# xaskasdf/ntransformer

Hardware: AMD Instinct MI355X
Metric: decode tokens/sec (Llama-3.1-8B Q8_0 class, resident weights, greedy, batch 1) (higher is better)
Workload: dtype f32; 1 GPU; Llama-3.1-8B-shaped Q8_0 GGUF tensors (seed 20260925), resident in HBM, 16-token prompt, greedy decode; ctx=4096, replicas=1, hipgraph=True

## Files before the change

include/ntk_engine.h:

```cpp
#ifndef NTK_ENGINE_H
#define NTK_ENGINE_H

#include "ntk.h"

#if defined(__GNUC__)
#pragma GCC visibility push(default)
#endif
#ifdef __cplusplus
extern "C" {
#endif

int ntk_rope_kv_store(float* q, const float* k, const float* v, const int* positions, int seq_len, int n_heads, int n_kv_heads, int head_dim,
                      float theta_base, float freq_scale, int interleaved, void* k_cache, void* v_cache, int start_pos, int max_seq, void* stream);
typedef struct ntk_gemv_seg {
    const void* W;
    float*      y;
    int         rows;
    int         dtype;
} ntk_gemv_seg;

int ntk_gemv_fused(const ntk_gemv_seg* segs, int nseg, const float* x, int in_features, const float* norm_w,
                   float eps, const float* resid, int silu_pair, void* stream);

size_t ntk_q8l_bytes(int rows, int in_features);
// ... 45 lines not shown
                            const float* inv_freq, int n_heads, int n_kv_heads, int head_dim, int max_seq, float scale, float theta_base,
                            float freq_scale, int nsplit, float* scratch, void* stream);
int ntk_kv_dequant_q8_f16(void* k_f16, void* v_f16, const void* k_cache, const void* v_cache, int n_rows, int n_kv_heads, int head_dim,
                          int max_seq, void* stream);
int ntk_attention_decode_q8_batch(float* output, const float* q, const float* k, const float* v, const ntk_kv_batch* caches, const int* positions,
                                  int n_rows, const float* inv_freq, int n_heads, int n_kv_heads, int head_dim, int max_seq, float scale,
                                  float theta_base, float freq_scale, int nsplit, float* scratch, void* stream);

int ntk_debug_gemv_fused_form(const ntk_gemv_seg* segs, int nseg, const float* x, int in_features, const float* norm_w, float eps,
                              const float* resid, int silu_pair, int integer_activations, void* stream);

size_t   ntk_tp_comm_bytes(size_t max_floats);
void*    ntk_tp_comm_alloc(size_t bytes);
int      ntk_tp_comm_reset(void* comm, void* stream);
float*   ntk_tp_slot(void* comm, size_t max_floats, unsigned call_index);
int      ntk_tp_allreduce_add(float* hidden, void* const* peers, int rank, int world, size_t max_floats, unsigned call_index, int n, void* stream);
int      ntk_tp_advance_epoch(void* comm, void* stream);
unsigned ntk_tp_error(void* comm);
int      ntk_ipc_export(void* devptr, void* handle64);
int      ntk_ipc_open(const void* handle64, void** devptr);
int      ntk_ipc_close(void* devptr);

int ntk_gemm_quant(float* Y, const void* W, const float* X, int n_tokens, int out_features, int in_features,
                   int weight_dtype, const float* resid, void* stream);

typedef struct ntk_gemm_partials {
    const float* part[3];
    float*       y[3];
    int          rows[3];
    int          nseg, n_tokens, nsplit;
} ntk_gemm_partials;
typedef struct ntk_gemm_desc {
    const ntk_gemv_seg* segs;
    int                 nseg;
    const float*        X;
    int                 n_tokens, in_features;
    const float*        resid;
    void*               workspace;
    size_t              workspace_bytes;
    int                 reuse_x;
    const float*        row_max;
    ntk_gemm_partials*  partials;
    int                 weights_repacked;
    int                 full_form;
} ntk_gemm_desc;
size_t ntk_gemm_quant_workspace_bytes(int in_features, int out_features);
int ntk_gemm_quant_f16(const ntk_gemm_desc* desc, void* stream);
int ntk_reduce_rmsnorm_rowmax(float* hidden, const ntk_gemm_partials* partials, const float* weight, float eps, float* x_out, float* row_max,
                              float* zero_tokens, void* stream);
int ntk_reduce_silu_mul_rowmax(float* output, const ntk_gemm_partials* partials, float* row_max, void* stream);
int ntk_rmsnorm_rowmax(float* output, const float* input, const float* weight, int n_tokens, int hidden_size, float eps, float* row_max,
                       float* zero_tokens, void* stream);
int ntk_silu_mul_rowmax(float* output, const float* gate, const float* up, int n_tokens, int width, float* row_max, void* stream);
int ntk_gemm_prepare_x(const float* X, int n_tokens, int in_features, void* workspace, void* stream);
int ntk_rmsnorm_prepare_x(float* output, const float* input, const float* weight, int n_tokens, int hidden_size, float eps, void* workspace, void* stream);
int ntk_reduce_rmsnorm_prepare_x(float* hidden, const ntk_gemm_partials* partials, const float* weight, float eps, float* x_out, void* workspace, void* stream);
int ntk_silu_mul_prepare_x(float* output, const float* gate, const float* up, int n_tokens, int width, void* workspace, void* stream);
int ntk_reduce_silu_mul_prepare_x(float* output, const ntk_gemm_partials* partials, void* workspace, void* stream);

int ntk_embed_rows(float* out, const void* table, const int* tokens, int n_tokens, int hidden, int dtype,
                   void* stream);

int ntk_argmax(const float* logits, int n, int* d_out_token, int* h_mirror, float* scratch, void* stream);

int ntk_logprob_rows(const float* logits, int n_rows, int vocab, int ld, const int* targets, float* logprob, int* top1, void* stream);

size_t ntk_sample_scratch_bytes(int n);
int ntk_sample_top_k(float* logits, int n, const int* d_recent, int n_recent, float repeat_penalty, float temperature,
                     int top_k, float top_p, float r, int* d_out_token, int* h_mirror, void* scratch, void* stream);
int ntk_repeat_penalty(float* logits, int n, const int* d_recent, int n_recent, float repeat_penalty, void* stream);

#define NTK_SAMPLE_ROWS_MAX 16
typedef struct ntk_sample_rows {
    float temperature[NTK_SAMPLE_ROWS_MAX], top_p[NTK_SAMPLE_ROWS_MAX], repeat_penalty[NTK_SAMPLE_ROWS_MAX], r[NTK_SAMPLE_ROWS_MAX];
    int   top_k[NTK_SAMPLE_ROWS_MAX], n_recent[NTK_SAMPLE_ROWS_MAX];
} ntk_sample_rows;
size_t ntk_sample_rows_scratch_bytes(int n_rows, int vocab);
int ntk_sample_rows_top_k(float* logits, int n_rows, int vocab, int ld, const int* d_recent, int recent_ld, const ntk_sample_rows* rows, int* d_out,
                          int* h_mirror, void* scratch, void* stream);

int ntk_argmax_advance(const float* logits, int n, int* d_out_token, int* h_mirror, unsigned long long* h_ring4, int* d_pos,
                       float* scratch, void* stream);

int ntk_debug_sclk(unsigned long long* d_out2, void* stream);
int ntk_debug_sclk_begin(unsigned* d_flag, unsigned long long* d_out2, void* side_stream);
int ntk_debug_sclk_end(unsigned* d_flag, void* other_stream);

void ntk_debug_malloc_budget(long long bytes);

int ntk_advance_pos(int* d_pos, void* stream);

#ifdef __cplusplus
}
#endif
#if defined(__GNUC__)
#pragma GCC visibility pop
#endif
#endif
```

ntransformer_amd/_lib.py:

```python
from __future__ import annotations

import ctypes as C
import os

_HERE = os.path.dirname(os.path.abspath(__file__))
LIB_PATH = os.environ.get("NTK_LIB_PATH") or os.path.join(_HERE, "libntransformer_hip.so")

NTK_OK = 0
_STATUS = {0: "ok", -1: "unsupported dtype", -2: "bad shape", -3: "HIP launch/runtime error", -4: "misaligned pointer",
           -5: "null pointer", -6: "no usable GPU", -7: "out of memory", -8: "I/O error", -9: "malformed GGUF"}


class NtkError(RuntimeError):
    def __init__(self, status: int, what: str = ""):
        self.status = status
        super().__init__("ntk status %d (%s)%s" % (status, _STATUS.get(status, "?"), (": " + what) if what else ""))


def check(status: int, what: str = "") -> None:
    if status != NTK_OK:
        raise NtkError(status, what)


class KvBatch(C.Structure):
# ... 28 lines not shown
        return _lib
    if not os.path.exists(LIB_PATH):
        raise ImportError("%s is missing: run `python -c 'import __graft_entry__ as g; g.build()'` "
                          "(hipcc --offload-arch=gfx950); there is no CPU fallback" % LIB_PATH)
    L = C.CDLL(LIB_PATH, mode=C.RTLD_GLOBAL)
    vp, i, f, sz = C.c_void_p, C.c_int, C.c_float, C.c_size_t
    sig = {
        "ntk_abi_version": (i, []),
        "ntk_status_string": (C.c_char_p, [i]),
        "ntk_row_bytes": (sz, [i, C.c_int64]),
        "ntk_device_count": (i, []),
        "ntk_device_init": (i, [i]),
        "ntk_device_name": (i, [C.c_char_p, sz]),
        "ntk_device_mem_info": (i, [C.POINTER(sz), C.POINTER(sz)]),
        "ntk_stream": (vp, [i]),
        "ntk_stream_synchronize": (i, [vp]),
        "ntk_device_synchronize": (i, []),
        "ntk_event_create": (vp, []),
        "ntk_event_destroy": (i, [vp]),
        "ntk_event_record": (i, [vp, vp]),
        "ntk_event_synchronize": (i, [vp]),
        "ntk_event_elapsed_ms": (i, [vp, vp, C.POINTER(f)]),
        "nt_hip_malloc": (vp, [sz]), "nt_hip_free": (None, [vp]),
        "nt_hip_memcpy_h2d": (None, [vp, vp, sz]), "nt_hip_memcpy_d2h": (None, [vp, vp, sz]),
        "nt_hip_memcpy_d2d": (None, [vp, vp, sz]), "nt_hip_memset": (None, [vp, i, sz]),
        "nt_hip_malloc_host": (vp, [sz]), "nt_hip_free_host": (None, [vp]),
        "ntk_memcpy_h2d_async": (i, [vp, vp, sz, vp]), "ntk_memcpy_d2h_async": (i, [vp, vp, sz, vp]),
        "nt_cuda_malloc": (vp, [sz]), "nt_cuda_free": (None, [vp]),
        "nt_cuda_memcpy_h2d": (None, [vp, vp, sz]), "nt_cuda_memcpy_d2h": (None, [vp, vp, sz]),
        "nt_cuda_memcpy_d2d": (None, [vp, vp, sz]), "nt_cuda_memset": (None, [vp, i, sz]),
        "nt_cuda_malloc_host": (vp, [sz]), "nt_cuda_free_host": (None, [vp]),
        "ntk_rmsnorm": (i, [vp, vp, vp, i, i, f, vp]),
        "ntk_rmsnorm_f16": (i, [vp, vp, vp, i, i, f, vp]),
        "ntk_rope": (i, [vp, vp, vp, i, i, i, i, i, f, f, i, vp]),
        "ntk_softmax": (i, [vp, vp, i, i, vp]),
        "ntk_masked_softmax": (i, [vp, vp, vp, i, i, vp]),
        "ntk_gemv": (i, [vp, vp, vp, i, i, i, vp]),
        "ntk_gemv_add": (i, [vp, vp, vp, i, i, i, vp]),
        "ntk_gemm_f32": (i, [vp, vp, vp, i, i, i, vp]),
        "ntk_silu_mul": (i, [vp, vp, vp, i, vp]),
        "ntk_rmsnorm_rowmax": (i, [vp, vp, vp, i, i, f, vp, vp, vp]),
        "ntk_rope_kv_store": (i, [vp, vp, vp, vp, i, i, i, i, f, f, i, vp, vp, i, i, vp]),
        "ntk_silu_mul_rowmax": (i, [vp, vp, vp, i, i, vp, vp]),
        "ntk_add_bias": (i, [vp, vp, i, vp]),
        "ntk_attention_decode": (i, [vp, vp, vp, vp, i, i, i, i, i, f, vp]),
        "ntk_attention_prefill": (i, [vp, vp, vp, vp, i, i, i, i, i, i, f, vp]),
        "ntk_copy_to_kv_cache": (i, [vp, vp, vp, vp, i, i, i, i, i, vp]),
        "ntk_add": (i, [vp, vp, vp, i, vp]),
        "ntk_add_inplace": (i, [vp, vp, i, vp]),
        "ntk_copy": (i, [vp, vp, i, vp]),
        "ntk_cosine_similarity": (i, [vp, vp, vp, i, vp]),
        "ntk_gemv_fused": (i, [C.POINTER(GemvSeg), i, vp, i, vp, f, vp, i, vp]),
        "ntk_debug_gemv_fused_form": (i, [C.POINTER(GemvSeg), i, vp, i, vp, f, vp, i, i, vp]),
        "ntk_q8l_bytes": (sz, [i, i]),
        "ntk_q8l_pack": (i, [vp, vp, i, i, vp]),
        "ntk_q8l_unpack": (i, [vp, vp, i, i, vp]),
        "ntk_rp_bytes": (sz, [i, i, i]),
        "ntk_rp_pack": (i, [vp, vp, i, i, i, vp]),
        "ntk_rp_dequant": (i, [vp, vp, i, i, i, vp]),
        "ntk_rp_unpack": (i, [vp, vp, i, i, i, vp]),
        "ntk_gemv_rp": (i, [vp, vp, vp, i, i, i, vp]),
        "ntk_gemv_rp_fused": (i, [C.POINTER(GemvSeg), i, vp, i, vp, f, vp, i, vp]),
        "ntk_debug_rp_prologue": (i, [vp, vp, vp, f, i, i, i, vp]),
        "ntk_debug_mfma_i8_probe": (i, [vp, vp, vp, vp]),
        "ntk_gemm_quant": (i, [vp, vp, vp, i, i, i, i, vp, vp]),
        "ntk_attention_decode_split": (i, [vp, vp, vp, vp, vp, vp, vp, vp, i, i, i, i, f, f, f, i, vp, vp]),
        "ntk_attention_split_scratch_bytes": (C.c_size_t, [i, i, i]),
        "ntk_attention_split_scratch_init": (i, [vp, i, vp]),
        "ntk_attention_decode_split_merged": (i, [vp, vp, vp, vp, vp, vp, vp, vp, i, i, i, i, f, f, f, i, vp, vp]),
        "ntk_attention_decode_fused": (i, [vp, vp, vp, vp, vp, vp, vp, vp, i, i, i, i, f, f, f, vp]),
        "ntk_attention_decode_batch": (i, [vp, vp, vp, vp, vp, vp, i, vp, i, i, i, i, f, f, f, i, vp, vp]),
        "ntk_kv_q8_cache_bytes": (C.c_size_t, [i, i, i]),
        "ntk_kv_store_q8": (i, [vp, vp, vp, vp, i, i, i, i, i, vp]),
        "ntk_rope_kv_store_q8": (i, [vp, vp, vp, vp, i, i, i, i, f, f, i, vp, vp, i, i, vp]),
        "ntk_attention_decode_q8": (i, [vp, vp, vp, vp, vp, vp, vp, vp, i, i, i, i, f, f, f, i, vp, vp]),
        "ntk_kv_dequant_q8_f16": (i, [vp, vp, vp, vp, i, i, i, i, vp]),
        "ntk_attention_decode_q8_batch": (i, [vp, vp, vp, vp, vp, vp, i, vp, i, i, i, i, f, f, f, i, vp, vp]),
        "ntk_embed_rows": (i, [vp, vp, vp, i, i, i, vp]),
        "ntk_argmax": (i, [vp, i, vp, vp, vp, vp]),
        "ntk_logprob_rows": (i, [vp, i, i, i, vp, vp, vp, vp]),
        "ntk_sample_rows_scratch_bytes": (C.c_size_t, [i, i]),
        "ntk_sample_rows_top_k": (i, [vp, i, i, i, vp, i, C.POINTER(SampleRows), vp, vp, vp, vp]),
        "ntk_advance_pos": (i, [vp, vp]),
        "ntk_debug_sclk": (i, [vp, vp]),
        "ntk_debug_sclk_begin": (i, [vp, vp, vp]),
        "ntk_debug_sclk_end": (i, [vp, vp]),
    }
    for name, (res, args) in sig.items():
        fn = getattr(L, name)
        fn.restype = res
        fn.argtypes = args
    _lib = L
    return L


EXPORTS_NTK_H = None
```

ntransformer_amd/csrc/common.hip.h:

```cpp
#pragma once
#include <hip/hip_runtime.h>
#include <stdint.h>
#include "../../include/ntk_engine.h"

#define NTK_WAVE 64

#define NTK_HIP_TRY(expr)                                   \
    do {                                                    \
        hipError_t e__ = (expr);                            \
        if (e__ != hipSuccess) return NTK_E_LAUNCH;         \
    } while (0)

#define NTK_EXTRA_API extern "C" __attribute__((visibility("default")))
#ifdef NTK_TUNE
#include <cstdlib>
#define NTK_TUNE_ENV_INT(name, dflt) ([] { const char* e__ = getenv(name); return e__ ? atoi(e__) : (dflt); }())
#else
#define NTK_TUNE_ENV_INT(name, dflt) (dflt)
#endif

namespace ntk {

hipStream_t resolve_stream(void* s);
int         last_launch_status();
int         q8l_gemv_fused(const ntk_gemv_seg* segs, int nseg, const float* x, int in, const float* norm_w, float eps, const float* resid,
                           int silu_pair, hipStream_t st);

__device__ __forceinline__ float h2f(uint16_t bits) {
    _Float16 h;
    __builtin_memcpy(&h, &bits, 2);
    return (float)h;
}
__device__ __forceinline__ uint16_t f2h(float f) {
    _Float16 h = (_Float16)f;
    uint16_t bits;
    __builtin_memcpy(&bits, &h, 2);
    return bits;
}

__device__ __forceinline__ void rope_rotate(const float a, const float b, const float c, const float s, float& ra, float& rb) {
#pragma clang fp contract(off)
    ra = a * c - b * s;
    rb = b * c + a * s;
}

template <int CTRL, int ROW_MASK>
__device__ __forceinline__ float dpp_or_zero(float v) {
    return __int_as_float(__builtin_amdgcn_update_dpp(0, __float_as_int(v), CTRL, ROW_MASK, 0xF, false));
}
template <int CTRL, int ROW_MASK>
__device__ __forceinline__ float dpp_or_self(float v) {
    return __int_as_float(__builtin_amdgcn_update_dpp(__float_as_int(v), __float_as_int(v), CTRL, ROW_MASK, 0xF, false));
}
constexpr int DPP_QUAD_1032 = 0xB1, DPP_QUAD_2301 = 0x4E, DPP_ROW_HALF_MIRROR = 0x141, DPP_ROW_MIRROR = 0x140,
              DPP_ROW_BCAST15 = 0x142, DPP_ROW_BCAST31 = 0x143;

__device__ __forceinline__ float wave_sum_lane63(float v) {
    v += dpp_or_zero<DPP_QUAD_1032, 0xF>(v);
    v += dpp_or_zero<DPP_QUAD_2301, 0xF>(v);
    v += dpp_or_zero<DPP_ROW_HALF_MIRROR, 0xF>(v);
    v += dpp_or_zero<DPP_ROW_MIRROR, 0xF>(v);
    v += dpp_or_zero<DPP_ROW_BCAST15, 0xA>(v);
    v += dpp_or_zero<DPP_ROW_BCAST31, 0xC>(v);
    return v;
}
__device__ __forceinline__ float wave_sum(float v) {
    return __int_as_float(__builtin_amdgcn_readlane(__float_as_int(wave_sum_lane63(v)), 63));
}
__device__ __forceinline__ float wave_max(float v) {
    v = fmaxf(v, dpp_or_self<DPP_QUAD_1032, 0xF>(v));
    v = fmaxf(v, dpp_or_self<DPP_QUAD_2301, 0xF>(v));
    v = fmaxf(v, dpp_or_self<DPP_ROW_HALF_MIRROR, 0xF>(v));
    v = fmaxf(v, dpp_or_self<DPP_ROW_MIRROR, 0xF>(v));
    v = fmaxf(v, dpp_or_self<DPP_ROW_BCAST15, 0xA>(v));
    v = fmaxf(v, dpp_or_self<DPP_ROW_BCAST31, 0xC>(v));
    return __int_as_float(__builtin_amdgcn_readlane(__float_as_int(v), 63));
}

template <int N>
__device__ __forceinline__ float group_sum(float v) {
    static_assert(N == 1 || N == 2 || N == 4 || N == 8 || N == 16 || N == 32, "group size");
    if constexpr (N >= 2) v += dpp_or_zero<DPP_QUAD_1032, 0xF>(v);
    if constexpr (N >= 4) v += dpp_or_zero<DPP_QUAD_2301, 0xF>(v);
    if constexpr (N >= 8) v += dpp_or_zero<DPP_ROW_HALF_MIRROR, 0xF>(v);
    if constexpr (N >= 16) v += dpp_or_zero<DPP_ROW_MIRROR, 0xF>(v);
    if constexpr (N >= 32) v += __shfl_xor(v, 16, 64);
    return v;
}

__device__ __forceinline__ float block_sum(float v, float* red) {
    const int lane = threadIdx.x & 63, wave = threadIdx.x >> 6, nw = (blockDim.x + 63) >> 6;
    v = wave_sum(v);
    __syncthreads();
    if (lane == 0) red[wave] = v;
    __syncthreads();
    float t = 0.0f;
    for (int i = 0; i < nw; ++i) t += red[i];
    return t;
}
__device__ __forceinline__ float block_max(float v, float* red) {
    const int lane = threadIdx.x & 63, wave = threadIdx.x >> 6, nw = (blockDim.x + 63) >> 6;
    v = wave_max(v);
    __syncthreads();
    if (lane == 0) red[wave] = v;
    __syncthreads();
    float t = red[0];
    for (int i = 1; i < nw; ++i) t = fmaxf(t, red[i]);
    return t;
}

__device__ __forceinline__ uint32_t lds_u32_at(const uint8_t* base, int off) {
    const int a = off & ~3;
    const uint32_t lo = *reinterpret_cast<const uint32_t*>(base + a);
    const uint32_t hi = *reinterpret_cast<const uint32_t*>(base + a + 4);
    return __builtin_amdgcn_alignbyte(hi, lo, (uint32_t)(off & 3));
}
template <int N>
__device__ __forceinline__ void lds_read_dwords(uint32_t (&dst)[N], const uint8_t* base, int off) {
    const int a = off & ~3;
    const uint32_t sh = (uint32_t)(off & 3);
    uint32_t w[N + 1];
#pragma unroll
    for (int i = 0; i <= N; ++i) w[i] = *reinterpret_cast<const uint32_t*>(base + a + 4 * i);
#pragma unroll
    for (int i = 0; i < N; ++i) dst[i] = __builtin_amdgcn_alignbyte(w[i + 1], w[i], sh);
}
// ... 26 lines not shown
```

ntransformer_amd/csrc/elementwise.hip:

```cpp
#include "common.hip.h"
#include <cfloat>

namespace ntk {

template <bool HALF_OUT>
__global__ __launch_bounds__(1024) void rmsnorm_kernel(void* __restrict__ output, const float* __restrict__ input,
                                                       const float* __restrict__ weight, int hidden, float eps) {
    __shared__ float red[16];
    const float* x = input + (size_t)blockIdx.x * hidden;
    float ssq = 0.0f;
    for (int i = threadIdx.x; i < hidden; i += blockDim.x) ssq = fmaf(x[i], x[i], ssq);
    const float tot = block_sum(ssq, red);
    const float rms_inv = 1.0f / sqrtf(tot / (float)hidden + eps);
    for (int i = threadIdx.x; i < hidden; i += blockDim.x) {
        const float v = x[i] * rms_inv * weight[i];
        if constexpr (HALF_OUT) reinterpret_cast<uint16_t*>(output)[(size_t)blockIdx.x * hidden + i] = f2h(v);
        else reinterpret_cast<float*>(output)[(size_t)blockIdx.x * hidden + i] = v;
    }
}

template <bool MASKED>
__global__ __launch_bounds__(1024) void softmax_kernel(float* __restrict__ out, const float* __restrict__ in,
                                                       const uint8_t* __restrict__ mask, int cols) {
    __shared__ float red[16];
// ... 18 lines not shown
        const float g = gate[i];
        out[i] = g / (1.0f + expf(-g)) * up[i];
    }
}
__global__ void add_kernel(float* __restrict__ o, const float* __restrict__ a, const float* __restrict__ b, int n) {
    const int i = blockIdx.x * blockDim.x + threadIdx.x;
    if (i < n) o[i] = a[i] + b[i];
}
__global__ void copy_kernel(float* __restrict__ d, const float* __restrict__ s, int n) {
    const int i = blockIdx.x * blockDim.x + threadIdx.x;
    if (i < n) d[i] = s[i];
}
__global__ void gemm_f32_kernel(float* __restrict__ C, const float* __restrict__ A, const float* __restrict__ B, int M, int N, int K) {
    const int col = blockIdx.x * blockDim.x + threadIdx.x, row = blockIdx.y * blockDim.y + threadIdx.y;
    if (row >= M || col >= N) return;
    float s = 0.0f;
    for (int k = 0; k < K; ++k) s = fmaf(A[(size_t)row * K + k], B[(size_t)col * K + k], s);
    C[(size_t)row * N + col] = s;
}
__global__ __launch_bounds__(256) void cosine_kernel(float* __restrict__ result, const float* __restrict__ a,
                                                     const float* __restrict__ b, int n) {
    __shared__ float red[16];
    float d = 0.0f, na = 0.0f, nb = 0.0f;
    for (int i = threadIdx.x; i < n; i += blockDim.x) {
        d = fmaf(a[i], b[i], d); na = fmaf(a[i], a[i], na); nb = fmaf(b[i], b[i], nb);
    }
    d = block_sum(d, red); na = block_sum(na, red); nb = block_sum(nb, red);
    if (threadIdx.x == 0) {
        const float den = sqrtf(na) * sqrtf(nb);
        *result = den > 1e-8f ? d / den : 0.0f;
    }
}

__device__ float embed_elem(const uint8_t* __restrict__ table, int tok, int hidden, int dt, int e) {
    switch (dt) {
        case NTK_DT_F32: return reinterpret_cast<const float*>(table)[(size_t)tok * hidden + e];
        case NTK_DT_F16: return h2f(reinterpret_cast<const uint16_t*>(table)[(size_t)tok * hidden + e]);
        case NTK_DT_Q8_0: {
            const uint8_t* b = table + ((size_t)tok * (hidden / 32) + e / 32) * 34;
            const float d = h2f((uint16_t)(b[0] | (b[1] << 8)));
            return __fmul_rn(d, (float)(int8_t)b[2 + (e & 31)]);
        }
        case NTK_DT_Q4_0: {
            const uint8_t* b = table + ((size_t)tok * (hidden / 32) + e / 32) * 18;
            const float d = h2f((uint16_t)(b[0] | (b[1] << 8)));
            const int j = e & 31;
            const int nib = j < 16 ? (b[2 + j] & 0x0F) : (b[2 + j - 16] >> 4);
            return __fmul_rn(d, (float)(nib - 8));
        }
        case NTK_DT_Q4_K: {
            const uint8_t* b = table + ((size_t)tok * (hidden / 256) + e / 256) * 144;
            const float d = h2f((uint16_t)(b[0] | (b[1] << 8))), dmin = h2f((uint16_t)(b[2] | (b[3] << 8)));
            const int w = e & 255, sub = w >> 5, l = w & 31, chunk = sub >> 1;
            const uint8_t* s = b + 4;
            uint32_t sc, mn;
            if (sub < 4) { sc = s[sub] & 63; mn = s[sub + 4] & 63; }
            else { sc = (s[sub + 4] & 0x0F) | ((s[sub - 4] >> 6) << 4); mn = (s[sub + 4] >> 4) | ((s[sub] >> 6) << 4); }
            const uint8_t qb = b[16 + 32 * chunk + l];
            const int nib = (sub & 1) ? (qb >> 4) : (qb & 0x0F);
            return __fsub_rn(__fmul_rn(__fmul_rn(d, (float)sc), (float)nib), __fmul_rn(dmin, (float)mn));
        }
        case NTK_DT_Q6_K: {
            const uint8_t* b = table + ((size_t)tok * (hidden / 256) + e / 256) * 210;
            const float d = h2f((uint16_t)(b[208] | (b[209] << 8)));
            const int w = e & 255, hf = w >> 7, g = (w >> 5) & 3, l = w & 31, is = l >> 4;
            const uint8_t* ql = b + 64 * hf;
            const uint8_t* qh = b + 128 + 32 * hf;
            const int8_t sc = (int8_t)b[192 + 8 * hf + is + 2 * g];
            const uint8_t qlb = ql[l + 32 * (g & 1)];
            const int lo = (g >> 1) ? (qlb >> 4) : (qlb & 0x0F);
            const int q = (lo | (((qh[l] >> (2 * g)) & 3) << 4)) - 32;
            return __fmul_rn(__fmul_rn(d, (float)sc), (float)q);
        }
        default: return 0.0f;
    }
}
__global__ void embed_rows_kernel(float* __restrict__ out, const uint8_t* __restrict__ table, const int* __restrict__ tokens,
                                  int hidden, int dt) {
    const int tok = tokens[blockIdx.x];
    const int e = blockIdx.y * blockDim.x + threadIdx.x;
    if (e < hidden) out[(size_t)blockIdx.x * hidden + e] = embed_elem(table, tok, hidden, dt, e);
}

__device__ __forceinline__ void amax_merge(float& v, int& i, float ov, int oi) {
    if (ov > v || (ov == v && oi < i)) { v = ov; i = oi; }
}
__global__ __launch_bounds__(256) void argmax_stage1(const float* __restrict__ x, int n, float* __restrict__ sv, int* __restrict__ si) {
    __shared__ float rv[4];
    __shared__ int ri[4];
    float v = -FLT_MAX;
    int idx = 0x7FFFFFFF;
    for (int i = blockIdx.x * blockDim.x + threadIdx.x; i < n; i += gridDim.x * blockDim.x) amax_merge(v, idx, x[i], i);
    for (int off = 32; off > 0; off >>= 1) amax_merge(v, idx, __shfl_xor(v, off, 64), __shfl_xor(idx, off, 64));
    if ((threadIdx.x & 63) == 0) { rv[threadIdx.x >> 6] = v; ri[threadIdx.x >> 6] = idx; }
    __syncthreads();
    if (threadIdx.x == 0) {
        for (int w = 1; w < 4; ++w) amax_merge(v, idx, rv[w], ri[w]);
        sv[blockIdx.x] = v; si[blockIdx.x] = idx;
    }
}
__global__ __launch_bounds__(256) void argmax_stage2(const float* __restrict__ sv, const int* __restrict__ si, int nblk,
                                                     int* __restrict__ d_out, int* __restrict__ h_mirror) {
    __shared__ float rv[4];
    __shared__ int ri[4];
    float v = -FLT_MAX;
    int idx = 0x7FFFFFFF;
    for (int i = threadIdx.x; i < nblk; i += blockDim.x) amax_merge(v, idx, sv[i], si[i]);
    for (int off = 32; off > 0; off >>= 1) amax_merge(v, idx, __shfl_xor(v, off, 64), __shfl_xor(idx, off, 64));
    if ((threadIdx.x & 63) == 0) { rv[threadIdx.x >> 6] = v; ri[threadIdx.x >> 6] = idx; }
    __syncthreads();
    if (threadIdx.x == 0) {
        for (int w = 1; w < 4; ++w) amax_merge(v, idx, rv[w], ri[w]);
        if (idx == 0x7FFFFFFF) idx = 0;
        *d_out = idx;
        if (h_mirror) *h_mirror = idx;
    }
}
__global__ void advance_pos_kernel(int* p) { if (threadIdx.x == 0 && blockIdx.x == 0) *p += 1; }

__global__ __launch_bounds__(64) void sclk_probe_kernel(unsigned long long* out) {
    const unsigned long long t0 = __builtin_amdgcn_s_memtime(), r0 = __builtin_amdgcn_s_memrealtime();
    unsigned long long r1 = r0;
    float acc = (float)threadIdx.x;
    while (r1 - r0 < 5000ull) {
#pragma unroll
        for (int i = 0; i < 64; ++i) acc = fmaf(acc, 1.0000001f, 1e-9f);
        r1 = __builtin_amdgcn_s_memrealtime();
    }
    const unsigned long long t1 = __builtin_amdgcn_s_memtime();
    if (threadIdx.x == 0) { out[0] = t1 - t0; out[1] = r1 - r0; }
    if (acc == 12345.678f) out[2] = 0;
}

__global__ __launch_bounds__(64) void sclk_span_kernel(const unsigned* flag, unsigned long long* out) {
    const unsigned long long t0 = __builtin_amdgcn_s_memtime(), r0 = __builtin_amdgcn_s_memrealtime();
    unsigned long long r1 = r0;
    for (;;) {
        __builtin_amdgcn_s_sleep(64);
        r1 = __builtin_amdgcn_s_memrealtime();
        if (__hip_atomic_load(flag, __ATOMIC_RELAXED, __HIP_MEMORY_SCOPE_SYSTEM) != 0u || r1 - r0 > 300000000ull) break;
    }
    const unsigned long long t1 = __builtin_amdgcn_s_memtime();
    if (threadIdx.x == 0) { out[0] = t1 - t0; out[1] = r1 - r0; }
}

__global__ __launch_bounds__(256) void argmax_advance_stage2(const float* __restrict__ sv, const int* __restrict__ si, int nblk,
                                                             int* __restrict__ d_out, int* __restrict__ h_mirror,
                                                             unsigned long long* __restrict__ h_ring, int* __restrict__ d_pos) {
    __shared__ float rv[4];
    __shared__ int ri[4];
    float v = -FLT_MAX;
    int idx = 0x7FFFFFFF;
    for (int i = threadIdx.x; i < nblk; i += blockDim.x) amax_merge(v, idx, sv[i], si[i]);
    for (int off = 32; off > 0; off >>= 1) amax_merge(v, idx, __shfl_xor(v, off, 64), __shfl_xor(idx, off, 64));
    if ((threadIdx.x & 63) == 0) { rv[threadIdx.x >> 6] = v; ri[threadIdx.x >> 6] = idx; }
    __syncthreads();
    if (threadIdx.x == 0) {
        for (int w = 1; w < 4; ++w) amax_merge(v, idx, rv[w], ri[w]);
        if (idx == 0x7FFFFFFF) idx = 0;
        const int pos = *d_pos;
        *d_out = idx;
        if (h_mirror) *h_mirror = idx;
        if (h_ring)
            __hip_atomic_store(h_ring + (pos & 3), (unsigned long long)(unsigned)idx | ((unsigned long long)(unsigned)(pos + 1) << 32),
                               __ATOMIC_RELEASE, __HIP_MEMORY_SCOPE_SYSTEM);
        *d_pos = pos + 1;
    }
}

static inline dim3 g1(int n) { return dim3((n + 255) / 256); }

}

extern "C" {
using namespace ntk;

static int rms_block(int hidden) { return hidden <= 1024 ? 256 : (hidden <= 4096 ? 512 : 1024); }

int ntk_rmsnorm(float* output, const float* input, const float* weight, int batch_size, int hidden_size, float eps, void* stream) {
    if (!output || !input || !weight) return NTK_E_NULL;
    if (batch_size < 0 || hidden_size <= 0) return NTK_E_SHAPE;
    if (batch_size == 0) return NTK_OK;
    hipLaunchKernelGGL(rmsnorm_kernel<false>, dim3(batch_size), dim3(rms_block(hidden_size)), 0, resolve_stream(stream),
                       (void*)output, input, weight, hidden_size, eps);
    return last_launch_status();
}
int ntk_rmsnorm_f16(void* output, const float* input, const float* weight, int batch_size, int hidden_size, float eps, void* stream) {
    if (!output || !input || !weight) return NTK_E_NULL;
    if (batch_size < 0 || hidden_size <= 0) return NTK_E_SHAPE;
    if (batch_size == 0) return NTK_OK;
    hipLaunchKernelGGL(rmsnorm_kernel<true>, dim3(batch_size), dim3(rms_block(hidden_size)), 0, resolve_stream(stream),
                       output, input, weight, hidden_size, eps);
    return last_launch_status();
}
int ntk_softmax(float* output, const float* input, int rows, int cols, void* stream) {
    if (!output || !input) return NTK_E_NULL;
    if (rows < 0 || cols <= 0) return NTK_E_SHAPE;
    if (rows == 0) return NTK_OK;
    hipLaunchKernelGGL(softmax_kernel<false>, dim3(rows), dim3(cols <= 1024 ? 256 : 1024), 0, resolve_stream(stream), output,
                       input, (const uint8_t*)nullptr, cols);
    return last_launch_status();
}
int ntk_masked_softmax(float* output, const float* input, const uint8_t* mask, int rows, int cols, void* stream) {
    if (!output || !input || !mask) return NTK_E_NULL;
    if (rows < 0 || cols <= 0) return NTK_E_SHAPE;
    if (rows == 0) return NTK_OK;
    hipLaunchKernelGGL(softmax_kernel<true>, dim3(rows), dim3(cols <= 1024 ? 256 : 1024), 0, resolve_stream(stream), output,
                       input, mask, cols);
    return last_launch_status();
}
int ntk_gemm_f32(float* C, const float* A, const float* B, int M, int N, int K, void* stream) {
    if (!C || !A || !B) return NTK_E_NULL;
    if (M < 0 || N < 0 || K < 0) return NTK_E_SHAPE;
    if (M == 0 || N == 0) return NTK_OK;
    hipLaunchKernelGGL(gemm_f32_kernel, dim3((N + 15) / 16, (M + 15) / 16), dim3(16, 16), 0, resolve_stream(stream), C, A, B, M, N, K);
    return last_launch_status();
}
int ntk_silu_mul(float* output, const float* gate, const float* up, int size, void* stream) {
    if (!output || !gate || !up) return NTK_E_NULL;
    if (size < 0) return NTK_E_SHAPE;
    if (size == 0) return NTK_OK;
    hipLaunchKernelGGL(silu_mul_kernel, g1(size), dim3(256), 0, resolve_stream(stream), output, gate, up, size);
    return last_launch_status();
}
int ntk_add(float* out, const float* a, const float* b, int size, void* stream) {
    if (!out || !a || !b) return NTK_E_NULL;
    if (size < 0) return NTK_E_SHAPE;
    if (size == 0) return NTK_OK;
    hipLaunchKernelGGL(add_kernel, g1(size), dim3(256), 0, resolve_stream(stream), out, a, b, size);
    return last_launch_status();
}
int ntk_add_inplace(float* a, const float* b, int size, void* stream) { return ntk_add(a, a, b, size, stream); }
int ntk_add_bias(float* y, const float* bias, int size, void* stream) { return ntk_add(y, y, bias, size, stream); }
int ntk_copy(float* dst, const float* src, int size, void* stream) {
    if (!dst || !src) return NTK_E_NULL;
    if (size < 0) return NTK_E_SHAPE;
    if (size == 0) return NTK_OK;
    hipLaunchKernelGGL(copy_kernel, g1(size), dim3(256), 0, resolve_stream(stream), dst, src, size);
    return last_launch_status();
}
int ntk_cosine_similarity(float* result, const float* a, const float* b, int size, void* stream) {
    if (!result || !a || !b) return NTK_E_NULL;
    if (size < 0) return NTK_E_SHAPE;
    hipLaunchKernelGGL(cosine_kernel, dim3(1), dim3(256), 0, resolve_stream(stream), result, a, b, size);
    return last_launch_status();
}
int ntk_embed_rows(float* out, const void* table, const int* tokens, int n_tokens, int hidden, int dtype, void* stream) {
    if (!out || !table || !tokens) return NTK_E_NULL;
    if (n_tokens < 0 || hidden <= 0) return NTK_E_SHAPE;
    if (n_tokens == 0) return NTK_OK;
    hipLaunchKernelGGL(embed_rows_kernel, dim3(n_tokens, (hidden + 255) / 256), dim3(256), 0, resolve_stream(stream), out, (const uint8_t*)table,
                       tokens, hidden, dtype);
    const int st = last_launch_status();
    if (st != NTK_OK) return st;
    switch (dtype) {
        case NTK_DT_F32: case NTK_DT_F16: case NTK_DT_Q8_0: case NTK_DT_Q4_0: case NTK_DT_Q4_K: case NTK_DT_Q6_K: return NTK_OK;
        default: return NTK_E_DTYPE;
    }
}
int ntk_argmax(const float* logits, int n, int* d_out_token, int* h_mirror, float* scratch, void* stream) {
    if (!logits || !d_out_token || !scratch) return NTK_E_NULL;
    if (n <= 0) return NTK_E_SHAPE;
    const int nblk = n < 256 * 8 ? 1 : (n / (256 * 8) < 1024 ? n / (256 * 8) : 1024);
    float* sv = scratch;
    int* si = reinterpret_cast<int*>(scratch + 1024);
    hipStream_t st = resolve_stream(stream);
    hipLaunchKernelGGL(argmax_stage1, dim3(nblk), dim3(256), 0, st, logits, n, sv, si);
    hipLaunchKernelGGL(argmax_stage2, dim3(1), dim3(256), 0, st, (const float*)sv, (const int*)si, nblk, d_out_token, h_mirror);
    return last_launch_status();
}
int ntk_argmax_advance(const float* logits, int n, int* d_out_token, int* h_mirror, unsigned long long* h_ring4, int* d_pos, float* scratch,
                       void* stream) {
    if (!logits || !d_out_token || !scratch || !d_pos) return NTK_E_NULL;
    if (n <= 0) return NTK_E_SHAPE;
    const int nblk = n < 256 * 8 ? 1 : (n / (256 * 8) < 1024 ? n / (256 * 8) : 1024);
    float* sv = scratch;
    int* si = reinterpret_cast<int*>(scratch + 1024);
    hipStream_t st = resolve_stream(stream);
    hipLaunchKernelGGL(argmax_stage1, dim3(nblk), dim3(256), 0, st, logits, n, sv, si);
    hipLaunchKernelGGL(argmax_advance_stage2, dim3(1), dim3(256), 0, st, (const float*)sv, (const int*)si, nblk, d_out_token, h_mirror, h_ring4, d_pos);
    return last_launch_status();
}
int ntk_debug_sclk(unsigned long long* d_out2, void* stream) {
    if (!d_out2) return NTK_E_NULL;
    hipLaunchKernelGGL(sclk_probe_kernel, dim3(1), dim3(64), 0, resolve_stream(stream), d_out2);
    return last_launch_status();
}
int ntk_debug_sclk_begin(unsigned* d_flag, unsigned long long* d_out2, void* side_stream) {
    if (!d_flag || !d_out2 || !side_stream) return NTK_E_NULL;
    hipStream_t st = static_cast<hipStream_t>(side_stream);
    if (hipMemsetAsync(d_flag, 0, 4, st) != hipSuccess) return NTK_E_LAUNCH;
    hipLaunchKernelGGL(sclk_span_kernel, dim3(1), dim3(64), 0, st, (const unsigned*)d_flag, d_out2);
    return last_launch_status();
}
int ntk_debug_sclk_end(unsigned* d_flag, void* other_stream) {
    if (!d_flag || !other_stream) return NTK_E_NULL;
    static const unsigned one = 1u;
    return hipMemcpyAsync(d_flag, &one, 4, hipMemcpyHostToDevice, static_cast<hipStream_t>(other_stream)) == hipSuccess ? NTK_OK : NTK_E_LAUNCH;
}
int ntk_advance_pos(int* d_pos, void* stream) {
    if (!d_pos) return NTK_E_NULL;
    hipLaunchKernelGGL(advance_pos_kernel, dim3(1), dim3(64), 0, resolve_stream(stream), d_pos);
    return last_launch_status();
}

}
```

ntransformer_amd/csrc/engine/model.cpp:

```cpp
#include "model_impl.h"
#include <thread>

namespace nt {

Model::~Model() { free_all(); }

void Model::drop_graphs(int slot) {
    for (auto& row : graphs_)
        for (int k = 0; k <= kAttnRegimes; ++k) {
            if (slot >= 0 && k != slot) continue;
            if (row[k]) (void)hipGraphExecDestroy(reinterpret_cast<hipGraphExec_t>(row[k]));
            row[k] = nullptr;
        }
}

void Model::free_all() {
    drop_graphs();
    destroy_persistent_plan();
    persistent_on_ = false;
    for (int r = 0; r < 8; ++r) {
        if (tp_peer_opened_[r] && tp_peers_[r]) (void)ntk_ipc_close(tp_peers_[r]);
        tp_peers_[r] = nullptr;
        tp_peer_opened_[r] = false;
    }
    tp_connected_ = false;
    tp_comm_ = nullptr;
    tp_call_ = 0;
    if (own_stream_ && stream_) (void)hipStreamDestroy(static_cast<hipStream_t>(stream_));
    own_stream_ = false;
    stream_ = nullptr;
    for (void* p : allocs_) nt_hip_free(p);
    allocs_.clear();
    auto free_host = [](auto*& p) { if (p) nt_hip_free_host(p); p = nullptr; };
    free_host(h_token_); free_host(h_ring_); free_host(h_recent_); free_host(h_batch_recent_); free_host(h_batch_next_);
    sample_scratch_ = gemm_ws_ = gemm_ws2_ = nullptr;
    d_recent_ = nullptr;
    attn_sync_ = nullptr;
    shares_weights_ = false;
    layers_.clear();
    token_embd_ = output_norm_ = output_ = DevTensor();
    weight_bytes_ = repack_bytes_ = raw_freed_bytes_ = 0;
    raw_scratch_ = nullptr; raw_scratch_bytes_ = raw_cursor_ = 0; raw_err_ = 0;
    repack_done_ = output_tied_ = false;
    host_pos_ = attn_regime_ = 0;
    k_cache_ = v_cache_ = nullptr;
    slot_k_.clear(); slot_v_.clear(); slot_k_q8_.clear(); slot_v_q8_.clear();
    batch_logits_ = batch_logprob_ = batch_attn_scratch_ = nullptr; batch_in_ = batch_next_ = batch_recent_ = nullptr; batch_sample_scratch_ = nullptr;
    kv_capture_ = nullptr; kv_capture_layer_ = -1; kv_capture_T_ = 0;
    k_cache_q8_ = v_cache_q8_ = nullptr; kv_f16_k_ = kv_f16_v_ = nullptr; kv_q8_layer_bytes_ = 0; kv_cache_bytes_ = 0;
    hidden_ = residual_ = workspace_ = logits_ = argmax_scratch_ = rope_inv_freq_ = attn_scratch_ = row_max_ = nullptr;
    positions_ = tokens_dev_ = d_pos_ = d_token_ = nullptr;
    score_logits_ = score_logprob_ = nullptr; score_targets_ = score_top1_ = nullptr; score_cap_ = 0;
    score_ws_ = nullptr; score_ws_bytes_ = 0;
}

int Model::share_weights(const Model& src, int max_context) {
    if (&src == this) { err_ = "share_weights: a model cannot share its own weights"; return NTK_E_NULL; }
    free_all();
    if (src.layers_.empty()) { err_ = "share_weights: the source model is not loaded"; return NTK_E_NULL; }
    if (src.tp_world_ != 1 || src.shares_weights_) {
        err_ = "share_weights: the source must hold whole tensors of its own (no tensor parallelism, not itself a sharing sequence)";
        return NTK_E_SHAPE;
    }
    cfg_ = src.cfg_;
    cfg_full_ = src.cfg_;
    if (max_context > 0) cfg_.max_seq_len = max_context;
    vocab_ = src.vocab_;
    layers_ = src.layers_;
    token_embd_ = src.token_embd_; output_norm_ = src.output_norm_; output_ = src.output_;
    output_tied_ = src.output_tied_;
    weight_bytes_ = src.weight_bytes_;
    repack_ = src.repack_; repack_wanted_ = src.repack_; repack_done_ = true;
    repack_bytes_ = 0;
    shares_weights_ = true;
    if (src.raw_freed_bytes_ > 0 && src.raw_scratch_bytes_ > 0) {
        void* d = nt_hip_malloc(src.raw_scratch_bytes_);
        if (!d) { err_ = "share_weights: no device memory for the unpack scratch"; free_all(); return NTK_E_NOMEM; }
        allocs_.push_back(d);
        raw_scratch_ = d; raw_scratch_bytes_ = src.raw_scratch_bytes_;
        raw_freed_bytes_ = src.raw_freed_bytes_;
    }
    int rc = own_stream();
    if (rc == NTK_OK) rc = alloc_buffers();
    if (rc != NTK_OK) free_all();
    return rc;
}

int Model::set_attention_merge(bool on) {
    if (on == attn_merge_) return NTK_OK;
    if (!layers_.empty()) {
        NT_TRY(sync());
        drop_graphs();
    }
    attn_merge_ = on;
    return NTK_OK;
}

int Model::set_repack(int level) {
    level = level < 0 ? 0 : level > 3 ? 3 : level;
    if (shares_weights_) { err_ = "set_repack: this sequence shares another model's tensors"; return NTK_E_SHAPE; }
    repack_wanted_ = level;
    if (layers_.empty()) { repack_ = level; return NTK_OK; }
    if (level == 3) level = 2;
    if (level == repack_) return NTK_OK;
    NT_TRY(sync());
    drop_graphs();
    int rc = NTK_OK;
    if (level < 2 && raw_freed_bytes_ > 0) rc = restore_raw_all();
    if (rc == NTK_OK && level > 0 && !repack_done_) {
        rc = repack_all();
        if (rc == NTK_E_NOMEM) { fprintf(stderr, "warning: decode repack incomplete (device memory): the rest stays on the raw path\n"); rc = NTK_OK; err_.clear(); }
    }
    if (rc != NTK_OK) { err_ = std::string("set_repack: ") + ntk_status_string(rc); return rc; }
    repack_ = level;
    if (level == 2) {
        destroy_persistent_plan();
        persistent_on_ = false;
        rc = drop_raw_all();
    }
    return rc;
}

uint64_t Model::bytes_per_token(int pos) const {
    uint64_t b = 0;
    for (const auto& L : layers_)
        for (auto m : kLayerMatrices) b += (L.*m).nbytes;
    b += output_.nbytes;
    b += (uint64_t)(2 * cfg_.n_layers + 1) * cfg_.hidden_size * 4;
    const uint64_t kv_elems = (uint64_t)cfg_.n_kv_heads * cfg_.head_dim;
    const uint64_t kv_row = kv_q8_ ? kv_elems + kv_elems / 16 : kv_elems * 2;
    b += 2ull * cfg_.n_layers * kv_row * (uint64_t)(pos + 1) + 2ull * cfg_.n_layers * kv_row;
    b += ntk_row_bytes(token_embd_.dtype, cfg_.hidden_size);
    return b;
}

int Model::set_device_token(int token) {
    if (token < 0 || token >= cfg_.vocab_size) { err_ = "token id out of range"; return NTK_E_SHAPE; }
    *h_token_ = token;
    return ntk_memcpy_h2d_async(d_token_, h_token_, 4, stream_);
}
int Model::set_device_pos(int pos) {
    host_pos_ = pos;
    NT_TRY(ntk_memcpy_h2d_async(d_pos_, &pos, 4, stream_));
    NT_TRY(ntk_stream_synchronize(stream_));
    if (h_ring_) memset(h_ring_, 0, 64);
    return NTK_OK;
}
int Model::sync() { return ntk_stream_synchronize(stream_); }
int Model::host_token() const { return *h_token_; }
int Model::copy_logits(float* host) {
    NT_TRY(ntk_memcpy_d2h_async(host, logits_, (size_t)cfg_.vocab_size * 4, stream_));
    return ntk_stream_synchronize(stream_);
}

int Model::sample_on_device(const int* recent, int n_recent, float repeat_penalty, float temperature, int top_k, float top_p, float r) {
    if (!sample_scratch_ || !d_recent_ || !h_recent_) return NTK_E_NOMEM;
    if (n_recent > kRecentCap) { recent += n_recent - kRecentCap; n_recent = kRecentCap; }
    void* s = stream_;
    if (repeat_penalty > 1.0f && n_recent > 0) {
        memcpy(h_recent_, recent, (size_t)n_recent * 4);
        NT_TRY(ntk_memcpy_h2d_async(d_recent_, h_recent_, (size_t)n_recent * 4, s));
    } else {
        n_recent = 0;
    }
    if (temperature <= 0.0f) {
        NT_TRY(ntk_repeat_penalty(logits_, cfg_.vocab_size, d_recent_, n_recent, repeat_penalty, s));
        return ntk_argmax(logits_, cfg_.vocab_size, d_token_, h_token_, argmax_scratch_, s);
    }
    return ntk_sample_top_k(logits_, cfg_.vocab_size, d_recent_, n_recent, repeat_penalty, temperature, top_k, top_p, r, d_token_,
                            h_token_, sample_scratch_, s);
}

int Model::wait_token(int pos, int* token) {
    volatile unsigned long long* slot = h_ring_ + (pos & 3);
    const unsigned want = (unsigned)(pos + 1);
    for (unsigned spins = 0;; ++spins) {
        const unsigned long long v = *slot;
        if ((unsigned)(v >> 32) == want) { *token = (int)(unsigned)v; return NTK_OK; }
#if defined(__x86_64__) || defined(__i386__)
        __builtin_ia32_pause();
#else
        std::this_thread::yield();
#endif
        if ((spins & 0xFFFFu) == 0xFFFFu) {
            const auto now = std::chrono::steady_clock::now();
            if (spins == 0xFFFFu) wait_t0_ = now;
            else if (std::chrono::duration<double>(now - wait_t0_).count() > 2.0) break;
        }
    }
    static bool warned = false;
    if (!warned) { warned = true; fprintf(stderr, "warning: the pinned token ring was not seen updating for 2 s (host memory not coherent with a running kernel?); falling back to a stream synchronisation per token\n"); }
    NT_TRY(ntk_stream_synchronize(stream_));
    const unsigned long long v = *slot;
    if ((unsigned)(v >> 32) != want) { err_ = "decode step finished without publishing its token"; return NTK_E_LAUNCH; }
    *token = (int)(unsigned)v;
    return NTK_OK;
}

int Model::set_sequences(int n) {
    if (n < 1 || n > kMaxSequences) { err_ = "sequences must lie in 1 .. " + std::to_string(kMaxSequences); return NTK_E_SHAPE; }
    sequences_ = n;
    return NTK_OK;
}

int Model::set_batch_kv_q8(bool on) {
    if (!layers_.empty()) { err_ = "batch_kv_q8 must be set before the model is loaded"; return NTK_E_SHAPE; }
    batch_kv_q8_ = on;
    return NTK_OK;
}

int Model::set_kv_cache(const std::string& kind) {
    if (kind != "f16" && kind != "q8_0") { err_ = "kv_cache: unknown format '" + kind + "' (f16 or q8_0)"; return NTK_E_DTYPE; }
    if (!layers_.empty()) { err_ = "kv_cache must be set before the model is loaded"; return NTK_E_SHAPE; }
    const bool q8 = kind == "q8_0";
    if (q8 && fuse_attention_) { err_ = "kv_cache=q8_0 is not supported with the attention-inside-Wo launch (fuse_attention)"; return NTK_E_SHAPE; }
    kv_q8_ = q8;
    return NTK_OK;
}

int Model::set_fuse_attention(bool on) {
    if (on && kv_q8_) { err_ = "fuse_attention (attention inside the Wo launch) is not supported with kv_cache=q8_0"; return NTK_E_SHAPE; }
    fuse_attention_ = on;
    return NTK_OK;
}

bool Model::use_persistent_now() const {
    return persistent_plan_ && persistent_on_ && attn_regime_ == 0 && !prof_;
}

void Model::set_persistent(int level) {
    const bool on = level != 0;
    persistent_on_ = false;
    persistent_wanted_ = level;
    if (on && !experiments_built()) fprintf(stderr, "note: the persistent token kernels are built by experiments/Makefile only (experiments/libntransformer_hip_exp.so); this library decodes with fused launches\n");
    if (persistent_plan_ && persistent_kind_ != (level == 2 ? 2 : 1)) {
        (void)sync();
        destroy_persistent_plan();
    }
    if (!on || tp_world_ != 1 || layers_.empty()) return;
    if (kv_q8_) { fprintf(stderr, "note: the persistent token kernels read the F16 KV cache; kv_cache=q8_0 decodes with fused launches\n"); return; }
// ... 43 lines not shown
```

ntransformer_amd/csrc/engine/model.h:

```cpp
#pragma once
#include <array>
#include <chrono>
#include <cstdint>
#include <string>
#include <vector>
#include "gguf.h"
#include "synth.h"

struct ntk_sample_rows;

struct ihipGraphExec_t;

namespace nt {

struct DevTensor {
    void* ptr = nullptr;
    int dtype = 0;
    int64_t in_f = 0, out_f = 0;
    size_t nbytes = 0;
    void* rp = nullptr;
    size_t rp_bytes = 0;
};

struct LayerWeights {
// ... 39 lines not shown
        if (pos < 544) return 0;
        return pos < (head_dim == 128 ? 3072 : 16384) ? 1 : 2;
    }
    static int attention_splits(int regime, int head_dim) { return regime <= 1 ? 8 : head_dim == 128 ? 32 : 16; }
    static constexpr int kMaxAttnSplits = 32;
    void pick_attention_regime();
    int sync();
    int host_token() const;
    int wait_token(int pos, int* token);
    float* logits_ptr() { return logits_; }
    int copy_logits(float* host);
    int sample_on_device(const int* recent, int n_recent, float repeat_penalty, float temperature, int top_k, float top_p, float r);
    static bool device_sampler_supports(float temperature, int top_k, int vocab) {
        return temperature <= 0.0f || (top_k > 0 && top_k <= 64 && top_k < vocab && vocab <= 131072);
    }

    const ModelConfig& config() const { return cfg_; }
    const GgufVocab& vocab() const { return vocab_; }
    const std::string& error() const { return err_; }
    uint64_t weight_bytes() const { return weight_bytes_; }
    uint64_t bytes_per_token(int pos) const;
    void set_batched_prefill(bool on) { batched_prefill_ = on; }
    void set_persistent(int level);
    int persistent_kind() const { return persistent_plan_ ? persistent_kind_ : 0; }
    int set_fuse_attention(bool on);
    int set_kv_cache(const std::string& kind);
    bool kv_q8() const { return kv_q8_; }
    static int kv_q8_splits(int regime) { return regime == 0 ? 4 : regime == 1 ? 16 : 32; }
    uint64_t kv_cache_bytes() const { return kv_cache_bytes_; }
    int debug_kv_inputs_capture(int layer);
    int debug_kv_inputs_read(int n, float* k, float* v);
    int debug_kv_q8(int layer, int pos0, int n, uint8_t* k_blocks, uint8_t* v_blocks, bool write, int slot = 0);
    void set_prefill_row_max(bool on) { prefill_row_max_ = on; }
    void set_prefill_fused_split(bool on) { prefill_fused_split_ = on; }
    int set_attention_merge(bool on);
    int set_repack(int level);
    bool repack() const { return repack_ != 0; }
    int repack_level() const { return repack_; }
    uint64_t repack_bytes() const { return repack_bytes_; }
    uint64_t resident_weight_bytes() const { return weight_bytes_ - raw_freed_bytes_ + repack_bytes_ + raw_scratch_bytes_; }
    void set_bf16_prefill(bool on) { bf16_prefill_ = on; }
    bool persistent_available() const { return persistent_plan_ != nullptr; }
    void* persistent_plan() const { return persistent_plan_; }
    const char* decode_path() const;
    int check_persistent();
    int check_tp();
    int debug_run_layers(const float* hidden_in, int T, int start_pos, int first, int count, int mode, float* hidden_out);
    int debug_kv(int layer, int pos0, int n, uint16_t* k, uint16_t* v, bool write, int slot = 0);
    int profile_token(float ms[4], int calls[4], bool coarse);
    void* stream() const { return stream_; }

    int tp_configure(int rank, int world);
    int tp_rank() const { return tp_rank_; }
    int tp_world() const { return tp_world_; }
    int tp_export(void* handle64, void** raw);
    int tp_connect(const void* handles, void* const* raws);
    unsigned tp_error();
    static int slice_columns(void* dst, const void* src, int dtype, int64_t out_f, int64_t in_f, int rank, int world);

private:
    int load_impl(const std::string& gguf_path, int max_context);
    int finish_load();
    int init_device();
    int own_stream();
    int alloc_buffers();
    int upload(DevTensor& dst, const void* host, int dtype, int64_t in_f, int64_t out_f, size_t nbytes);
    int upload_shard(DevTensor& dst, const void* host_full, int dtype, int64_t in_f, int64_t out_f, size_t nbytes_full, Shard how);
    struct TensorSlot { DevTensor* dst; Shard how; int64_t in_f, out_f; };
    bool slot_of(const std::string& name, TensorSlot* slot);
    template <class F> void for_each_projection(F&& fn) { for (auto& L : layers_) for (auto m : kLayerMatrices) fn(L.*m); fn(output_); }
    int repack_all();
    int repack_one(DevTensor& t);
    int drop_raw_all();
    int restore_raw_all();
    void raw_begin() { raw_cursor_ = 0; }
    const void* raw_of(const DevTensor& t);
    int tp_check_shapes();
    int tp_allreduce(float* hidden, int n);
    float* tp_slot() const;
    void free_all();
    void drop_graphs(int slot = -1);
    struct Views { float *q, *k, *v, *attn_out, *gate, *up; };
    Views views(int T) const;
    int enqueue_token(bool greedy);
    int enqueue_layers(int first, int last);
    int decode_project(const DevTensor* const* ws, float* const* ys, int n, const float* x, const DevTensor* norm, const float* resid, int kind,
                       int silu_pair = 0, bool timed = true);
    struct KvTarget { int slot; const int* slots; int max_pos; };
    int layers_1to1(int T, int start_pos, int first, int last, const KvTarget& kv = KvTarget{0, nullptr, 0});
    int lm_head(float* logits, const float* X, int n, const float* row_max);
    bool lm_head_f16() const;
    int lm_head_workspace(const char* who);
    int batch_buffers();
    int batch_logits(const int* slots, const int* tokens, const int* positions, int B);
    int batch_sample_buffers();
    int score_buffers();
    void prof_mark(int cls, bool begin);
    bool use_persistent_now() const;
    static bool experiments_built();
    int build_persistent_plan(int kind);
    void destroy_persistent_plan();
    int launch_persistent();
    int attention_in_wo(const LayerWeights& L, int layer);
    int check_experiments();

    ModelConfig cfg_;
    GgufVocab vocab_;
    std::string err_;
    std::vector<LayerWeights> layers_;
    DevTensor token_embd_, output_norm_, output_;
    bool output_tied_ = false;
    uint64_t weight_bytes_ = 0;
    std::vector<void*> allocs_;
    bool shares_weights_ = false;

    uint16_t* k_cache_ = nullptr;
    uint16_t* v_cache_ = nullptr;
    bool kv_q8_ = false;
    int sequences_ = 1;
    std::vector<uint16_t*> slot_k_, slot_v_;
    float* batch_logits_ = nullptr;
    int* batch_in_ = nullptr;
    int batch_host_[3 * 16] = {};
    float* batch_logprob_ = nullptr;
    int* batch_next_ = nullptr;
    float* batch_attn_scratch_ = nullptr;
    int* batch_recent_ = nullptr;
    int* h_batch_recent_ = nullptr;
    void* batch_sample_scratch_ = nullptr;
    int* h_batch_next_ = nullptr;
    uint8_t* k_cache_q8_ = nullptr;
    uint8_t* v_cache_q8_ = nullptr;
    size_t kv_q8_layer_bytes_ = 0;
    bool batch_kv_q8_ = false;
    std::vector<uint8_t*> slot_k_q8_, slot_v_q8_;
    uint16_t* kv_f16_k_ = nullptr;
    uint16_t* kv_f16_v_ = nullptr;
    uint64_t kv_cache_bytes_ = 0;
    float* kv_capture_ = nullptr;
    int kv_capture_layer_ = -1, kv_capture_T_ = 0;
    float* hidden_ = nullptr;
    float* residual_ = nullptr;
    float* workspace_ = nullptr;
    size_t workspace_floats_ = 0;
    float* logits_ = nullptr;
    int score_rows_ = 256;
    float* score_logits_ = nullptr;
    int score_cap_ = 0;
    int* score_targets_ = nullptr;
    float* score_logprob_ = nullptr;
    int* score_top1_ = nullptr;
    void* score_ws_ = nullptr;
    size_t score_ws_bytes_ = 0;
    int* positions_ = nullptr;
    int* tokens_dev_ = nullptr;
    int* d_pos_ = nullptr;
    int* d_token_ = nullptr;
    int* h_token_ = nullptr;
    unsigned long long* h_ring_ = nullptr;
    std::chrono::steady_clock::time_point wait_t0_;
    float* argmax_scratch_ = nullptr;
    void* sample_scratch_ = nullptr;
    int* d_recent_ = nullptr;
    int* h_recent_ = nullptr;
    static constexpr int kRecentCap = kMaxRecent;
    float* rope_inv_freq_ = nullptr;
    void* stream_ = nullptr;
    bool batched_prefill_ = true;
    struct Timed { int cls; void* a; void* b; int n; bool shared_a; };
    bool prof_coarse_ = false;
    std::vector<Timed>* prof_ = nullptr;
    static constexpr int kPersistentSlot = kAttnRegimes;
    ihipGraphExec_t* graphs_[2][kAttnRegimes + 1] = {};
    int host_pos_ = 0;
    int attn_regime_ = 0;
    float* attn_scratch_ = nullptr;
    bool prefill_row_max_ = true;
    float* row_max_ = nullptr;
    void* gemm_ws_ = nullptr;
    void* gemm_ws2_ = nullptr;
    bool prefill_fused_split_ = true;
    size_t gemm_ws_bytes_ = 0;
    bool bf16_prefill_ = true;
    unsigned* attn_sync_ = nullptr;
    int repack_ = 3;
    int repack_wanted_ = 3;
    bool repack_done_ = false;
    uint64_t repack_bytes_ = 0;
    uint64_t raw_freed_bytes_ = 0;
    void* raw_scratch_ = nullptr;
    size_t raw_scratch_bytes_ = 0, raw_cursor_ = 0;
    int raw_err_ = 0;
    bool attn_merge_ = false;
    bool fuse_attention_ = false;
    int tp_rank_ = 0, tp_world_ = 1;
    void* tp_comm_ = nullptr;
    size_t tp_max_floats_ = 0;
    void* tp_peers_[8] = {nullptr, nullptr, nullptr, nullptr, nullptr, nullptr, nullptr, nullptr};
    bool tp_peer_opened_[8] = {false, false, false, false, false, false, false, false};
    bool tp_connected_ = false;
    unsigned tp_call_ = 0;
    bool own_stream_ = false;
    ModelConfig cfg_full_;
    void* persistent_plan_ = nullptr;
    bool persistent_on_ = false;
    int persistent_wanted_ = 0;
    int persistent_kind_ = 1;
};

}
```

ntransformer_amd/csrc/engine/model_debug.cpp:

```cpp
#include "model_impl.h"

namespace nt {

int Model::debug_run_layers(const float* hidden_in, int T, int start_pos, int first, int count, int mode, float* hidden_out) {
    if (!hidden_in || !hidden_out) return NTK_E_NULL;
    if (T <= 0 || start_pos < 0 || start_pos + T > cfg_.max_seq_len || first < 0 || count < 0 || first + count > cfg_.n_layers) return NTK_E_SHAPE;
    if (mode != 0 && T != 1) return NTK_E_SHAPE;
    if (tp_world_ > 1) return NTK_E_SHAPE;
    const size_t bytes = (size_t)T * cfg_.hidden_size * 4;
    void* s = stream_;
    NT_TRY(ntk_memcpy_h2d_async(hidden_, hidden_in, bytes, s));
    int rc;
    if (mode == 0) {
        std::vector<int> pos(T);
        for (int i = 0; i < T; ++i) pos[i] = start_pos + i;
        NT_TRY(ntk_memcpy_h2d_async(positions_, pos.data(), (size_t)T * 4, s));
        NT_TRY(ntk_stream_synchronize(s));
        rc = layers_1to1(T, start_pos, first, first + count);
    } else {
        NT_TRY(set_device_pos(start_pos));
        pick_attention_regime();
        if (mode == 1) {
            rc = enqueue_layers(first, first + count);
        } else {
            hipStream_t st = static_cast<hipStream_t>(s);
            hipGraphExec_t ex = nullptr;
            rc = capture_graph(st, hipStreamCaptureModeThreadLocal, [&] { return enqueue_layers(first, first + count); }, &ex);
            if (rc == NTK_OK && hipGraphLaunch(ex, st) != hipSuccess) rc = NTK_E_LAUNCH;
            if (rc == NTK_OK) rc = ntk_stream_synchronize(s);
            if (ex) (void)hipGraphExecDestroy(ex);
        }
    }
    if (rc != NTK_OK) return rc;
    NT_TRY(ntk_memcpy_d2h_async(hidden_out, hidden_, bytes, s));
    return ntk_stream_synchronize(s);
}

int Model::debug_kv(int layer, int pos0, int n, uint16_t* k, uint16_t* v, bool write, int slot) {
    if (!k || !v) return NTK_E_NULL;
    if (kv_q8_) { err_ = "debug_kv: the KV cache is q8_0 (use the _q8 form)"; return NTK_E_DTYPE; }
    if (layer < 0 || layer >= cfg_.n_layers || pos0 < 0 || n < 0 || pos0 + n > cfg_.max_seq_len || slot < 0 || slot >= (int)slot_k_.size()) return NTK_E_SHAPE;
    const size_t per = (size_t)cfg_.n_kv_heads * cfg_.head_dim;
    uint16_t* const kcache = slot_k_[slot];
    uint16_t* const vcache = slot_v_[slot];
    const size_t off = ((size_t)layer * cfg_.max_seq_len + pos0) * per, bytes = (size_t)n * per * 2;
    void* s = stream_;
    NT_TRY(write ? ntk_memcpy_h2d_async(kcache + off, k, bytes, s) : ntk_memcpy_d2h_async(k, kcache + off, bytes, s));
    NT_TRY(write ? ntk_memcpy_h2d_async(vcache + off, v, bytes, s) : ntk_memcpy_d2h_async(v, vcache + off, bytes, s));
    return ntk_stream_synchronize(s);
}

int Model::debug_kv_q8(int layer, int pos0, int n, uint8_t* k_blocks, uint8_t* v_blocks, bool write, int slot) {
    if (!k_blocks || !v_blocks) return NTK_E_NULL;
    if (!kv_q8_) { err_ = "debug_kv_q8: the KV cache is f16"; return NTK_E_DTYPE; }
    if (layer < 0 || layer >= cfg_.n_layers || pos0 < 0 || n < 0 || pos0 + n > cfg_.max_seq_len || slot < 0 || slot >= (int)slot_k_q8_.size()) return NTK_E_SHAPE;
    if (n == 0) return NTK_OK;
    const size_t per = (size_t)cfg_.n_kv_heads * cfg_.head_dim, nb = per / 32;
    const size_t qbytes = (size_t)n * per, sbytes = (size_t)n * nb * 2;
    void* s = stream_;
    std::vector<uint8_t> qh(qbytes), sh(sbytes);
    for (int side = 0; side < 2; ++side) {
        uint8_t* base = (side ? slot_v_q8_[slot] : slot_k_q8_[slot]) + (size_t)layer * kv_q8_layer_bytes_;
        uint8_t* qd = base + (size_t)pos0 * per;
        uint8_t* sd = base + (size_t)cfg_.max_seq_len * per + (size_t)pos0 * nb * 2;
        uint8_t* blocks = side ? v_blocks : k_blocks;
        if (write) {
            for (size_t b = 0; b < (size_t)n * nb; ++b) {
                memcpy(&sh[2 * b], blocks + 34 * b, 2);
                memcpy(&qh[32 * b], blocks + 34 * b + 2, 32);
            }
            NT_TRY(ntk_memcpy_h2d_async(qd, qh.data(), qbytes, s));
            NT_TRY(ntk_memcpy_h2d_async(sd, sh.data(), sbytes, s));
            NT_TRY(ntk_stream_synchronize(s));
        } else {
            NT_TRY(ntk_memcpy_d2h_async(qh.data(), qd, qbytes, s));
            NT_TRY(ntk_memcpy_d2h_async(sh.data(), sd, sbytes, s));
            NT_TRY(ntk_stream_synchronize(s));
            for (size_t b = 0; b < (size_t)n * nb; ++b) {
                memcpy(blocks + 34 * b, &sh[2 * b], 2);
                memcpy(blocks + 34 * b + 2, &qh[32 * b], 32);
            }
        }
    }
    return NTK_OK;
}

int Model::debug_kv_inputs_capture(int layer) {
    if (layers_.empty()) return NTK_E_NULL;
    if (layer >= cfg_.n_layers) return NTK_E_SHAPE;
    kv_capture_layer_ = layer < 0 ? -1 : layer;
    kv_capture_T_ = 0;
    if (layer >= 0 && !kv_capture_) {
        const size_t bytes = 2 * (size_t)cfg_.max_seq_len * cfg_.n_kv_heads * cfg_.head_dim * 4;
// ... 17 lines not shown
```

ntransformer_amd/csrc/engine/model_decode.cpp:

```cpp
#include "model_impl.h"

namespace nt {

void Model::prof_mark(int cls, bool begin) {
    if (!prof_) return;
    void* s = stream_;
    if (prof_coarse_) {
        if (!begin) return;
        if (!prof_->empty() && prof_->back().cls == cls) { ++prof_->back().n; return; }
        void* e = ntk_event_create();
        ntk_event_record(e, s);
        const bool shared = !prof_->empty();
        if (shared) prof_->back().b = e;
        prof_->push_back({cls, e, nullptr, 1, shared});
        return;
    }
    void* e = ntk_event_create();
    ntk_event_record(e, s);
    if (begin) prof_->push_back({cls, e, nullptr, 1, false}); else prof_->back().b = e;
}

int Model::enqueue_token(bool greedy) {
    const int H = cfg_.hidden_size;
    void* s = stream_;
    tp_call_ = 0;
    prof_mark(2, true);
    const int est = ntk_embed_rows(hidden_, token_embd_.ptr, d_token_, 1, H, token_embd_.dtype, s);
    prof_mark(2, false);
    if (est != NTK_OK && est != NTK_E_DTYPE) return est;
    if (use_persistent_now()) {
        NT_TRY(launch_persistent());
    } else {
        NT_TRY(enqueue_layers(0, cfg_.n_layers));
        const DevTensor* const w = &output_;
        const bool timed = is_quant(w->dtype);
        if (timed) prof_mark(0, true);
        NT_TRY(decode_project(&w, &logits_, 1, hidden_, &output_norm_, nullptr, 16, 0, false));
        if (timed) prof_mark(0, false);
    }
    prof_mark(2, true);
    if (greedy) NT_TRY(ntk_argmax_advance(logits_, cfg_.vocab_size, d_token_, h_token_, h_ring_, d_pos_, argmax_scratch_, s));
    else NT_TRY(ntk_advance_pos(d_pos_, s));
    if (tp_world_ > 1) NT_TRY(ntk_tp_advance_epoch(tp_comm_, s));
    prof_mark(2, false);
    return NTK_OK;
}

int Model::decode_project(const DevTensor* const* ws, float* const* ys, int n, const float* x, const DevTensor* norm, const float* resid, int kind,
                          int silu_pair, bool timed) {
    const int H = cfg_.hidden_size;
    void* s = stream_;
    auto mark = [&](bool begin) { if (timed) prof_mark(0, begin); };
    const float* nw = norm ? (const float*)norm->ptr : nullptr;
    auto one_launch = [&](bool rp, const float* r, int silu) {
        ntk_gemv_seg segs[3];
        if (!rp) raw_begin();
        for (int a = 0; a < n; ++a) segs[a] = {rp ? ws[a]->rp : raw_of(*ws[a]), ys[a], (int)ws[a]->out_f, ws[a]->dtype};
        mark(true);
        const int st = (rp ? ntk_gemv_rp_fused : ntk_gemv_fused)(segs, n, x, (int)ws[0]->in_f, nw, cfg_.norm_eps, r, silu, s);
        mark(false);
        return st;
    };
    bool all_rp = repack_ && (rp_mask() & kind), all_quant = true, mixed = false;
    for (int a = 0; a < n; ++a) {
        all_rp = all_rp && ws[a]->rp != nullptr && ws[a]->in_f == ws[0]->in_f;
        all_quant = all_quant && is_quant(ws[a]->dtype);
        mixed = mixed || ws[a]->dtype != ws[0]->dtype;
    }
    if (all_rp) {
        const int st = one_launch(true, resid, silu_pair);
        if (!not_taken(st)) return st;
    }
    if (n > 1 && !resid && all_quant && mixed) {
        const int st = one_launch(false, nullptr, 0);
        if (!not_taken(st)) return st;
    }
    bool done[3] = {false, false, false};
    for (int a = 0; a < n; ++a) {
        if (done[a]) continue;
        const DevTensor& w = *ws[a];
        if (!is_quant(w.dtype)) {
            const float* xin = x;
            if (nw) {
                NT_TRY(ntk_rmsnorm(residual_ + H, x, nw, 1, (int)w.in_f, cfg_.norm_eps, s));
                xin = residual_ + H;
            }
            float* y = resid ? residual_ : ys[a];
            raw_begin();
            NT_TRY(ntk_gemv(y, raw_of(w), xin, (int)w.out_f, (int)w.in_f, w.dtype, s));
            if (resid) NT_TRY(ntk_add(ys[a], resid, residual_, (int)w.out_f, s));
            done[a] = true;
            continue;
        }
        ntk_gemv_seg segs[3];
        int m = 0;
        raw_begin();
        for (int b = a; b < n; ++b) {
            if (done[b] || ws[b]->dtype != w.dtype) continue;
            segs[m++] = {raw_of(*ws[b]), ys[b], (int)ws[b]->out_f, ws[b]->dtype};
            done[b] = true;
        }
        mark(true);
        NT_TRY(ntk_gemv_fused(segs, m, x, (int)w.in_f, nw, cfg_.norm_eps, resid, silu_pair, s));
        mark(false);
    }
    return NTK_OK;
}

int Model::enqueue_layers(int first, int last_layer) {
    const int H = cfg_.hidden_size, I = cfg_.intermediate_size, hd = cfg_.head_dim, nh = cfg_.n_heads, nkv = cfg_.n_kv_heads;
    void* s = stream_;
    const float scale = 1.0f / sqrtf((float)hd);
    const size_t kv_layer = (size_t)cfg_.max_seq_len * nkv * hd;
    const Views act = views(1);
    auto project_add = [&](const DevTensor& w, const float* x, int kind) -> int {
        const DevTensor* const wp = &w;
        float* y = tp_world_ > 1 ? tp_slot() : hidden_;
        NT_TRY(decode_project(&wp, &y, 1, x, nullptr, tp_world_ > 1 ? nullptr : hidden_, kind));
        return tp_world_ > 1 ? tp_allreduce(hidden_, H) : (int)NTK_OK;
    };

    for (int i = first; i < last_layer; ++i) {
        const LayerWeights& L = layers_[i];
        const DevTensor* const qkv[3] = {&L.wq, &L.wk, &L.wv};
        float* const qkv_out[3] = {act.q, act.k, act.v};
        NT_TRY(decode_project(qkv, qkv_out, 3, hidden_, &L.attn_norm, nullptr, 1));
        const int fused = fuse_attention_ ? attention_in_wo(L, i) : (int)NTK_E_SHAPE;
        if (fused != NTK_OK) {
            if (!not_taken(fused)) return fused;
            uint16_t* kc = kv_q8_ ? nullptr : k_cache_ + (size_t)i * kv_layer;
            uint16_t* vc = kv_q8_ ? nullptr : v_cache_ + (size_t)i * kv_layer;
            prof_mark(1, true);
            if (kv_q8_)
                NT_TRY(ntk_attention_decode_q8(act.attn_out, act.q, act.k, act.v, k_cache_q8_ + (size_t)i * kv_q8_layer_bytes_,
                                               v_cache_q8_ + (size_t)i * kv_q8_layer_bytes_, d_pos_, rope_inv_freq_, nh, nkv, hd, cfg_.max_seq_len, scale,
                                               cfg_.rope_theta, cfg_.rope_freq_scale, kv_q8_splits(attn_regime_), attn_scratch_, s));
            else if (attn_regime_ == 0)
                NT_TRY(ntk_attention_decode_fused(act.attn_out, act.q, act.k, act.v, kc, vc, d_pos_, rope_inv_freq_, nh, nkv, hd,
                                                  cfg_.max_seq_len, scale, cfg_.rope_theta, cfg_.rope_freq_scale, s));
            else
                NT_TRY((attn_merge_ ? ntk_attention_decode_split_merged : ntk_attention_decode_split)(
                    act.attn_out, act.q, act.k, act.v, kc, vc, d_pos_, rope_inv_freq_, nh, nkv, hd, cfg_.max_seq_len, scale, cfg_.rope_theta,
                    cfg_.rope_freq_scale, attention_splits(attn_regime_, hd), attn_scratch_, s));
            prof_mark(1, false);
            NT_TRY(project_add(L.wo, act.attn_out, 2));
        }
        const DevTensor* const ffn[2] = {&L.w_gate, &L.w_up};
        float* const ffn_out[2] = {act.gate, act.up};
        const bool pair = is_quant(L.w_gate.dtype) && L.w_gate.dtype == L.w_up.dtype;
        if (pair) prof_mark(0, true);
        NT_TRY(decode_project(ffn, ffn_out, 2, hidden_, &L.ffn_norm, nullptr, 4, pair, !pair));
        if (pair) prof_mark(0, false);
        else NT_TRY(ntk_silu_mul(act.gate, act.gate, act.up, I, s));
        NT_TRY(project_add(L.w_down, act.gate, 8));
    }
    return NTK_OK;
}

void Model::pick_attention_regime() {
    attn_regime_ = (attn_scratch_ && (cfg_.head_dim == 64 || cfg_.head_dim == 128 || cfg_.head_dim == 256))
                       ? attention_regime(host_pos_, cfg_.head_dim) : 0;
    ++host_pos_;
}

int Model::decode_step_fused(bool greedy, bool use_graph) {
    pick_attention_regime();
    if (!use_graph) return enqueue_token(greedy);
    ihipGraphExec_t*& slot = graphs_[greedy ? 1 : 0][use_persistent_now() ? kPersistentSlot : attn_regime_];
    hipStream_t st = static_cast<hipStream_t>(stream_);
    if (!slot) {
        hipGraphExec_t ex = nullptr;
        NT_TRY(capture_graph(st, tp_world_ > 1 ? hipStreamCaptureModeRelaxed : hipStreamCaptureModeThreadLocal, [&] { return enqueue_token(greedy); }, &ex));
        slot = reinterpret_cast<ihipGraphExec_t*>(ex);
    }
    return hipGraphLaunch(reinterpret_cast<hipGraphExec_t>(slot), st) == hipSuccess ? NTK_OK : NTK_E_LAUNCH;
}

int Model::profile_token(float ms[4], int calls[4], bool coarse) {
    std::vector<Timed> rec;
    rec.reserve(1024);
    prof_ = &rec;
    prof_coarse_ = coarse;
    pick_attention_regime();
    int rc = enqueue_token(true);
    if (coarse && !rec.empty()) {
        void* e = ntk_event_create();
        ntk_event_record(e, stream_);
        rec.back().b = e;
    }
    prof_ = nullptr;
    prof_coarse_ = false;
    if (rc == NTK_OK) rc = ntk_stream_synchronize(stream_);
    for (int c = 0; c < 4; ++c) { ms[c] = 0.0f; calls[c] = 0; }
    for (auto& t : rec) {
        float m = 0.0f;
        if (t.a && t.b && ntk_event_elapsed_ms(t.a, t.b, &m) == NTK_OK) { ms[t.cls] += m; calls[t.cls] += t.n; }
        ++calls[3];
    }
    for (auto& t : rec) {
        if (t.a && !t.shared_a) ntk_event_destroy(t.a);
        if (t.b) ntk_event_destroy(t.b);
    }
    return rc;
}

}
```

ntransformer_amd/csrc/engine/model_prompt.cpp:

```cpp
#include "model_impl.h"
#include <type_traits>

namespace nt {

float* Model::forward(const int* tokens, int T, int start_pos, int slot) {
    if (T <= 0 || start_pos < 0 || start_pos + T > cfg_.max_seq_len) { err_ = "forward: sequence exceeds context"; return nullptr; }
    if (slot < 0 || slot >= sequences_) { err_ = "forward: no such sequence slot"; return nullptr; }
    for (int i = 0; i < T; ++i)
        if (tokens[i] < 0 || tokens[i] >= cfg_.vocab_size) { err_ = "forward: token id out of range"; return nullptr; }
    const int H = cfg_.hidden_size;
    void* s = stream_;
    tp_call_ = 0;
    if (ntk_memcpy_h2d_async(tokens_dev_, tokens, (size_t)T * 4, s) != NTK_OK) return nullptr;
    const int est = ntk_embed_rows(hidden_, token_embd_.ptr, tokens_dev_, T, H, token_embd_.dtype, s);
    if (est == NTK_E_DTYPE) fprintf(stderr, "Error: Unsupported embedding dtype: %s\n", dtype_name(token_embd_.dtype));
    else if (est != NTK_OK) return nullptr;
    std::vector<int> pos(T);
    for (int i = 0; i < T; ++i) pos[i] = start_pos + i;
    if (ntk_memcpy_h2d_async(positions_, pos.data(), (size_t)T * 4, s) != NTK_OK) return nullptr;
    if (ntk_stream_synchronize(s) != NTK_OK) return nullptr;

    const KvTarget kv{slot, nullptr, 0};
    int rc = layers_1to1(T, start_pos, 0, cfg_.n_layers, kv);
    auto ok = [&](int st) { if (st != NTK_OK && rc == NTK_OK) rc = st; };
    float* last = hidden_ + (size_t)(T - 1) * H;
    ok(ntk_rmsnorm(last, last, (const float*)output_norm_.ptr, 1, H, cfg_.norm_eps, s));
    {
        raw_begin();
        const int st = ntk_gemv(logits_, raw_of(output_), last, (int)output_.out_f, (int)output_.in_f, output_.dtype, s);
        if (st == NTK_E_DTYPE) fprintf(stderr, "Unsupported dtype for GEMV: %s\n", dtype_name(output_.dtype));
        else ok(st);
    }
    if (tp_world_ > 1) ok(ntk_tp_advance_epoch(tp_comm_, s));
    ok(ntk_stream_synchronize(s));
    if (raw_err_ != NTK_OK) { rc = raw_err_; raw_err_ = NTK_OK; }
    if (rc == NTK_OK) rc = check_tp();
    if (rc != NTK_OK) { if (err_.empty() || rc != NTK_E_LAUNCH) err_ = std::string("forward failed: ") + ntk_status_string(rc); return nullptr; }
    return logits_;
}

struct OperandPlanes {
    void* ws[2];
    int cur = 0;
    const float* of = nullptr;
    void* current() const { return ws[cur]; }
    bool hold(const float* X) const { return X == of; }
    void* other() { cur ^= 1; of = nullptr; return ws[cur]; }
    void written(const float* X, bool split) { of = split ? X : nullptr; }
    void in_current(const float* X) { of = X; }
};

static bool f16_ok(const DevTensor& w) {
    const bool kq = w.dtype == NTK_DT_Q4_0 || w.dtype == NTK_DT_Q4_K || w.dtype == NTK_DT_Q5_K || w.dtype == NTK_DT_Q6_K;
    return (w.dtype == NTK_DT_Q8_0 || kq) && w.in_f % (kq ? 256 : 128) == 0 && w.out_f % 16 == 0 && (w.ptr || w.rp);
}
static bool rp_only(const DevTensor& w) {
    return !w.ptr && w.rp && (w.dtype == NTK_DT_Q4_K || w.dtype == NTK_DT_Q5_K || w.dtype == NTK_DT_Q6_K) && w.out_f % 16 == 0;
}

int Model::layers_1to1(int T, int start_pos, int first, int last_layer, const KvTarget& kv) {
    const int H = cfg_.hidden_size, I = cfg_.intermediate_size, hd = cfg_.head_dim, nh = cfg_.n_heads, nkv = cfg_.n_kv_heads;
    const int qd = nh * hd, kvd = nkv * hd;
    void* s = stream_;
    const size_t kv_layer = (size_t)cfg_.max_seq_len * kvd;
    const float scale = 1.0f / sqrtf((float)hd);
    const Views act = views(T);
    int rc = NTK_OK;
    auto ok = [&](int st) { if (st != NTK_OK && rc == NTK_OK) rc = st; };
    auto gemv = [&](float* y, const DevTensor& w, const void* wp, const float* x) {
        const int st = ntk_gemv(y, wp, x, (int)w.out_f, (int)w.in_f, w.dtype, s);
        if (st == NTK_E_DTYPE) fprintf(stderr, "Unsupported dtype for GEMV: %s\n", dtype_name(w.dtype));
        else ok(st);
    };
    const bool batched = batched_prefill_ && T > 1;
    const bool bf16_now = bf16_prefill_ && gemm_ws_ && T > 1;
    OperandPlanes planes{{gemm_ws_, gemm_ws2_}};
    const bool with_max = batched && bf16_now && row_max_ != nullptr && prefill_row_max_;
    float* rm_a = with_max ? row_max_ : nullptr;
    float* rm_b = with_max ? row_max_ + cfg_.max_seq_len : nullptr;
    enum class XForm { plain, row_max, split };
    auto x_form = [&](int width, const DevTensor& next_w) {
        if (with_max && prefill_fused_split_ && gemm_ws2_ != nullptr && T <= 64 && tp_world_ == 1 && f16_ok(next_w) && (int)next_w.in_f == width) return XForm::split;
        return with_max ? XForm::row_max : XForm::plain;
    };
    auto gemm_group = [&](float* const* Ys, const DevTensor* const* Ws, int n, const float* X, const float* resid, const float* rm, ntk_gemm_partials* pt,
                          const void* const* raw) {
        bool repacked = raw == nullptr;
        for (int k = 0; k < n; ++k) repacked = repacked && rp_only(*Ws[k]);
        if (!repacked && !raw) raw_begin();
        ntk_gemv_seg segs[3];
        for (int k = 0; k < n; ++k) segs[k] = {repacked ? Ws[k]->rp : raw ? raw[k] : raw_of(*Ws[k]), Ys[k], (int)Ws[k]->out_f, Ws[k]->dtype};
        ntk_gemm_desc d{};
        d.segs = segs; d.nseg = n; d.X = X; d.n_tokens = T; d.in_features = (int)Ws[0]->in_f; d.resid = resid;
        d.workspace = planes.current(); d.workspace_bytes = gemm_ws_bytes_; d.reuse_x = planes.hold(X) ? 1 : 0; d.row_max = rm; d.partials = pt;
        d.weights_repacked = repacked ? 1 : 0;
// ... 192 lines not shown
    };
    auto release = [&](auto*& p) {
        if (!p) return;
        allocs_.erase(std::remove(allocs_.begin(), allocs_.end(), (void*)p), allocs_.end());
        nt_hip_free(p);
        p = nullptr;
    };
    auto fail = [&](const char* what) { err_ = std::string("score: no device memory for ") + what; return NTK_E_NOMEM; };
    if (!score_targets_ && !(score_targets_ = (int*)dev(S * 4))) return fail("the targets");
    if (!score_logprob_ && !(score_logprob_ = (float*)dev(S * 4))) return fail("the results");
    if (!score_top1_ && !(score_top1_ = (int*)dev(S * 4))) return fail("the results");
    if (score_cap_ < score_rows_) {
        NT_TRY(sync());
        release(score_logits_);
        score_cap_ = 0;
        if (!(score_logits_ = (float*)dev((size_t)score_rows_ * V * 4))) return fail("the chunk of logits (score_rows x vocab floats)");
        score_cap_ = score_rows_;
    }
    return lm_head_workspace("score");
}

int Model::lm_head_workspace(const char* who) {
    const size_t need = ntk_gemm_quant_workspace_bytes(cfg_.hidden_size, cfg_.vocab_size);
    if (!(gemm_ws_ && bf16_prefill_ && f16_ok(output_) && need > gemm_ws_bytes_ && need > score_ws_bytes_)) return NTK_OK;
    if (score_ws_) {
        NT_TRY(sync());
        allocs_.erase(std::remove(allocs_.begin(), allocs_.end(), score_ws_), allocs_.end());
        nt_hip_free(score_ws_);
        score_ws_ = nullptr;
    }
    score_ws_bytes_ = 0;
    if (!(score_ws_ = nt_hip_malloc(need + 256))) { err_ = std::string(who) + ": no device memory for the LM head's GEMM workspace"; return NTK_E_NOMEM; }
    allocs_.push_back(score_ws_);
    score_ws_bytes_ = need;
    return NTK_OK;
}

bool Model::lm_head_f16() const { return batched_prefill_ && is_quant(output_.dtype) && bf16_prefill_ && gemm_ws_ && f16_ok(output_); }

int Model::lm_head(float* logits, const float* X, int n, const float* chunk_max) {
    const DevTensor& w = output_;
    const int H = cfg_.hidden_size, V = cfg_.vocab_size;
    void* s = stream_;
    const bool batched = batched_prefill_ && is_quant(w.dtype);
    void* const ws = score_ws_ ? score_ws_ : gemm_ws_;
    const size_t ws_bytes = score_ws_ ? score_ws_bytes_ : gemm_ws_bytes_;
    int st = NTK_E_DTYPE;
    if (lm_head_f16()) {
        const bool repacked = rp_only(w);
        if (!repacked) raw_begin();
        const ntk_gemv_seg seg{repacked ? w.rp : raw_of(w), logits, V, w.dtype};
        ntk_gemm_desc d{};
        d.segs = &seg; d.nseg = 1; d.X = X; d.n_tokens = n; d.in_features = H;
        d.workspace = ws; d.workspace_bytes = ws_bytes; d.row_max = chunk_max; d.weights_repacked = repacked ? 1 : 0;
        d.full_form = 1;
        st = ntk_gemm_quant_f16(&d, s);
    }
    if (batched && not_taken(st)) { raw_begin(); st = ntk_gemm_quant(logits, raw_of(w), X, n, V, H, w.dtype, nullptr, s); }
    if (batched && !not_taken(st)) return st;
    raw_begin();
    const void* wp = raw_of(w);
    for (int t = 0; t < n; ++t) {
        st = ntk_gemv(logits + (size_t)t * V, wp, X + (size_t)t * H, V, H, w.dtype, s);
        if (st == NTK_E_DTYPE) fprintf(stderr, "Unsupported dtype for GEMV: %s\n", dtype_name(w.dtype));
        if (st != NTK_OK) return st;
    }
    return NTK_OK;
}

int Model::score(const int* tokens, const int* targets, int T, int start_pos, float* logprob_out, int* top1_out, int slot) {
    if (!tokens || !targets || !logprob_out) { err_ = "score: null argument"; return NTK_E_NULL; }
    if (tp_world_ > 1) { err_ = "score: not available under tensor parallelism"; return NTK_E_SHAPE; }
    if (T <= 0) { err_ = "score: no tokens to score"; return NTK_E_SHAPE; }
    if (start_pos < 0 || start_pos + T > cfg_.max_seq_len) { err_ = "score: sequence exceeds context"; return NTK_E_SHAPE; }
    if (slot < 0 || slot >= sequences_) { err_ = "score: no such sequence slot"; return NTK_E_SHAPE; }
    const int H = cfg_.hidden_size, V = cfg_.vocab_size;
    for (int i = 0; i < T; ++i) {
        if (tokens[i] < 0 || tokens[i] >= V) { err_ = "score: token id out of range"; return NTK_E_SHAPE; }
        if (targets[i] >= V) { err_ = "score: target id out of range"; return NTK_E_SHAPE; }
    }
    NT_TRY(score_buffers());
    void* s = stream_;
    tp_call_ = 0;
    NT_TRY(ntk_memcpy_h2d_async(tokens_dev_, tokens, (size_t)T * 4, s));
    NT_TRY(ntk_memcpy_h2d_async(score_targets_, targets, (size_t)T * 4, s));
    const int est = ntk_embed_rows(hidden_, token_embd_.ptr, tokens_dev_, T, H, token_embd_.dtype, s);
    if (est == NTK_E_DTYPE) fprintf(stderr, "Error: Unsupported embedding dtype: %s\n", dtype_name(token_embd_.dtype));
    else if (est != NTK_OK) return est;
    std::vector<int> pos(T);
    for (int i = 0; i < T; ++i) pos[i] = start_pos + i;
    NT_TRY(ntk_memcpy_h2d_async(positions_, pos.data(), (size_t)T * 4, s));
    NT_TRY(ntk_stream_synchronize(s));

    const KvTarget kv{slot, nullptr, 0};
    int rc = layers_1to1(T, start_pos, 0, cfg_.n_layers, kv);
    auto ok = [&](int st) { if (st != NTK_OK && rc == NTK_OK) rc = st; };
    const float* rm = lm_head_f16() && row_max_ && prefill_row_max_ ? row_max_ : nullptr;
    if (rm) ok(ntk_rmsnorm_rowmax(residual_, hidden_, (const float*)output_norm_.ptr, T, H, cfg_.norm_eps, row_max_, nullptr, s));
    else ok(ntk_rmsnorm(residual_, hidden_, (const float*)output_norm_.ptr, T, H, cfg_.norm_eps, s));
    for (int t0 = 0; t0 < T && rc == NTK_OK; t0 += score_rows_) {
        const int n = std::min(score_rows_, T - t0);
        ok(lm_head(score_logits_, residual_ + (size_t)t0 * H, n, rm ? rm + t0 : nullptr));
        ok(ntk_logprob_rows(score_logits_, n, V, V, score_targets_ + t0, score_logprob_ + t0, top1_out ? score_top1_ + t0 : nullptr, s));
    }
    if (rc == NTK_OK) ok(ntk_memcpy_d2h_async(logprob_out, score_logprob_, (size_t)T * 4, s));
    if (rc == NTK_OK && top1_out) ok(ntk_memcpy_d2h_async(top1_out, score_top1_, (size_t)T * 4, s));
    ok(ntk_stream_synchronize(s));
    if (raw_err_ != NTK_OK) { rc = raw_err_; raw_err_ = NTK_OK; }
    if (rc != NTK_OK && (err_.empty() || rc != NTK_E_LAUNCH)) err_ = std::string("score failed: ") + ntk_status_string(rc);
    return rc;
}

int Model::batch_buffers() {
    const size_t V = (size_t)cfg_.vocab_size, N = kMaxSequences;
    auto need = [&](auto*& p, size_t bytes) {
        if (p) return true;
        void* d = nt_hip_malloc(bytes + 256);
        if (!d) return false;
        allocs_.push_back(d);
        nt_hip_memset(d, 0, bytes);
        p = static_cast<std::remove_reference_t<decltype(p)>>(d);
        return true;
    };
    if (!need(batch_in_, 3 * N * 4) || !need(batch_logprob_, N * 4) || !need(batch_next_, N * 4) ||
        !need(batch_attn_scratch_, N * ntk_attention_split_scratch_bytes(cfg_.n_heads, cfg_.head_dim, kMaxAttnSplits)) || !need(batch_logits_, N * V * 4)) {
        err_ = "decode_batch: no device memory for the batch buffers (16 x vocab floats of logits)";
        return NTK_E_NOMEM;
    }
    return lm_head_workspace("decode_batch");
}

int Model::validate_batch(const int* slots, const int* tokens, const int* positions, int B, int sequences, int max_seq, int vocab, std::string* why) {
    auto fail = [&](int rc, const char* msg) { if (why) *why = msg; return rc; };
    if (!slots || !tokens || !positions) return fail(NTK_E_NULL, "decode_batch: null argument");
    if (B < 1 || B > sequences || B > kMaxSequences) return fail(NTK_E_SHAPE, "decode_batch: the batch must hold 1 .. `sequences` rows");
    unsigned seen = 0;
    for (int b = 0; b < B; ++b) {
        if (slots[b] < 0 || slots[b] >= sequences || slots[b] >= kMaxSequences) return fail(NTK_E_SHAPE, "decode_batch: no such sequence slot");
        if (seen & (1u << slots[b])) return fail(NTK_E_SHAPE, "decode_batch: the same sequence slot twice in one batch");
        seen |= 1u << slots[b];
        if (positions[b] < 0 || positions[b] >= max_seq) return fail(NTK_E_SHAPE, "decode_batch: position outside the context");
        if (tokens[b] < 0 || tokens[b] >= vocab) return fail(NTK_E_SHAPE, "decode_batch: token id out of range");
    }
    return NTK_OK;
}

int Model::batch_logits(const int* slots, const int* tokens, const int* positions, int B) {
    const int H = cfg_.hidden_size, N = kMaxSequences;
    void* s = stream_;
    tp_call_ = 0;
    int* const host = batch_host_;
    KvTarget kv{0, slots, 0};
    for (int b = 0; b < N; ++b) {
        host[b] = b < B ? tokens[b] : 0;
        host[N + b] = b < B ? positions[b] : 0;
        host[2 * N + b] = -1;
        if (b < B) kv.max_pos = std::max(kv.max_pos, positions[b]);
    }
    NT_TRY(ntk_memcpy_h2d_async(batch_in_, host, sizeof batch_host_, s));
    const int est = ntk_embed_rows(hidden_, token_embd_.ptr, batch_in_, B, H, token_embd_.dtype, s);
    if (est == NTK_E_DTYPE) fprintf(stderr, "Error: Unsupported embedding dtype: %s\n", dtype_name(token_embd_.dtype));
    else if (est != NTK_OK) return est;

    int rc = layers_1to1(B, 0, 0, cfg_.n_layers, kv);
    auto ok = [&](int st) { if (st != NTK_OK && rc == NTK_OK) rc = st; };
    const float* rm = lm_head_f16() && row_max_ && prefill_row_max_ ? row_max_ : nullptr;
    if (rm) ok(ntk_rmsnorm_rowmax(residual_, hidden_, (const float*)output_norm_.ptr, B, H, cfg_.norm_eps, row_max_, nullptr, s));
    else ok(ntk_rmsnorm(residual_, hidden_, (const float*)output_norm_.ptr, B, H, cfg_.norm_eps, s));
    ok(lm_head(batch_logits_, residual_, B, rm));
    return rc;
}

int Model::decode_batch(const int* slots, const int* tokens, const int* positions, int B, float* logits_out, int* next_out) {
    NT_TRY(validate_batch(slots, tokens, positions, B, sequences_, cfg_.max_seq_len, cfg_.vocab_size, &err_));
    if ((kv_q8_ && !batch_kv_q8_) || tp_world_ > 1) { err_ = "decode_batch: not available with kv_cache=q8_0 or tensor parallelism"; return NTK_E_SHAPE; }
    NT_TRY(batch_buffers());
    const int V = cfg_.vocab_size, N = kMaxSequences;
    void* s = stream_;
    int rc = batch_logits(slots, tokens, positions, B);
    auto ok = [&](int st) { if (st != NTK_OK && rc == NTK_OK) rc = st; };
    if (next_out) ok(ntk_logprob_rows(batch_logits_, B, V, V, batch_in_ + 2 * N, batch_logprob_, batch_next_, s));
    if (rc == NTK_OK && logits_out) ok(ntk_memcpy_d2h_async(logits_out, batch_logits_, (size_t)B * V * 4, s));
    if (rc == NTK_OK && next_out) ok(ntk_memcpy_d2h_async(next_out, batch_next_, (size_t)B * 4, s));
    ok(ntk_stream_synchronize(s));
    if (raw_err_ != NTK_OK) { rc = raw_err_; raw_err_ = NTK_OK; }
    if (rc != NTK_OK && (err_.empty() || rc != NTK_E_LAUNCH)) err_ = std::string("decode_batch failed: ") + ntk_status_string(rc);
    return rc;
}

int Model::batch_sample_buffers() {
    const size_t N = kMaxSequences;
    auto need = [&](auto*& p, size_t bytes) {
        if (p) return true;
        void* d = nt_hip_malloc(bytes + 256);
        if (!d) return false;
        allocs_.push_back(d);
        p = static_cast<std::remove_reference_t<decltype(p)>>(d);
        return true;
    };
    if (!need(batch_recent_, N * kRecentCap * 4) || !need(batch_sample_scratch_, ntk_sample_rows_scratch_bytes((int)N, cfg_.vocab_size))) {
        err_ = "decode_batch_sample: no device memory for the rows' windows and the sampler's scratch";
        return NTK_E_NOMEM;
    }
    if (!h_batch_recent_) h_batch_recent_ = (int*)nt_hip_malloc_host(N * kRecentCap * 4);
    if (!h_batch_next_) h_batch_next_ = (int*)nt_hip_malloc_host(N * 4);
    if (!h_batch_recent_ || !h_batch_next_) { err_ = "decode_batch_sample: no pinned host memory for the windows and the sampled tokens"; return NTK_E_NOMEM; }
    return NTK_OK;
}

int Model::decode_batch_sample(const int* slots, const int* tokens, const int* positions, int B, const ntk_sample_rows& rows, const int* const* recent,
                               float* logits_out, float* const* row_logits, int* next_out) {
    NT_TRY(validate_batch(slots, tokens, positions, B, sequences_, cfg_.max_seq_len, cfg_.vocab_size, &err_));
    if ((kv_q8_ && !batch_kv_q8_) || tp_world_ > 1) { err_ = "decode_batch_sample: not available with kv_cache=q8_0 or tensor parallelism"; return NTK_E_SHAPE; }
    if (!next_out) { err_ = "decode_batch_sample: null argument"; return NTK_E_NULL; }
    const int V = cfg_.vocab_size;
    int pitch = 0;
    for (int b = 0; b < B; ++b) {
        if (V > 131072 || !device_sampler_supports(rows.temperature[b], rows.top_k[b], V)) {
            err_ = "decode_batch_sample: a row the device sampler does not take (temperature > 0 needs 0 < top_k <= 64, top_k < vocab <= 131072)";
            return NTK_E_SHAPE;
        }
        if (rows.n_recent[b] < 0 || rows.n_recent[b] > kMaxRecent) { err_ = "decode_batch_sample: a window of 0 .. 4096 tokens per row"; return NTK_E_SHAPE; }
        if (rows.repeat_penalty[b] > 1.0f && rows.n_recent[b] > 0) {
            if (!recent || !recent[b]) { err_ = "decode_batch_sample: null window"; return NTK_E_NULL; }
            pitch = std::max(pitch, rows.n_recent[b]);
        }
    }
    NT_TRY(batch_buffers());
    NT_TRY(batch_sample_buffers());
    void* s = stream_;
    ntk_sample_rows dev = rows;
    for (int b = 0; b < B; ++b) {
        if (rows.repeat_penalty[b] > 1.0f && rows.n_recent[b] > 0) memcpy(h_batch_recent_ + (size_t)b * pitch, recent[b], (size_t)rows.n_recent[b] * 4);
// ... 18 lines not shown
```

ntransformer_amd/csrc/gemv.hip:

```cpp
#include "gemv_core.hip.h"
#ifdef NTK_EXPERIMENTS
#include "ntk_experiments.h"
#endif
#include <algorithm>
#include <cmath>
#include <cstdio>
#include <cstdlib>

namespace ntk {

#ifdef NTK_EXPERIMENTS
#include "gemv_attfuse.hip.h"
#else
struct AttnFuse {};
#endif

enum { NS_ANY = 0, NS_ONE = 1, NS_SPLIT = 2 };
template <int DT, bool NORM, bool XFAST, bool A16, bool ATT = false, bool XI = false, bool LM = false, int NSF = NS_ANY>
__device__ __forceinline__ void gemv_quant_body(const GemvParams& p, const int bid, const int nblk, const AttnFuse* attp = nullptr) {
    using F = Fmt<DT>;
    static_assert(!LM || (DT == NTK_DT_Q8_0 && !A16 && !ATT && !XI), "lane-major rows: Q8_0");
    static_assert(NSF == NS_ANY || LM, "compile-time slice forms: the lane-major kernels");
    constexpr int NL = LM ? 4 : F::NL;
    constexpr int STAGE = LM ? 0 : NL * 1024 + 64;
    extern __shared__ __attribute__((aligned(16))) uint8_t smem[];
#ifdef NTK_GEMV_TRACE
    unsigned long long gv_t[GT_EV] = {0, 0, 0, 0, 0, 0, 0, 0, 0, 0, 0, 0, 0, 0};
#endif
    GV_STAMP(0);
#ifndef NTK_GEMV_NO_KARG_PREFETCH
    {
        const auto* ka = __builtin_amdgcn_kernarg_segment_ptr();
        unsigned d0, d1, d2, d3, d4;
        asm volatile("s_load_dword %0, %5, 0x0\n\ts_load_dword %1, %5, 0x40\n\ts_load_dword %2, %5, 0x80\n\ts_load_dword %3, %5, 0xc0\n\t"
                     "s_load_dword %4, %5, 0x100\n\ts_waitcnt lgkmcnt(0)"
                     : "=&s"(d0), "=&s"(d1), "=&s"(d2), "=&s"(d3), "=&s"(d4) : "s"(ka) : "memory");
        __builtin_amdgcn_sched_barrier(0);
    }
#endif

    const int tid = threadIdx.x;
    constexpr int XIT = 8, WIT = 4;
    u32x4 xv[XIT], wv[WIT];
    if constexpr (XFAST && !ATT) {
        const int step0 = (int)blockDim.x * 4;
#pragma unroll
        for (int i = 0; i < XIT; ++i) {
            xv[i] = u32x4{0u, 0u, 0u, 0u};
            if (i * step0 < p.in) xv[i] = *reinterpret_cast<const u32x4*>(p.x + min(tid * 4 + i * step0, p.in - 4));
        }
        if constexpr (NORM) {
#pragma unroll
            for (int i = 0; i < WIT; ++i) {
                wv[i] = u32x4{0u, 0u, 0u, 0u};
                if (i * step0 < p.in) wv[i] = *reinterpret_cast<const u32x4*>(p.norm_w + min(tid * 4 + i * step0, p.in - 4));
            }
        }
        GV_STAMP(7);
    }
    const int lane = tid & 63;
    const int wave = __builtin_amdgcn_readfirstlane(tid >> 6);
    const int ns = NSF == NS_ONE ? 1 : p.ns;
    const bool single = NSF == NS_ANY ? p.ns == 1 : NSF == NS_ONE;
    const int nwaves = ns * p.rw;
    const int s = wave % ns;
    const int g = wave / ns;
    constexpr bool norm = NORM;

    const size_t image_bytes = (size_t)std::min(ns, 4) * 64 * XPITCH * 4;
    const size_t stage0 = single ? image_bytes : 0;
    const size_t regionA = single ? image_bytes + (size_t)nwaves * STAGE : std::max((size_t)nwaves * STAGE, image_bytes);
    float* part = reinterpret_cast<float*>(smem + regionA);
    float* red = part + 2 * p.rw * ns * RB;
    const size_t lds_floats_total = regionA / 4 + (size_t)(2 * p.rw * ns * RB + 16 + 16);

    uint8_t* stage = smem + stage0 + (size_t)wave * STAGE;
    const int my_len = min(p.slice_cols, p.in - s * p.slice_cols);
    const int ncols = min(64, max(0, my_len - 64 * lane));
    const unsigned slice_byte0 = (unsigned)((size_t)s * p.slice_cols / F::BW * F::BB);
    const unsigned slice_bytes = (unsigned)(my_len / F::BW * F::BB);
    const int group = bid * p.rw + g;
    const int ngroups = nblk * p.rw;
    const int mats = p.silu_pair ? 2 : 1;
    const int n_my = (p.total_rows > group) ? ((p.total_rows - 1 - group) / ngroups + 1) * mats : 0;

    static_assert(MAX_SEG == 3, "locate / seg_y: unrolled for three segments");
    const int seg_rows0 = p.seg[0].rows, seg_rows1 = p.seg[1].rows;
    float* const seg_y0 = p.seg[0].y;
    float* const seg_y1 = p.seg[1].y;
    float* const seg_y2 = p.seg[2].y;
    auto locate = [&](int q, int& seg, int& row) {
        int r = group + (q >> (mats - 1)) * ngroups;
        if (p.silu_pair) { seg = q & 1; row = r; return; }
        seg = 0;
        if (p.nseg > 1 && r >= seg_rows0) {
            r -= seg_rows0; seg = 1;
            if (p.nseg > 2 && r >= seg_rows1) { r -= seg_rows1; seg = 2; }
        }
        row = r;
    };
    auto seg_y = [&](int seg) { return seg == 0 ? seg_y0 : seg == 1 ? seg_y1 : seg_y2; };
    int cu_seg = 0, cu_row = group, cu_rows = p.silu_pair ? 0x7fffffff : p.seg[0].rows;
    auto cursor_normalise = [&]() {
        while (cu_seg + 1 < p.nseg && cu_row >= cu_rows) { cu_row -= cu_rows; ++cu_seg; cu_rows = p.seg[cu_seg].rows; }
    };
    if (!p.silu_pair) cursor_normalise();
    auto cursor_advance = [&]() {
        if (p.silu_pair) {
            if (cu_seg == 0) { cu_seg = 1; } else { cu_seg = 0; cu_row += ngroups; }
        } else {
            cu_row += ngroups;
            cursor_normalise();
        }
    };

    u32x4 pf[NL], pf2[LM ? NL : 1];
    uint32_t pf_sc = 0u, pf2_sc = 0u;
    const int lm_nl = my_len >> 6, lm_lane = min(lane, max(lm_nl - 1, 0));
    unsigned pre_off[NL];
    if constexpr (A16) {
        const unsigned last0 = (slice_bytes - 1u) & ~15u;
#pragma unroll
        for (int j = 0; j < NL; ++j) pre_off[j] = min(16u * (unsigned)(lane + 64 * j), last0);
    }
    int pf_seg = 0, pf_row = 0, pf_shift = 0;
    float pf_res = 0.0f;
    auto issue = [&]() {
        pf_seg = cu_seg; pf_row = cu_row;
        if (p.resid != nullptr && single) {
            int idx = cu_row;
            asm volatile("" : "+v"(idx));
            pf_res = p.resid[idx];
        }
        if constexpr (LM) return;
        const unsigned rel = (unsigned)p.seg[cu_seg].delta + (unsigned)cu_row * p.row_bytes + slice_byte0;
        pf_shift = (int)(rel & 15u);
        const unsigned nbytes = (rel & 15u) + slice_bytes;
        const unsigned last = (nbytes - 1u) & ~15u;
        const uint8_t* a = p.seg[cu_seg].W + (rel & ~15u);
#pragma unroll
        for (int j = 0; j < NL; ++j) {
            unsigned off;
            if constexpr (A16) off = pre_off[j]; else off = min(16u * (unsigned)(lane + 64 * j), last);
            pf[j] = __builtin_nontemporal_load(reinterpret_cast<const u32x4*>(a + off));
        }
    };
    auto issue_lm = [&](u32x4 (&c)[NL], uint32_t& sc) {
        const uint8_t* a = p.seg[cu_seg].W + ((unsigned)cu_row * p.row_bytes + slice_byte0);
#pragma unroll
        for (int j = 0; j < NL; ++j)
            c[j] = __builtin_nontemporal_load(reinterpret_cast<const u32x4*>(a + 16u * (unsigned)(j * lm_nl + lm_lane)));
        sc = __builtin_nontemporal_load(reinterpret_cast<const uint32_t*>(a + 64u * (unsigned)lm_nl + 4u * (unsigned)lm_lane));
    };
    auto issue_first = [&]() { issue(); if constexpr (LM) issue_lm(pf, pf_sc); };
    if (n_my <= 0) { cu_seg = 0; cu_row = 0; }

    f32x2 x2[32];
    XInt xi;
    static_assert(!XI || (XFAST && !ATT && ((DT == NTK_DT_Q4_K && A16) || DT == NTK_DT_Q6_K)), "integer activations: fast prologue, Q4_K (aligned rows) / Q6_K");
    {
        float* ximg = reinterpret_cast<float*>(smem);
        constexpr int GS = 4;
        auto img_index = [&](int c, int g0) {
            if (single) return (c >> 6) * XPITCH + (c & 63);
            const int sp = c / p.slice_cols, cc = c - sp * p.slice_cols;
            return ((sp - g0) * 64 + (cc >> 6)) * XPITCH + (cc & 63);
        };
        const int step = (int)blockDim.x * 4;
        const int dummy = (int)(lds_floats_total - 16);
        const bool have_lo = ncols > 0, have_hi = ncols > 32;
        auto read_own_row = [&](int g0) {
            const float* xrow = ximg + ((s - g0) * 64 + lane) * XPITCH;
            const float* xr0 = xrow, *xr1 = xrow + 32;
            if constexpr (DT == NTK_DT_Q6_K) {
                xr0 = ximg + ((s - g0) * 64 + (lane & ~1)) * XPITCH + 32 * (lane & 1);
                xr1 = xr0 + XPITCH;
            }
#pragma unroll
            for (int j = 0; j < 64; j += 4) {
                const float4 v = *reinterpret_cast<const float4*>((j < 32 ? xr0 : xr1 - 32) + j);
                const bool have = j < 32 ? have_lo : have_hi;
                x2[j / 2] = f32x2{have ? v.x : 0.0f, have ? v.y : 0.0f};
                x2[j / 2 + 1] = f32x2{have ? v.z : 0.0f, have ? v.w : 0.0f};
            }
        };
        if constexpr (XFAST) {
            if constexpr (ATT) {
#ifdef NTK_EXPERIMENTS
                issue_first();
                att_wait(*attp);
#pragma unroll
                for (int i = 0; i < XIT; ++i) xv[i] = asm_load16_sc1(p.x, 4u * (unsigned)min(tid * 4 + i * step, p.in - 4));
                asm volatile("s_waitcnt vmcnt(0)" : "+v"(xv[0]), "+v"(xv[1]), "+v"(xv[2]), "+v"(xv[3]), "+v"(xv[4]), "+v"(xv[5]), "+v"(xv[6]), "+v"(xv[7]));
#endif
            } else {
#ifndef NTK_GEMV_NO_XWAIT
            asm volatile("" : "+v"(xv[0]), "+v"(xv[1]), "+v"(xv[2]), "+v"(xv[3]), "+v"(xv[4]), "+v"(xv[5]), "+v"(xv[6]), "+v"(xv[7]));
            if constexpr (NORM) asm volatile("" : "+v"(wv[0]), "+v"(wv[1]), "+v"(wv[2]), "+v"(wv[3]));
#endif
            issue_first();
            GV_STAMP(8);
            }
            __builtin_amdgcn_sched_barrier(0);
            GV_STAMP(1);
            float rms_inv = 1.0f;
            if constexpr (NORM) {
                float ssq = 0.0f;
#pragma unroll
                for (int i = 0; i < WIT; ++i) {
                    const float m = (tid * 4 + i * step < p.in) ? 1.0f : 0.0f;
                    const float x0 = __uint_as_float(xv[i].x), x1 = __uint_as_float(xv[i].y), x2_ = __uint_as_float(xv[i].z), x3 = __uint_as_float(xv[i].w);
                    ssq = fmaf(x0 * m, x0, ssq); ssq = fmaf(x1 * m, x1, ssq); ssq = fmaf(x2_ * m, x2_, ssq); ssq = fmaf(x3 * m, x3, ssq);
                }
                ssq = wave_sum(ssq);
                if (lane == 0) red[wave] = ssq;
                __syncthreads();
                float tot = 0.0f;
                for (int w = 0; w < nwaves; ++w) tot += red[w];
                rms_inv = 1.0f / sqrtf(tot / (float)p.in + p.eps);
#pragma unroll
                for (int i = 0; i < WIT; ++i) {
                    xv[i].x = __float_as_uint(__uint_as_float(xv[i].x) * rms_inv * __uint_as_float(wv[i].x));
                    xv[i].y = __float_as_uint(__uint_as_float(xv[i].y) * rms_inv * __uint_as_float(wv[i].y));
                    xv[i].z = __float_as_uint(__uint_as_float(xv[i].z) * rms_inv * __uint_as_float(wv[i].z));
                    xv[i].w = __float_as_uint(__uint_as_float(xv[i].w) * rms_inv * __uint_as_float(wv[i].w));
                }
            }
            if constexpr (XI) {
                uint8_t* dimg = smem;
                auto xi_store = [&](const u32x4 q, const int sp, const int cc, const bool live) {
                    const float v0 = live ? __uint_as_float(q.x) : 0.0f, v1 = live ? __uint_as_float(q.y) : 0.0f,
                                v2 = live ? __uint_as_float(q.z) : 0.0f, v3 = live ? __uint_as_float(q.w) : 0.0f;
                    float am = fmaxf(fmaxf(fabsf(v0), fabsf(v1)), fmaxf(fabsf(v2), fabsf(v3)));
                    am = fmaxf(am, dpp_or_self<DPP_QUAD_1032, 0xF>(am));
                    am = fmaxf(am, dpp_or_self<DPP_QUAD_2301, 0xF>(am));
                    am = fmaxf(am, dpp_or_self<DPP_ROW_HALF_MIRROR, 0xF>(am));
                    float sm = (v0 + v1) + (v2 + v3);
                    sm += dpp_or_zero<DPP_QUAD_1032, 0xF>(sm);
                    sm += dpp_or_zero<DPP_QUAD_2301, 0xF>(sm);
                    const int e = am > 0.0f ? __builtin_amdgcn_frexp_expf(am) : 0;
                    const float up = __builtin_ldexpf(1.0f, 22 - e), inv = __builtin_ldexpf(1.0f, e - 22);
                    const uint32_t x0 = __float_as_uint(fmaf(v0, up, 12582912.0f)) - 0x4B400000u, x1 = __float_as_uint(fmaf(v1, up, 12582912.0f)) - 0x4B400000u,
                                   x2i = __float_as_uint(fmaf(v2, up, 12582912.0f)) - 0x4B400000u, x3 = __float_as_uint(fmaf(v3, up, 12582912.0f)) - 0x4B400000u;
                    const uint32_t ta = __builtin_amdgcn_perm(x1, x0, 0x05010400u);
                    const uint32_t tb = __builtin_amdgcn_perm(x1, x0, 0x07030602u);
                    const uint32_t tc = __builtin_amdgcn_perm(x3, x2i, 0x05010400u);
                    const uint32_t td = __builtin_amdgcn_perm(x3, x2i, 0x07030602u);
                    const uint32_t p0 = __builtin_amdgcn_perm(tc, ta, 0x05040100u);
                    const uint32_t p1 = __builtin_amdgcn_perm(tc, ta, 0x07060302u);
                    const uint32_t p2 = __builtin_amdgcn_perm(td, tb, 0x05040100u);
                    if (live) {
                        uint8_t* row = dimg + (size_t)(sp * 64 + (cc >> 6)) * (XPITCH * 4);
                        *reinterpret_cast<uint32_t*>(row + (cc & 63)) = p0;
                        *reinterpret_cast<uint32_t*>(row + 64 + (cc & 63)) = p1;
                        *reinterpret_cast<uint32_t*>(row + 128 + (cc & 63)) = p2;
                        float* meta = reinterpret_cast<float*>(row + 192);
                        if ((cc & 31) == 0) meta[(cc >> 5) & 1] = inv;
                        if ((cc & 15) == 0) meta[2 + ((cc >> 4) & 3)] = sm;
                    }
                };
                auto xi_read = [&](const int g0) {
                    const bool have_lo_ = ncols > 0, have_hi_ = ncols > 32;
                    const uint8_t* rowA = dimg + (size_t)((s - g0) * 64 + lane) * (XPITCH * 4);
                    const uint8_t* rowB = rowA;
                    int offA = 0, offB = 32;
                    if constexpr (DT == NTK_DT_Q6_K) {
                        rowA = dimg + (size_t)((s - g0) * 64 + (lane & ~1)) * (XPITCH * 4);
                        rowB = rowA + XPITCH * 4;
                        offA = offB = 32 * (lane & 1);
                    }
#pragma unroll
                    for (int pl = 0; pl < 3; ++pl)
#pragma unroll
                        for (int k4 = 0; k4 < 4; ++k4) {
                            const uint8_t* src = (k4 < 2 ? rowA + offA : rowB + offB) + 64 * pl + 16 * (k4 & 1);
                            const u32x4 v = *reinterpret_cast<const u32x4*>(src);
                            const bool have = k4 < 2 ? have_lo_ : have_hi_;
                            xi.d[pl][4 * k4] = have ? v.x : 0u; xi.d[pl][4 * k4 + 1] = have ? v.y : 0u;
                            xi.d[pl][4 * k4 + 2] = have ? v.z : 0u; xi.d[pl][4 * k4 + 3] = have ? v.w : 0u;
                        }
                    const float* mA = reinterpret_cast<const float*>(rowA + 192);
                    const float* mB = reinterpret_cast<const float*>(rowB + 192);
                    xi.inv[0] = have_lo_ ? mA[offA >> 5] : 0.0f;
                    xi.inv[1] = have_hi_ ? mB[offB >> 5] : 0.0f;
                    xi.sx[0] = have_lo_ ? mA[2 + (offA >> 4)] : 0.0f; xi.sx[1] = have_lo_ ? mA[3 + (offA >> 4)] : 0.0f;
                    xi.sx[2] = have_hi_ ? mB[2 + (offB >> 4)] : 0.0f; xi.sx[3] = have_hi_ ? mB[3 + (offB >> 4)] : 0.0f;
                };
                int isp = 0, icc = tid * 4;
#pragma unroll
                for (int i = 0; i < XIT; ++i) {
                    if (i * step >= p.in) continue;
                    xi_store(xv[i], isp, icc, tid * 4 + i * step < p.in);
                    icc += step;
                    if (icc >= p.slice_cols) { icc -= p.slice_cols; ++isp; }
                }
                __syncthreads();
                xi_read(0);
            } else
            {
                const int cend = min(p.in, GS * p.slice_cols);
                int isp = 0, icc = tid * 4;
#pragma unroll
                for (int i = 0; i < XIT; ++i) {
                    if (i * step >= cend) continue;
                    const int c = tid * 4 + i * step;
                    *reinterpret_cast<u32x4*>(ximg + (c < cend ? (isp * 64 + (icc >> 6)) * XPITCH + (icc & 63) : dummy)) = xv[i];
                    icc += step;
                    if (icc >= p.slice_cols) { icc -= p.slice_cols; ++isp; }
                }
                for (int c = XIT * step + tid * 4; c < cend; c += step)
                    *reinterpret_cast<float4*>(ximg + img_index(c, 0)) = *reinterpret_cast<const float4*>(p.x + c);
                GV_STAMP(9);
                __syncthreads();
                GV_STAMP(10);
                if (s < GS) read_own_row(0);
#ifdef NTK_GEMV_TRACE
                asm volatile("s_waitcnt lgkmcnt(0)" ::: "memory");
                GV_STAMP(11);
#endif
            }
            if constexpr (!XI)
            for (int g0 = GS; g0 < ns; g0 += GS) {
                const int cbeg = g0 * p.slice_cols, cend = min(p.in, (g0 + GS) * p.slice_cols);
                __syncthreads();
                for (int c = cbeg + tid * 4; c < cend; c += step)
                    *reinterpret_cast<float4*>(ximg + img_index(c, g0)) = *reinterpret_cast<const float4*>(p.x + c);
                __syncthreads();
                if (s >= g0 && s < g0 + GS) read_own_row(g0);
            }
        } else {
            issue_first();
            float rms_inv = 1.0f;
            if (NORM && !(kAblate & 1)) {
                float ssq = 0.0f;
                for (int c = tid; c < p.in; c += blockDim.x) ssq = fmaf(p.x[c], p.x[c], ssq);
                ssq = wave_sum(ssq);
                if (lane == 0) red[wave] = ssq;
                __syncthreads();
                float tot = 0.0f;
                for (int w = 0; w < nwaves; ++w) tot += red[w];
                rms_inv = 1.0f / sqrtf(tot / (float)p.in + p.eps);
            }
            for (int g0 = 0; g0 < ns; g0 += GS) {
                const int cbeg = g0 * p.slice_cols, cend = min(p.in, (g0 + GS) * p.slice_cols);
                if (g0 > 0) __syncthreads();
                if (!(kAblate & 1)) {
                    for (int c = cbeg + tid; c < cend; c += blockDim.x)
                        ximg[img_index(c, g0)] = NORM ? p.x[c] * rms_inv * p.norm_w[c] : p.x[c];
                }
                __syncthreads();
                if (s >= g0 && s < g0 + GS) read_own_row(g0);
            }
        }
        if ((kAblate & 1) || XI) {
#pragma unroll
            for (int j = 0; j < 32; ++j) x2[j] = f32x2{1.0f, 1.0f};
        }
        if (!single && !LM) __syncthreads();
        GV_STAMP(2);
    }
    float sx16[4], sx32[2];
#pragma unroll
    for (int r = 0; r < 4; ++r) {
        float t = 0.0f;
#pragma unroll
        for (int j = 0; j < 8; ++j) t += x2[8 * r + j].x + x2[8 * r + j].y;
        sx16[r] = t;
    }
    sx32[0] = sx16[0] + sx16[1];
    sx32[1] = sx16[2] + sx16[3];
    if constexpr (DT == NTK_DT_Q4_K) {
#pragma unroll
        for (int j = 16; j < 32; ++j) x2[j] *= 0.0625f;
    }
    if constexpr (DT == NTK_DT_Q4_0) {
#pragma unroll
        for (int j = 0; j < 32; ++j) if ((j & 8) != 0) x2[j] *= 0.0625f;
    }
    float gate_carry = 0.0f;
    float pair_g = 0.0f, pair_u = 0.0f;
    auto silu_flush = [&](const int last_pair) {
        const int base = last_pair & ~63;
        if (lane <= last_pair - base) {
            const int row = group + (base + lane) * ngroups;
            p.seg[0].y[row] = pair_g / (1.0f + expf(-pair_g)) * pair_u;
        }
    };

    float res_pf = 0.0f;
    auto prefetch_resid = [&](int b) {
        if (p.resid == nullptr || s != 0 || lane >= RB || b * RB + lane >= n_my) return;
        int seg, row;
        locate(b * RB + lane, seg, row);
        res_pf = p.resid[row];
    };
    if (!single) prefetch_resid(0);
    auto combine = [&](int b, int cnt) {
        if (s != 0) return;
        const float* pg = part + (size_t)(b & 1) * p.rw * ns * RB + (size_t)(g * ns) * RB;
        float t = 0.0f;
        if (lane < cnt)
            for (int ss = 0; ss < ns; ++ss) t += pg[ss * RB + lane];
        const float nxt = __shfl_down(t, 1, 64);
        if (lane < cnt) {
            int seg, row;
            locate(b * RB + lane, seg, row);
            if (p.silu_pair) {
                if ((lane & 1) == 0) seg_y0[row] = t / (1.0f + expf(-t)) * nxt;
            } else {
                float v = t;
                if (p.resid != nullptr && seg == 0) v = res_pf + v;
                seg_y(seg)[row] = v;
            }
        }
        prefetch_resid(b + 1);
    };

    auto row_step = [&](const int q, u32x4 (&cur)[NL], uint32_t& cur_sc, u32x4 (&nxt)[LM ? NL : 1], uint32_t& nxt_sc) __attribute__((always_inline)) {
        const int seg = pf_seg, row = pf_row, shift = A16 ? 0 : pf_shift;
        const float res = pf_res;
        float acc;
        if constexpr (LM) {
            asm volatile("" : "+v"(cur[0]), "+v"(cur[1]), "+v"(cur[2]), "+v"(cur[3]), "+v"(cur_sc));
#ifdef NTK_GEMV_TRACE
            if (q == 0) GV_STAMP(3);
            if (q == n_my - 1) GV_STAMP(5);
#endif
            if (q + 1 < n_my) { cursor_advance(); issue(); issue_lm(nxt, nxt_sc); }
            __builtin_amdgcn_sched_barrier(0);
            acc = dot_q8_regs(cur, cur_sc, ncols, x2);
        } else {
#pragma unroll
            for (int j = 0; j < NL; ++j) {
                if (kAblate & 4) { asm volatile("" ::"v"(pf[j])); continue; }
                *reinterpret_cast<u32x4*>(stage + 16 * (lane + 64 * j)) = pf[j];
            }
            __builtin_amdgcn_wave_barrier();
#ifdef NTK_GEMV_TRACE
            if (q == 0) GV_STAMP(3);
            if (q == n_my - 1) GV_STAMP(5);
#endif
            if (q + 1 < n_my) { cursor_advance(); issue(); }
            if constexpr (XI && DT == NTK_DT_Q6_K) acc = DotI<DT>::run(stage, shift, lane, ncols, xi);
            else if constexpr (XI) acc = DotI<DT>::run(stage, lane, ncols, xi);
            else acc = (kAblate & 2) ? x2[0].x + (float)q : Dot<DT, A16>::run(stage, shift, lane, ncols, x2, sx16, sx32);
            __builtin_amdgcn_wave_barrier();
        }
        const float tot = wave_sum_lane63(acc);
#ifdef NTK_GEMV_TRACE
        if (q == 0) { asm volatile("" :: "v"(tot)); GV_STAMP(4); }
#endif

        if (single) {
            if (p.silu_pair) {
                const float t63 = __int_as_float(__builtin_amdgcn_readlane(__float_as_int(tot), 63));
                const int pi = (q >> 1) & 63;
                if ((q & 1) == 0) { if (lane == pi) pair_g = t63; }
                else {
                    if (lane == pi) pair_u = t63;
                    if (pi == 63 || q == n_my - 1) silu_flush(q >> 1);
                }
            } else if (lane == 63) {
                float v = tot;
                if (p.resid != nullptr && seg == 0) v = res + v;
                p.seg[seg].y[row] = v;
            }
        } else {
            const int b = q / RB, i = q % RB;
            if (lane == 63) part[(size_t)(b & 1) * p.rw * ns * RB + (size_t)(g * ns + s) * RB + i] = tot;
            if (i == RB - 1) {
                __syncthreads();
                combine(b, RB);
            }
        }
    };
    for (int q = 0; q < n_my; ++q) {
        row_step(q, pf, pf_sc, pf2, pf2_sc);
        if constexpr (LM) { if (++q < n_my) row_step(q, pf2, pf2_sc, pf, pf_sc); }
    }
    if (!single) {
        int done = n_my / RB;
        if (n_my % RB) {
            __syncthreads();
            combine(done, n_my % RB);
            ++done;
        }
        for (; done < p.nbatch; ++done) __syncthreads();
    }
#ifdef NTK_EXPERIMENTS
    if constexpr (ATT) att_finish(*attp, nblk);
#endif
#ifdef NTK_GEMV_TRACE
    GV_STAMP(6);
    if (tid == 0 && bid < GT_WG) {
        gv_t[13] = (unsigned long long)n_my;
        for (int e = 0; e < GT_EV; ++e) g_gemv_trace[p.trace_slot & (GT_SLOTS - 1)][bid][e] = gv_t[e];
    }
#endif
}

template <bool NORM, bool XFAST, int NSF>
__global__ __launch_bounds__(512, Fmt<NTK_DT_Q8_0>::MINW) void gemv_q8l_kernel(const GemvParams p) {
    gemv_quant_body<NTK_DT_Q8_0, NORM, XFAST, false, false, false, true, NSF>(p, (int)blockIdx.x, (int)gridDim.x);
}
template <bool UNPACK>
__global__ __launch_bounds__(256) void q8l_pack_kernel(uint8_t* __restrict__ dst, const uint8_t* __restrict__ src, const int rows, const int in,
                                                       const int slice_cols) {
    const int lanes_row = in >> 6;
    const size_t t = (size_t)blockIdx.x * blockDim.x + threadIdx.x;
    if (t >= (size_t)rows * lanes_row) return;
    const int row = (int)(t / lanes_row), gl = (int)(t % lanes_row);
    const int lanes_slice = slice_cols >> 6, sl = gl / lanes_slice, l = gl - sl * lanes_slice;
    const int nl = min(lanes_slice, lanes_row - sl * lanes_slice);
    const size_t row0 = (size_t)row * lanes_row * 68;
    uint32_t* file = reinterpret_cast<uint32_t*>(const_cast<uint8_t*>(UNPACK ? dst : src) + row0 + (size_t)gl * 68);
    uint8_t* slice = const_cast<uint8_t*>(UNPACK ? src : dst) + row0 + (size_t)sl * lanes_slice * 68;
    uint32_t w[17], q[16], sc;
    if constexpr (!UNPACK) {
#pragma unroll
        for (int k = 0; k < 17; ++k) w[k] = file[k];
#pragma unroll
        for (int k = 0; k < 8; ++k) { q[k] = (w[k] >> 16) | (w[k + 1] << 16); q[8 + k] = w[9 + k]; }
        sc = (w[0] & 0xFFFFu) | (w[8] & 0xFFFF0000u);
#pragma unroll
        for (int j = 0; j < 4; ++j) *reinterpret_cast<u32x4*>(slice + (size_t)(j * nl + l) * 16) = u32x4{q[4 * j], q[4 * j + 1], q[4 * j + 2], q[4 * j + 3]};
        *reinterpret_cast<uint32_t*>(slice + (size_t)64 * nl + 4 * l) = sc;
    } else {
#pragma unroll
        for (int j = 0; j < 4; ++j) {
            const u32x4 v = *reinterpret_cast<const u32x4*>(slice + (size_t)(j * nl + l) * 16);
            q[4 * j] = v.x; q[4 * j + 1] = v.y; q[4 * j + 2] = v.z; q[4 * j + 3] = v.w;
        }
        sc = *reinterpret_cast<const uint32_t*>(slice + (size_t)64 * nl + 4 * l);
        w[0] = (sc & 0xFFFFu) | (q[0] << 16);
#pragma unroll
        for (int k = 1; k < 8; ++k) w[k] = (q[k - 1] >> 16) | (q[k] << 16);
        w[8] = (q[7] >> 16) | (sc & 0xFFFF0000u);
#pragma unroll
        for (int k = 0; k < 8; ++k) w[9 + k] = q[8 + k];
#pragma unroll
        for (int k = 0; k < 17; ++k) file[k] = w[k];
    }
}

#ifdef NTK_EXPERIMENTS
template <int DT>
__global__ __launch_bounds__(512, Fmt<DT>::MINW) void gemv_quant_att_kernel(const GemvParams p, const AttnFuse att) {
    extern __shared__ __attribute__((aligned(16))) uint8_t att_smem[];
    const int nh = att.n_heads;
    if ((int)blockIdx.x < nh) {
        att_produce(att, reinterpret_cast<float*>(att_smem), (int)blockIdx.x);
        return;
    }
    gemv_quant_body<DT, false, true, A16_OK<DT>, true>(p, (int)blockIdx.x - nh, (int)gridDim.x - nh, &att);
}
#endif

template <int DT, bool NORM, bool XFAST, bool A16>
__global__ __launch_bounds__(512, Fmt<DT>::MINW) void gemv_quant_kernel(const GemvParams p) {
    gemv_quant_body<DT, NORM, XFAST, A16>(p, (int)blockIdx.x, (int)gridDim.x);
}
template <int DT, bool NORM>
__global__ __launch_bounds__(512, Fmt<DT>::MINW) void gemv_quant_xi_kernel(const GemvParams p) {
    gemv_quant_body<DT, NORM, true, A16_OK<DT>, false, true>(p, (int)blockIdx.x, (int)gridDim.x);
}
template <int DTA, int DTB, bool NORM>
__global__ __launch_bounds__(512, 4) void gemv_quant_pair_kernel(const GemvParams pa, const GemvParams pb, const int split) {
    if ((int)blockIdx.x < split) gemv_quant_body<DTA, NORM, true, A16_OK<DTA>>(pa, (int)blockIdx.x, split);
    else gemv_quant_body<DTB, NORM, true, A16_OK<DTB>>(pb, (int)blockIdx.x - split, (int)gridDim.x - split);
}

#ifdef NTK_EXPERIMENTS
#include "gemv_colsplit.hip.h"
#endif

template <typename T, bool ADD>
__global__ __launch_bounds__(256) void gemv_dense_kernel(float* __restrict__ y, const T* __restrict__ W,
                                                         const float* __restrict__ x, int out, int in) {
    const int lane = threadIdx.x & 63;
    const int wave = blockIdx.x * (blockDim.x >> 6) + (threadIdx.x >> 6);
    const int nwaves = gridDim.x * (blockDim.x >> 6);
    constexpr int V = 16 / (int)sizeof(T);
    for (int r = wave; r < out; r += nwaves) {
        const T* w = W + (size_t)r * in;
        float acc = 0.0f;
        int done = 0;
// ... 5 lines not shown
                    const float4 xv = *reinterpret_cast<const float4*>(x + 4 * i);
                    acc = fmaf(__uint_as_float(raw.x), xv.x, acc); acc = fmaf(__uint_as_float(raw.y), xv.y, acc);
                    acc = fmaf(__uint_as_float(raw.z), xv.z, acc); acc = fmaf(__uint_as_float(raw.w), xv.w, acc);
                } else {
                    const float4 x0 = *reinterpret_cast<const float4*>(x + 8 * i);
                    const float4 x1 = *reinterpret_cast<const float4*>(x + 8 * i + 4);
                    acc = fmaf(h2f((uint16_t)(raw.x & 0xFFFF)), x0.x, acc); acc = fmaf(h2f((uint16_t)(raw.x >> 16)), x0.y, acc);
                    acc = fmaf(h2f((uint16_t)(raw.y & 0xFFFF)), x0.z, acc); acc = fmaf(h2f((uint16_t)(raw.y >> 16)), x0.w, acc);
                    acc = fmaf(h2f((uint16_t)(raw.z & 0xFFFF)), x1.x, acc); acc = fmaf(h2f((uint16_t)(raw.z >> 16)), x1.y, acc);
                    acc = fmaf(h2f((uint16_t)(raw.w & 0xFFFF)), x1.z, acc); acc = fmaf(h2f((uint16_t)(raw.w >> 16)), x1.w, acc);
                }
            }
            done = nv * V;
        }
        for (int i = done + lane; i < in; i += 64) {
            float wv;
            if constexpr (sizeof(T) == 4) wv = (float)w[i]; else wv = h2f((uint16_t)w[i]);
            acc = fmaf(wv, x[i], acc);
        }
        acc = wave_sum(acc);
        if (lane == 0) y[r] = ADD ? y[r] + acc : acc;
    }
}

static bool is_quant(int dt) {
    return dt == NTK_DT_Q8_0 || dt == NTK_DT_Q4_0 || dt == NTK_DT_Q4_K || dt == NTK_DT_Q5_K || dt == NTK_DT_Q6_K;
}

struct GemvLaunch {
    GemvParams p;
    int grid, nwaves;
    size_t lds;
    bool xfast, a16;
};

static bool raise_lds_limit(const void* fn) {
    return hipFuncSetAttribute(fn, hipFuncAttributeMaxDynamicSharedMemorySize, 160 * 1024) == hipSuccess;
}

template <int DT>
static int prepare_quant(const ntk_gemv_seg* segs, int nseg, const float* x, int in, const float* norm_w, float eps,
                         const float* resid, int silu_pair, int max_wg, GemvLaunch& L, bool lm = false) {
    using F = Fmt<DT>;
    if (in <= 0 || in % F::BW != 0) return NTK_E_SHAPE;
    GemvParams& p = L.p;
    p = GemvParams{};
    long total = 0;
    const size_t row_bytes = (size_t)in / F::BW * F::BB;
    for (int i = 0; i < nseg; ++i) {
        if (segs[i].rows < 0) return NTK_E_SHAPE;
        if (segs[i].rows > 0 && (!segs[i].W || !segs[i].y)) return NTK_E_NULL;
        if ((size_t)segs[i].rows * row_bytes > 0xFFFFFFF0ull) return NTK_E_SHAPE;
        const uintptr_t w = reinterpret_cast<uintptr_t>(segs[i].W);
        if (w & 1) return NTK_E_ALIGN;
        p.seg[i].W = reinterpret_cast<const uint8_t*>(w & ~(uintptr_t)15);
        p.seg[i].delta = (int)(w & 15);
        p.seg[i].y = segs[i].y;
        p.seg[i].rows = segs[i].rows;
        total += segs[i].rows;
    }
    if (silu_pair) {
        if (nseg != 2 || segs[0].rows != segs[1].rows || resid) return NTK_E_SHAPE;
        total = segs[0].rows;
    }
    p.nseg = nseg;
    p.total_rows = (int)total;
    p.x = x;
    p.in = in;
    if (!gemv_slices(in, F::BW == 256 ? 256 : 64, p.ns, p.slice_cols)) return NTK_E_SHAPE;
    static const int env_waves = std::max(1, NTK_TUNE_ENV_INT("NTK_GEMV_WAVES", 8));
    p.rw = std::max(1, env_waves / p.ns);
    L.nwaves = p.ns * p.rw;
    p.x_vec = ((reinterpret_cast<uintptr_t>(x) & 15) == 0 &&
               (!norm_w || (reinterpret_cast<uintptr_t>(norm_w) & 15) == 0) && (p.slice_cols % 4 == 0)) ? 1 : 0;
    p.norm_w = norm_w;
    p.eps = eps;
    p.resid = resid;
    p.silu_pair = silu_pair;
    p.row_bytes = (unsigned)row_bytes;
    const int mats = silu_pair ? 2 : 1;
    int grid = (int)std::min<long>((total + p.rw - 1) / p.rw, max_wg);
    grid = std::max(grid, 1);
    L.grid = grid;
    const long ngroups = (long)grid * p.rw;
    const long rows_per_group = (total + ngroups - 1) / ngroups;
    p.nbatch = (int)((rows_per_group * mats + RB - 1) / RB);
    const int STAGE = lm ? 0 : F::NL * 1024 + 64;
    const size_t image_bytes = (size_t)std::min(p.ns, 4) * 64 * XPITCH * 4;
    const size_t regionA = p.ns == 1 ? image_bytes + (size_t)L.nwaves * STAGE : std::max((size_t)L.nwaves * STAGE, image_bytes);
    L.lds = regionA + (size_t)(2 * p.rw * p.ns * RB + 16 + 16) * sizeof(float);
    L.xfast = p.x_vec && (in % 4 == 0) && in >= 4 && !(kAblate & 1) && (!norm_w || in <= 4 * 4 * 64 * L.nwaves) &&
              (p.ns == 1 || 4 * 64 * L.nwaves <= p.slice_cols);
    bool a16 = (DT == NTK_DT_Q4_K || DT == NTK_DT_Q5_K);
    for (int i = 0; i < nseg; ++i) a16 = a16 && p.seg[i].delta == 0;
    L.a16 = a16;
    return NTK_OK;
}

constexpr size_t kXiMinBytes = (size_t)48 << 20;
enum { XI_DEFAULT = -1, XI_NEVER = 0, XI_ALWAYS = 1 };

static int max_workgroups() {
    static const int max_wg = std::max(1, NTK_TUNE_ENV_INT("NTK_GEMV_MAX_WG", 512));
    return max_wg;
}

template <int DT>
static int launch_quant(const ntk_gemv_seg* segs, int nseg, const float* x, int in, const float* norm_w, float eps,
                        const float* resid, int silu_pair, hipStream_t st, int xi_mode = XI_DEFAULT) {
    GemvLaunch L;
    const int rc = prepare_quant<DT>(segs, nseg, x, in, norm_w, eps, resid, silu_pair, max_workgroups(), L);
    if (rc != NTK_OK) return rc;
    if (L.p.total_rows == 0) return NTK_OK;
    using KernelFn = void (*)(const GemvParams);
    static const KernelFn table[2][2][2] = {
        {{gemv_quant_kernel<DT, false, false, false>, gemv_quant_kernel<DT, false, false, A16_OK<DT>>},
         {gemv_quant_kernel<DT, false, true, false>, gemv_quant_kernel<DT, false, true, A16_OK<DT>>}},
        {{gemv_quant_kernel<DT, true, false, false>, gemv_quant_kernel<DT, true, false, A16_OK<DT>>},
         {gemv_quant_kernel<DT, true, true, false>, gemv_quant_kernel<DT, true, true, A16_OK<DT>>}}};
    if (L.lds > 64 * 1024) {
        static bool once = [] {
            bool ok = true;
            for (int a = 0; a < 2; ++a)
                for (int b = 0; b < 2; ++b)
                    for (int c = 0; c < 2; ++c)
                        ok = ok && hipFuncSetAttribute((const void*)table[a][b][c], hipFuncAttributeMaxDynamicSharedMemorySize,
                                                       160 * 1024) == hipSuccess;
            return ok;
        }();
        if (!once || L.lds > 160 * 1024) return NTK_E_SHAPE;
    }
#ifdef NTK_EXPERIMENTS
    if constexpr (DT == NTK_DT_Q8_0) {
        static const int cs_mode = NTK_TUNE_ENV_INT("NTK_GEMV_COLSPLIT", 0);
        bool cs = cs_mode != 0 && in == CS_COLS && L.xfast && !(kAblate & 7);
        for (int i = 0; i < nseg && cs; ++i) cs = L.p.seg[i].delta == 0;
        if (cs) {
            const int total = L.p.total_rows, mats = silu_pair ? 2 : 1;
            const int cgrid = std::min(total, max_workgroups());
            const size_t items = (size_t)((total + cgrid - 1) / cgrid) * mats;
            const size_t clds = (size_t)8 * CS_RBT * CS_STRIPE + items * 8 * sizeof(float) + 64;
            using CFn = void (*)(const GemvParams);
            static const CFn ct[2] = {gemv_q8_colsplit_kernel<false>, gemv_q8_colsplit_kernel<true>};
            static const bool ok = raise_lds_limit((const void*)ct[0]) && raise_lds_limit((const void*)ct[1]);
            if (ok && clds <= 150 * 1024) {
                hipLaunchKernelGGL(ct[norm_w ? 1 : 0], dim3(cgrid), dim3(512), clds, st, L.p);
                return last_launch_status();
            }
        }
    }
#endif
    const dim3 g(L.grid), b(64 * L.nwaves);
#ifdef NTK_GEMV_TRACE
    static int trace_counter = 0;
    L.p.trace_slot = trace_counter++;
#endif
    if constexpr (DT == NTK_DT_Q4_K || DT == NTK_DT_Q6_K) {
        const size_t launch_bytes = (size_t)L.p.total_rows * (silu_pair ? 2 : 1) * L.p.row_bytes;
        const bool want = xi_mode == XI_ALWAYS || (xi_mode == XI_DEFAULT && launch_bytes >= kXiMinBytes);
        if (want && L.xfast && (L.a16 || DT == NTK_DT_Q6_K) && L.p.ns <= 2 && in <= 8 * 4 * 64 * L.nwaves) {
            using XFn = void (*)(const GemvParams);
            static const XFn xt[2] = {gemv_quant_xi_kernel<DT, false>, gemv_quant_xi_kernel<DT, true>};
            if (L.lds > 64 * 1024) {
                static bool once2 = hipFuncSetAttribute((const void*)xt[0], hipFuncAttributeMaxDynamicSharedMemorySize, 160 * 1024) == hipSuccess &&
                                    hipFuncSetAttribute((const void*)xt[1], hipFuncAttributeMaxDynamicSharedMemorySize, 160 * 1024) == hipSuccess;
                if (!once2) return NTK_E_SHAPE;
            }
            hipLaunchKernelGGL(xt[norm_w ? 1 : 0], g, b, L.lds, st, L.p);
            return last_launch_status();
        }
    }
    hipLaunchKernelGGL(table[norm_w ? 1 : 0][L.xfast ? 1 : 0][L.a16 ? 1 : 0], g, b, L.lds, st, L.p);
    return last_launch_status();
}

static size_t q8l_bytes(int rows, int in) {
    int ns, sc;
    return rows > 0 && q8l_layout(in, ns, sc) ? (size_t)rows * (size_t)(in / 32 * 34) : 0;
}

static int q8l_pack(void* dst, const void* raw, int rows, int in, bool unpack, hipStream_t st) {
    int ns, sc;
    if (rows <= 0 || !q8l_layout(in, ns, sc)) return NTK_E_SHAPE;
    if ((reinterpret_cast<uintptr_t>(unpack ? raw : dst) & 15) || (reinterpret_cast<uintptr_t>(unpack ? dst : raw) & 3)) return NTK_E_ALIGN;
    const size_t n = (size_t)rows * (in / 64);
    if ((n + 255) / 256 > 0x7FFFFFFFull) return NTK_E_SHAPE;
    const dim3 g((unsigned)((n + 255) / 256)), b(256);
    uint8_t* d = static_cast<uint8_t*>(dst);
    const uint8_t* r = static_cast<const uint8_t*>(raw);
    if (unpack) hipLaunchKernelGGL(q8l_pack_kernel<true>, g, b, 0, st, d, r, rows, in, sc);
    else hipLaunchKernelGGL(q8l_pack_kernel<false>, g, b, 0, st, d, r, rows, in, sc);
    return last_launch_status();
}

int q8l_gemv_fused(const ntk_gemv_seg* segs, int nseg, const float* x, int in, const float* norm_w, float eps, const float* resid,
                   int silu_pair, hipStream_t st) {
    int ns, sc;
    if (!q8l_layout(in, ns, sc)) return NTK_E_SHAPE;
    for (int i = 0; i < nseg; ++i)
        if (reinterpret_cast<uintptr_t>(segs[i].W) & 15) return NTK_E_ALIGN;
    GemvLaunch L;
    const int rc = prepare_quant<NTK_DT_Q8_0>(segs, nseg, x, in, norm_w, eps, resid, silu_pair, max_workgroups(), L, true);
    if (rc != NTK_OK) return rc;
    if (L.p.total_rows == 0) return NTK_OK;
    using KernelFn = void (*)(const GemvParams);
#define Q8L_FORMS(NORM, XFAST) {gemv_q8l_kernel<NORM, XFAST, NS_ONE>, gemv_q8l_kernel<NORM, XFAST, NS_SPLIT>}
    static const KernelFn table[2][2][2] = {{Q8L_FORMS(false, false), Q8L_FORMS(false, true)}, {Q8L_FORMS(true, false), Q8L_FORMS(true, true)}};
#undef Q8L_FORMS
    if (L.lds > 64 * 1024) {
        static const bool once = [] {
            bool ok = true;
            for (int a = 0; a < 2; ++a)
                for (int b = 0; b < 2; ++b)
                    for (int c = 0; c < 2; ++c) ok = ok && raise_lds_limit((const void*)table[a][b][c]);
            return ok;
        }();
        if (!once || L.lds > 160 * 1024) return NTK_E_SHAPE;
    }
#ifdef NTK_GEMV_TRACE
    static int trace_counter = 0;
    L.p.trace_slot = trace_counter++;
#endif
    hipLaunchKernelGGL(table[norm_w ? 1 : 0][L.xfast ? 1 : 0][L.p.ns == 1 ? 0 : 1], dim3(L.grid), dim3(64 * L.nwaves), L.lds, st, L.p);
    return last_launch_status();
}

#ifdef NTK_EXPERIMENTS
template <int DT>
static int launch_att(const AttnFuse& att, const ntk_gemv_seg* seg, int in, const float* resid, hipStream_t st) {
    GemvLaunch L;
    const int rc = prepare_quant<DT>(seg, 1, att.out, in, nullptr, 0.0f, resid, 0, max_workgroups(), L);
    if (rc != NTK_OK) return rc;
    if (!L.xfast || L.nwaves != 8 || L.p.seg[0].delta != 0 || L.p.total_rows == 0 || L.grid < 1) return NTK_E_ALIGN;
    const size_t att_lds = sizeof(float) * ((size_t)3 * att.hd + 16 + (size_t)8 * att.hd);
    if (att_lds > L.lds) return NTK_E_SHAPE;
    if (L.lds > 64 * 1024) {
        static bool once = hipFuncSetAttribute((const void*)gemv_quant_att_kernel<DT>, hipFuncAttributeMaxDynamicSharedMemorySize, 160 * 1024) == hipSuccess;
        if (!once || L.lds > 160 * 1024) return NTK_E_SHAPE;
    }
    hipLaunchKernelGGL(gemv_quant_att_kernel<DT>, dim3(L.grid + att.n_heads), dim3(64 * L.nwaves), L.lds, st, L.p, att);
    return last_launch_status();
}
#endif

template <int DTA, int DTB>
static int launch_pair(const ntk_gemv_seg* sa, int na, const ntk_gemv_seg* sb, int nb, const float* x, int in, const float* norm_w,
                       float eps, hipStream_t st) {
    const double ba = (double)Fmt<DTA>::BB / Fmt<DTA>::BW, bb = (double)Fmt<DTB>::BB / Fmt<DTB>::BW;
    long ra = 0, rb = 0;
    for (int i = 0; i < na; ++i) ra += sa[i].rows;
    for (int i = 0; i < nb; ++i) rb += sb[i].rows;
    if (ra <= 0 || rb <= 0) return NTK_E_SHAPE;
    const int total_wg = max_workgroups();
    int wa = (int)(total_wg * (ra * ba) / (ra * ba + rb * bb) + 0.5);
    wa = std::min(std::max(wa, 1), total_wg - 1);
    GemvLaunch A, B;
    int rc = prepare_quant<DTA>(sa, na, x, in, norm_w, eps, nullptr, 0, wa, A);
    if (rc == NTK_OK) rc = prepare_quant<DTB>(sb, nb, x, in, norm_w, eps, nullptr, 0, total_wg - wa, B);
    if (rc != NTK_OK) return rc;
    if (!A.xfast || !B.xfast || A.nwaves != B.nwaves || A.a16 != A16_OK<DTA> || B.a16 != A16_OK<DTB>) return NTK_E_ALIGN;
    for (int i = 0; i < na; ++i) if (A.p.seg[i].delta != 0 && A16_OK<DTA>) return NTK_E_ALIGN;
    using PairFn = void (*)(const GemvParams, const GemvParams, int);
    const size_t lds = std::max(A.lds, B.lds);
    static const PairFn table[2] = {gemv_quant_pair_kernel<DTA, DTB, false>, gemv_quant_pair_kernel<DTA, DTB, true>};
    if (lds > 64 * 1024) {
        static bool once = hipFuncSetAttribute((const void*)table[0], hipFuncAttributeMaxDynamicSharedMemorySize, 160 * 1024) == hipSuccess &&
                           hipFuncSetAttribute((const void*)table[1], hipFuncAttributeMaxDynamicSharedMemorySize, 160 * 1024) == hipSuccess;
        if (!once || lds > 160 * 1024) return NTK_E_SHAPE;
    }
    hipLaunchKernelGGL(table[norm_w ? 1 : 0], dim3(A.grid + B.grid), dim3(64 * A.nwaves), lds, st, A.p, B.p, A.grid);
    return last_launch_status();
}

static int dispatch_quant(int dt, const ntk_gemv_seg* segs, int nseg, const float* x, int in, const float* norm_w,
                          float eps, const float* resid, int silu_pair, hipStream_t st, int xi_mode = XI_DEFAULT) {
    switch (dt) {
        case NTK_DT_Q8_0: return launch_quant<NTK_DT_Q8_0>(segs, nseg, x, in, norm_w, eps, resid, silu_pair, st);
        case NTK_DT_Q4_0: return launch_quant<NTK_DT_Q4_0>(segs, nseg, x, in, norm_w, eps, resid, silu_pair, st);
        case NTK_DT_Q4_K: return launch_quant<NTK_DT_Q4_K>(segs, nseg, x, in, norm_w, eps, resid, silu_pair, st, xi_mode);
        case NTK_DT_Q5_K: return launch_quant<NTK_DT_Q5_K>(segs, nseg, x, in, norm_w, eps, resid, silu_pair, st);
        case NTK_DT_Q6_K: return launch_quant<NTK_DT_Q6_K>(segs, nseg, x, in, norm_w, eps, resid, silu_pair, st, xi_mode);
        default: return NTK_E_DTYPE;
    }
}

template <bool ADD>
static int launch_dense(float* y, const void* W, const float* x, int out, int in, int dt, hipStream_t st) {
    if (out == 0) return NTK_OK;
    const int grid = std::min((out + 3) / 4, 2048);
    if (dt == NTK_DT_F32)
        hipLaunchKernelGGL((gemv_dense_kernel<float, ADD>), dim3(grid), dim3(256), 0, st, y, (const float*)W, x, out, in);
    else
        hipLaunchKernelGGL((gemv_dense_kernel<uint16_t, ADD>), dim3(grid), dim3(256), 0, st, y, (const uint16_t*)W, x, out, in);
    return last_launch_status();
}

}

extern "C" {

#ifdef NTK_GEMV_TRACE
NTK_EXTRA_API int ntk_debug_gemv_trace(unsigned long long* out, size_t n) {
    return hipMemcpyFromSymbol(out, HIP_SYMBOL(ntk::g_gemv_trace), n * sizeof(unsigned long long)) == hipSuccess ? 0 : -3;
}
#endif

size_t ntk_q8l_bytes(int rows, int in_features) { return ntk::q8l_bytes(rows, in_features); }
int ntk_q8l_pack(void* dst, const void* raw, int rows, int in_features, void* stream) {
    if (!dst || !raw) return NTK_E_NULL;
    return ntk::q8l_pack(dst, raw, rows, in_features, false, ntk::resolve_stream(stream));
}
int ntk_q8l_unpack(void* raw, const void* packed, int rows, int in_features, void* stream) {
    if (!raw || !packed) return NTK_E_NULL;
    return ntk::q8l_pack(raw, packed, rows, in_features, true, ntk::resolve_stream(stream));
}

int ntk_gemv(float* y, const void* W, const float* x, int out_features, int in_features, int weight_dtype, void* stream) {
    if (!y || !W || !x) return NTK_E_NULL;
    if (out_features < 0 || in_features <= 0) return NTK_E_SHAPE;
    hipStream_t st = ntk::resolve_stream(stream);
    if (weight_dtype == NTK_DT_F32 || weight_dtype == NTK_DT_F16)
        return ntk::launch_dense<false>(y, W, x, out_features, in_features, weight_dtype, st);
    if (!ntk::is_quant(weight_dtype)) return NTK_E_DTYPE;
    ntk_gemv_seg seg{W, y, out_features, weight_dtype};
    return ntk::dispatch_quant(weight_dtype, &seg, 1, x, in_features, nullptr, 0.0f, nullptr, 0, st);
}

int ntk_gemv_add(float* y, const void* W, const float* x, int out_features, int in_features, int weight_dtype, void* stream) {
    if (!y || !W || !x) return NTK_E_NULL;
    if (out_features < 0 || in_features <= 0) return NTK_E_SHAPE;
    if (weight_dtype != NTK_DT_F16) return NTK_E_DTYPE;
    return ntk::launch_dense<true>(y, W, x, out_features, in_features, weight_dtype, ntk::resolve_stream(stream));
}

#ifdef NTK_EXPERIMENTS
int ntk_attention_gemv_fused(float* attn_out, const float* q, const float* k, const float* v, void* k_cache, void* v_cache,
                             const int* d_pos, const float* inv_freq, int n_heads, int n_kv_heads, int head_dim, int max_seq,
                             float scale, float theta_base, float freq_scale, const ntk_gemv_seg* wo, const float* resid,
                             unsigned* sync3, void* stream) {
    if (!attn_out || !q || !k || !v || !k_cache || !v_cache || !d_pos || !wo || !wo->W || !wo->y || !sync3) return NTK_E_NULL;
    if (n_heads <= 0 || n_kv_heads <= 0 || n_heads % n_kv_heads != 0 || max_seq <= 0) return NTK_E_SHAPE;
    if (head_dim != 64 && head_dim != 128 && head_dim != 256) return NTK_E_SHAPE;
    if ((reinterpret_cast<uintptr_t>(k_cache) & 15) || (reinterpret_cast<uintptr_t>(v_cache) & 15)) return NTK_E_ALIGN;
    ntk::AttnFuse a{};
    a.q = q; a.k = k; a.v = v; a.out = attn_out;
    a.kc = static_cast<uint16_t*>(k_cache); a.vc = static_cast<uint16_t*>(v_cache);
    a.d_pos = d_pos; a.inv_freq = inv_freq; a.sync = sync3;
    a.n_heads = n_heads; a.n_kv_heads = n_kv_heads; a.hd = head_dim; a.max_seq = max_seq;
    a.scale = scale; a.theta = theta_base; a.fscale = freq_scale;
    const int in = n_heads * head_dim;
    hipStream_t st = ntk::resolve_stream(stream);
    switch (wo->dtype) {
        case NTK_DT_Q8_0: return ntk::launch_att<NTK_DT_Q8_0>(a, wo, in, resid, st);
        case NTK_DT_Q4_0: return ntk::launch_att<NTK_DT_Q4_0>(a, wo, in, resid, st);
        case NTK_DT_Q4_K: return ntk::launch_att<NTK_DT_Q4_K>(a, wo, in, resid, st);
        case NTK_DT_Q5_K: return ntk::launch_att<NTK_DT_Q5_K>(a, wo, in, resid, st);
        case NTK_DT_Q6_K: return ntk::launch_att<NTK_DT_Q6_K>(a, wo, in, resid, st);
        default: return NTK_E_DTYPE;
    }
}
#endif

static int gemv_fused_form(const ntk_gemv_seg* segs, int nseg, const float* x, int in_features, const float* norm_w, float eps,
                           const float* resid, int silu_pair, void* stream, int xi_mode) {
    if (!segs || !x) return NTK_E_NULL;
    if (nseg < 1 || nseg > ntk::MAX_SEG) return NTK_E_SHAPE;
    ntk_gemv_seg a[3], b[3];
    int na = 0, nb = 0;
    for (int i = 0; i < nseg; ++i) {
        if (!ntk::is_quant(segs[i].dtype)) return NTK_E_DTYPE;
        if (segs[i].dtype == segs[0].dtype) a[na++] = segs[i];
        else if (nb == 0 || segs[i].dtype == b[0].dtype) b[nb++] = segs[i];
        else return NTK_E_DTYPE;
    }
    hipStream_t st = ntk::resolve_stream(stream);
    if (nb == 0) return ntk::dispatch_quant(segs[0].dtype, segs, nseg, x, in_features, norm_w, eps, resid, silu_pair, st, xi_mode);
    if (resid || silu_pair) return NTK_E_DTYPE;
    const int da = a[0].dtype, db = b[0].dtype;
    if (da == NTK_DT_Q4_K && db == NTK_DT_Q6_K) return ntk::launch_pair<NTK_DT_Q4_K, NTK_DT_Q6_K>(a, na, b, nb, x, in_features, norm_w, eps, st);
    if (da == NTK_DT_Q6_K && db == NTK_DT_Q4_K) return ntk::launch_pair<NTK_DT_Q4_K, NTK_DT_Q6_K>(b, nb, a, na, x, in_features, norm_w, eps, st);
    if (da == NTK_DT_Q4_K && db == NTK_DT_Q5_K) return ntk::launch_pair<NTK_DT_Q4_K, NTK_DT_Q5_K>(a, na, b, nb, x, in_features, norm_w, eps, st);
    if (da == NTK_DT_Q5_K && db == NTK_DT_Q4_K) return ntk::launch_pair<NTK_DT_Q4_K, NTK_DT_Q5_K>(b, nb, a, na, x, in_features, norm_w, eps, st);
    return NTK_E_DTYPE;
}

int ntk_gemv_fused(const ntk_gemv_seg* segs, int nseg, const float* x, int in_features, const float* norm_w, float eps,
                   const float* resid, int silu_pair, void* stream) {
    return gemv_fused_form(segs, nseg, x, in_features, norm_w, eps, resid, silu_pair, stream, ntk::XI_DEFAULT);
}
int ntk_debug_gemv_fused_form(const ntk_gemv_seg* segs, int nseg, const float* x, int in_features, const float* norm_w, float eps,
                              const float* resid, int silu_pair, int integer_activations, void* stream) {
    if (integer_activations < -1 || integer_activations > 1) return NTK_E_SHAPE;
    return gemv_fused_form(segs, nseg, x, in_features, norm_w, eps, resid, silu_pair, stream, integer_activations);
}

}
```

ntransformer_amd/ops.py:

```python
from __future__ import annotations

import ctypes as C
from typing import Optional, Sequence

import numpy as np

from . import _lib
from ._lib import GemvSeg, check


class DeviceBuffer:

    def __init__(self, nbytes: int):
        self.nbytes = int(nbytes)
        self.ptr = _lib.lib().nt_hip_malloc(max(self.nbytes, 1))
        if not self.ptr:
            raise _lib.NtkError(-7, "hipMalloc(%d)" % nbytes)

    @classmethod
    def from_numpy(cls, a: np.ndarray) -> "DeviceBuffer":
        a = np.ascontiguousarray(a)
        b = cls(a.nbytes)
        if a.nbytes:
            _lib.lib().nt_hip_memcpy_h2d(b.ptr, a.ctypes.data_as(C.c_void_p), a.nbytes)
# ... 312 lines not shown
    scratch = DeviceBuffer(int(L.ntk_sample_scratch_bytes(C.c_int(n))))
    L.ntk_sample_top_k.argtypes = [C.c_void_p, C.c_int, C.c_void_p, C.c_int, C.c_float, C.c_float, C.c_int, C.c_float, C.c_float,
                                   C.c_void_p, C.c_void_p, C.c_void_p, C.c_void_p]
    st = L.ntk_sample_top_k(_p(logits), n, _p(recent), n_recent, repeat_penalty, temperature, top_k, top_p, r, _p(d_out), None,
                            _p(scratch), stream)
    synchronize()
    return st


def sample_rows_top_k(logits, n_rows, vocab, ld, recent, recent_ld, rows, d_out, stream=None, null=()):
    L = _lib.lib()
    if not isinstance(rows, _lib.SampleRows):
        sr = _lib.SampleRows()
        for b, (temperature, top_k, top_p, repeat_penalty, r, n_recent) in enumerate(rows):
            sr.temperature[b], sr.top_k[b], sr.top_p[b], sr.repeat_penalty[b], sr.r[b], sr.n_recent[b] = temperature, top_k, top_p, repeat_penalty, r, n_recent
        rows = sr
    scratch = DeviceBuffer(int(L.ntk_sample_rows_scratch_bytes(min(max(n_rows, 1), 16), min(max(vocab, 1), 1 << 20))))
    arg = lambda name, v: None if name in null else v
    st = L.ntk_sample_rows_top_k(arg("logits", _p(logits)), n_rows, vocab, ld, _p(recent), recent_ld, arg("rows", C.pointer(rows)), arg("d_out", _p(d_out)), None,
                                 arg("scratch", _p(scratch)), stream)
    synchronize()
    return st


def gemm_quant(Y, W, X, n_tokens, out_features, in_features, dtype, resid=None, stream=None):
    check(_lib.lib().ntk_gemm_quant(_p(Y), _p(W), _p(X), n_tokens, out_features, in_features, int(dtype), _p(resid),
                                    stream), "gemm_quant")


def attention_decode_fused(output, q, k, v, k_cache, v_cache, d_pos, n_heads, n_kv_heads, head_dim, max_seq, scale,
                           theta_base, freq_scale=1.0, inv_freq=None, stream=None):
    check(_lib.lib().ntk_attention_decode_fused(_p(output), _p(q), _p(k), _p(v), _p(k_cache), _p(v_cache), _p(d_pos),
                                                _p(inv_freq), n_heads, n_kv_heads, head_dim, max_seq, scale, theta_base,
                                                freq_scale, stream), "attention_decode_fused")


def attention_decode_split(output, q, k, v, k_cache, v_cache, d_pos, n_heads, n_kv_heads, head_dim, max_seq, scale,
                           theta_base, nsplit, freq_scale=1.0, inv_freq=None, stream=None):
    scratch = DeviceBuffer(int(_lib.lib().ntk_attention_split_scratch_bytes(n_heads, head_dim, nsplit)))
    check(_lib.lib().ntk_attention_decode_split(_p(output), _p(q), _p(k), _p(v), _p(k_cache), _p(v_cache), _p(d_pos),
                                                _p(inv_freq), n_heads, n_kv_heads, head_dim, max_seq, scale, theta_base,
                                                freq_scale, nsplit, _p(scratch), stream), "attention_decode_split")
    synchronize()
    return None


def attention_decode_split_merged(output, q, k, v, k_cache, v_cache, d_pos, n_heads, n_kv_heads, head_dim, max_seq, scale,
                                  theta_base, nsplit, freq_scale=1.0, inv_freq=None, stream=None, launches=1):
    scratch = DeviceBuffer(int(_lib.lib().ntk_attention_split_scratch_bytes(n_heads, head_dim, nsplit)))
    check(_lib.lib().ntk_attention_split_scratch_init(_p(scratch), n_heads, stream), "attention_split_scratch_init")
    for _ in range(launches):
        check(_lib.lib().ntk_attention_decode_split_merged(_p(output), _p(q), _p(k), _p(v), _p(k_cache), _p(v_cache), _p(d_pos),
                                                           _p(inv_freq), n_heads, n_kv_heads, head_dim, max_seq, scale, theta_base,
                                                           freq_scale, nsplit, _p(scratch), stream), "attention_decode_split_merged")
    synchronize()
    return None


def attention_decode_batch(output, q, k, v, k_caches, v_caches, positions, n_rows, n_heads, n_kv_heads, head_dim, max_seq, scale,
                           theta_base, nsplit=1, freq_scale=1.0, inv_freq=None, stream=None, table=True):
    L = _lib.lib()
    kv = _lib.KvBatch()
    for b, (kc, vc) in enumerate(zip(k_caches, v_caches)):
        kv.k[b], kv.v[b] = _p(kc), _p(vc)
    scratch = DeviceBuffer(max(n_rows, 1) * int(L.ntk_attention_split_scratch_bytes(n_heads, head_dim, nsplit)))
    check(L.ntk_attention_decode_batch(_p(output), _p(q), _p(k), _p(v), C.addressof(kv) if table else None, _p(positions), n_rows, _p(inv_freq),
                                       n_heads, n_kv_heads, head_dim, max_seq, scale, theta_base, freq_scale, nsplit, _p(scratch), stream),
          "attention_decode_batch")
    synchronize()
    return None


def embed_rows(out, table, tokens, n_tokens, hidden, dtype, stream=None, allow_unsupported=False):
    st = _lib.lib().ntk_embed_rows(_p(out), _p(table), _p(tokens), n_tokens, hidden, int(dtype), stream)
    if not (allow_unsupported and st == -1):
        check(st, "embed_rows")
    return st


def argmax(logits, n, d_out_token, scratch, h_mirror=None, stream=None):
    check(_lib.lib().ntk_argmax(_p(logits), n, _p(d_out_token), _p(h_mirror), _p(scratch), stream), "argmax")


def logprob_rows(logits, n_rows, vocab, ld, targets, logprob, top1=None, stream=None):
    check(_lib.lib().ntk_logprob_rows(_p(logits), n_rows, vocab, ld, _p(targets), _p(logprob), _p(top1), stream), "logprob_rows")


def advance_pos(d_pos, stream=None):
    check(_lib.lib().ntk_advance_pos(_p(d_pos), stream), "advance_pos")


def sclk_mhz(stream=None) -> float:
    import numpy as np
    b = DeviceBuffer.zeros(24)
    check(_lib.lib().ntk_debug_sclk(_p(b), stream), "sclk probe")
    synchronize(stream)
    v = b.numpy(np.uint64)
    return 100.0 * float(v[0]) / max(float(v[1]), 1.0)


class SclkSpan:

    def __enter__(self):
        L = _lib.lib()
        self.flag, self.out = DeviceBuffer.zeros(8), DeviceBuffer.zeros(24)
        self.mhz = None
        check(L.ntk_debug_sclk_begin(_p(self.flag), _p(self.out), L.ntk_stream(1)), "sclk begin")
        return self

    def __exit__(self, *exc):
        import numpy as np
        L = _lib.lib()
        check(L.ntk_debug_sclk_end(_p(self.flag), L.ntk_stream(2)), "sclk end")
        check(L.ntk_stream_synchronize(L.ntk_stream(2)), "sync")
        check(L.ntk_stream_synchronize(L.ntk_stream(1)), "sync")
        v = self.out.numpy(np.uint64)
        if v[1] > 0:
            self.mhz = 100.0 * float(v[0]) / float(v[1])
        return False
```

Before: 554.5 tokens/s.

## Fuse LM-head argmax into Q8 GEMV and fold embedding into greedy tail

Adds a Q8_0 lane-major GEMV variant that computes per-block argmax candidates while writing logits. A new greedy tail kernel reduces those candidates, advances the token and position, and writes the next token's embedding row into the hidden buffer. The decode graph then gets a 'primed' form that skips the separate embedding launch. This removes the separate argmax stage-1 pass over the logits and the embed kernel per token, at the cost of extra graph variants and state tracking to invalidate the primed hidden buffer. The launch planner also adjusts rows-per-wave to balance the lane-major grid.

```diff
diff --git a/include/ntk_engine.h b/include/ntk_engine.h
--- a/include/ntk_engine.h
+++ b/include/ntk_engine.h
@@ -151,6 +151,11 @@
 int ntk_argmax_advance(const float* logits, int n, int* d_out_token, int* h_mirror, unsigned long long* h_ring4, int* d_pos,
                        float* scratch, void* stream);
 
+int ntk_gemv_q8l_argmax(const ntk_gemv_seg* seg, const float* x, int in_features, const float* norm_w, float eps, float* scratch, int* n_pairs,
+                        void* stream);
+int ntk_greedy_tail(const float* scratch, int n_pairs, int* d_out_token, int* h_mirror, unsigned long long* h_ring4, int* d_pos, float* hidden_out,
+                    const void* table, int hidden, int dtype, void* stream);
+
 int ntk_debug_sclk(unsigned long long* d_out2, void* stream);
 int ntk_debug_sclk_begin(unsigned* d_flag, unsigned long long* d_out2, void* side_stream);
 int ntk_debug_sclk_end(unsigned* d_flag, void* other_stream);
diff --git a/ntransformer_amd/_lib.py b/ntransformer_amd/_lib.py
--- a/ntransformer_amd/_lib.py
+++ b/ntransformer_amd/_lib.py
@@ -134,6 +134,9 @@
         "ntk_sample_rows_scratch_bytes": (C.c_size_t, [i, i]),
         "ntk_sample_rows_top_k": (i, [vp, i, i, i, vp, i, C.POINTER(SampleRows), vp, vp, vp, vp]),
         "ntk_advance_pos": (i, [vp, vp]),
+        "ntk_argmax_advance": (i, [vp, i, vp, vp, vp, vp, vp, vp]),
+        "ntk_gemv_q8l_argmax": (i, [C.POINTER(GemvSeg), vp, i, vp, f, vp, C.POINTER(i), vp]),
+        "ntk_greedy_tail": (i, [vp, i, vp, vp, vp, vp, vp, vp, i, i, vp]),
         "ntk_debug_sclk": (i, [vp, vp]),
         "ntk_debug_sclk_begin": (i, [vp, vp, vp]),
         "ntk_debug_sclk_end": (i, [vp, vp]),
diff --git a/ntransformer_amd/csrc/common.hip.h b/ntransformer_amd/csrc/common.hip.h
--- a/ntransformer_amd/csrc/common.hip.h
+++ b/ntransformer_amd/csrc/common.hip.h
@@ -42,6 +42,10 @@
 #pragma clang fp contract(off)
     ra = a * c - b * s;
     rb = b * c + a * s;
+}
+
+__device__ __forceinline__ void amax_merge(float& v, int& i, float ov, int oi) {
+    if (ov > v || (ov == v && oi < i)) { v = ov; i = oi; }
 }
 
 template <int CTRL, int ROW_MASK>
diff --git a/ntransformer_amd/csrc/elementwise.hip b/ntransformer_amd/csrc/elementwise.hip
--- a/ntransformer_amd/csrc/elementwise.hip
+++ b/ntransformer_amd/csrc/elementwise.hip
@@ -124,9 +124,6 @@
     if (e < hidden) out[(size_t)blockIdx.x * hidden + e] = embed_elem(table, tok, hidden, dt, e);
 }
 
-__device__ __forceinline__ void amax_merge(float& v, int& i, float ov, int oi) {
-    if (ov > v || (ov == v && oi < i)) { v = ov; i = oi; }
-}
 __global__ __launch_bounds__(256) void argmax_stage1(const float* __restrict__ x, int n, float* __restrict__ sv, int* __restrict__ si) {
     __shared__ float rv[4];
     __shared__ int ri[4];
@@ -210,6 +207,33 @@
     }
 }
 
+__global__ __launch_bounds__(256) void greedy_tail_kernel(const float* __restrict__ sv, const int* __restrict__ si, int nblk, int* __restrict__ d_out,
+                                                          int* __restrict__ h_mirror, unsigned long long* __restrict__ h_ring, int* __restrict__ d_pos,
+                                                          float* __restrict__ out, const uint8_t* __restrict__ table, int hidden, int dt) {
+    __shared__ float rv[4];
+    __shared__ int ri[4];
+    float v = -FLT_MAX;
+    int idx = 0x7FFFFFFF;
+    for (int i = threadIdx.x; i < nblk; i += blockDim.x) amax_merge(v, idx, sv[i], si[i]);
+    for (int off = 32; off > 0; off >>= 1) amax_merge(v, idx, __shfl_xor(v, off, 64), __shfl_xor(idx, off, 64));
+    if ((threadIdx.x & 63) == 0) { rv[threadIdx.x >> 6] = v; ri[threadIdx.x >> 6] = idx; }
+    __syncthreads();
+    v = rv[0]; idx = ri[0];
+    for (int w = 1; w < 4; ++w) amax_merge(v, idx, rv[w], ri[w]);
+    if (idx == 0x7FFFFFFF) idx = 0;
+    if (blockIdx.x == 0 && threadIdx.x == 0) {
+        const int pos = *d_pos;
+        *d_out = idx;
+        if (h_mirror) *h_mirror = idx;
+        if (h_ring)
+            __hip_atomic_store(h_ring + (pos & 3), (unsigned long long)(unsigned)idx | ((unsigned long long)(unsigned)(pos + 1) << 32),
+                               __ATOMIC_RELEASE, __HIP_MEMORY_SCOPE_SYSTEM);
+        *d_pos = pos + 1;
+    }
+    const int e = blockIdx.x * blockDim.x + threadIdx.x;
+    if (e < hidden) out[e] = embed_elem(table, idx, hidden, dt, e);
+}
+
 static inline dim3 g1(int n) { return dim3((n + 255) / 256); }
 
 }
@@ -323,6 +347,19 @@
     hipLaunchKernelGGL(argmax_advance_stage2, dim3(1), dim3(256), 0, st, (const float*)sv, (const int*)si, nblk, d_out_token, h_mirror, h_ring4, d_pos);
     return last_launch_status();
 }
+int ntk_greedy_tail(const float* scratch, int n_pairs, int* d_out_token, int* h_mirror, unsigned long long* h_ring4, int* d_pos, float* hidden_out,
+                    const void* table, int hidden, int dtype, void* stream) {
+    if (!scratch || !d_out_token || !d_pos || !hidden_out || !table) return NTK_E_NULL;
+    if (n_pairs <= 0 || n_pairs > 1024 || hidden <= 0) return NTK_E_SHAPE;
+    hipLaunchKernelGGL(greedy_tail_kernel, g1(hidden), dim3(256), 0, resolve_stream(stream), scratch, reinterpret_cast<const int*>(scratch + 1024), n_pairs,
+                       d_out_token, h_mirror, h_ring4, d_pos, hidden_out, (const uint8_t*)table, hidden, dtype);
+    const int st = last_launch_status();
+    if (st != NTK_OK) return st;
+    switch (dtype) {
+        case NTK_DT_F32: case NTK_DT_F16: case NTK_DT_Q8_0: case NTK_DT_Q4_0: case NTK_DT_Q4_K: case NTK_DT_Q6_K: return NTK_OK;
+        default: return NTK_E_DTYPE;
+    }
+}
 int ntk_debug_sclk(unsigned long long* d_out2, void* stream) {
     if (!d_out2) return NTK_E_NULL;
     hipLaunchKernelGGL(sclk_probe_kernel, dim3(1), dim3(64), 0, resolve_stream(stream), d_out2);
diff --git a/ntransformer_amd/csrc/engine/model.cpp b/ntransformer_amd/csrc/engine/model.cpp
--- a/ntransformer_amd/csrc/engine/model.cpp
+++ b/ntransformer_amd/csrc/engine/model.cpp
@@ -6,12 +6,13 @@
 Model::~Model() { free_all(); }
 
 void Model::drop_graphs(int slot) {
-    for (auto& row : graphs_)
-        for (int k = 0; k <= kAttnRegimes; ++k) {
-            if (slot >= 0 && k != slot) continue;
-            if (row[k]) (void)hipGraphExecDestroy(reinterpret_cast<hipGraphExec_t>(row[k]));
-            row[k] = nullptr;
-        }
+    for (auto& form : graphs_)
+        for (auto& row : form)
+            for (int k = 0; k <= kAttnRegimes; ++k) {
+                if (slot >= 0 && k != slot) continue;
+                if (row[k]) (void)hipGraphExecDestroy(reinterpret_cast<hipGraphExec_t>(row[k]));
+                row[k] = nullptr;
+            }
 }
 
 void Model::free_all() {
@@ -43,6 +44,7 @@
     raw_scratch_ = nullptr; raw_scratch_bytes_ = raw_cursor_ = 0; raw_err_ = 0;
     repack_done_ = output_tied_ = false;
     host_pos_ = attn_regime_ = 0;
+    touch_token_state();
     k_cache_ = v_cache_ = nullptr;
     slot_k_.clear(); slot_v_.clear(); slot_k_q8_.clear(); slot_v_q8_.clear();
     batch_logits_ = batch_logprob_ = batch_attn_scratch_ = nullptr; batch_in_ = batch_next_ = batch_recent_ = nullptr; batch_sample_scratch_ = nullptr;
@@ -137,6 +139,7 @@
 int Model::set_device_token(int token) {
     if (token < 0 || token >= cfg_.vocab_size) { err_ = "token id out of range"; return NTK_E_SHAPE; }
     *h_token_ = token;
+    touch_token_state();
     return ntk_memcpy_h2d_async(d_token_, h_token_, 4, stream_);
 }
 int Model::set_device_pos(int pos) {
@@ -156,6 +159,7 @@
 int Model::sample_on_device(const int* recent, int n_recent, float repeat_penalty, float temperature, int top_k, float top_p, float r) {
     if (!sample_scratch_ || !d_recent_ || !h_recent_) return NTK_E_NOMEM;
     if (n_recent > kRecentCap) { recent += n_recent - kRecentCap; n_recent = kRecentCap; }
+    touch_token_state();
     void* s = stream_;
     if (repeat_penalty > 1.0f && n_recent > 0) {
         memcpy(h_recent_, recent, (size_t)n_recent * 4);
diff --git a/ntransformer_amd/csrc/engine/model.h b/ntransformer_amd/csrc/engine/model.h
--- a/ntransformer_amd/csrc/engine/model.h
+++ b/ntransformer_amd/csrc/engine/model.h
@@ -145,7 +145,7 @@
     void drop_graphs(int slot = -1);
     struct Views { float *q, *k, *v, *attn_out, *gate, *up; };
     Views views(int T) const;
-    int enqueue_token(bool greedy);
+    int enqueue_token(bool greedy, bool graph_form = false, bool primed = false);
     int enqueue_layers(int first, int last);
     int decode_project(const DevTensor* const* ws, float* const* ys, int n, const float* x, const DevTensor* norm, const float* resid, int kind,
                        int silu_pair = 0, bool timed = true);
@@ -234,7 +234,11 @@
     bool prof_coarse_ = false;
     std::vector<Timed>* prof_ = nullptr;
     static constexpr int kPersistentSlot = kAttnRegimes;
-    ihipGraphExec_t* graphs_[2][kAttnRegimes + 1] = {};
+    ihipGraphExec_t* graphs_[2][2][kAttnRegimes + 1] = {};
+    bool graph_primes_[2][kAttnRegimes + 1] = {};
+    bool hidden_primed_ = false;
+    bool tail_primes_ = false;
+    void touch_token_state() { hidden_primed_ = false; }
     int host_pos_ = 0;
     int attn_regime_ = 0;
     float* attn_scratch_ = nullptr;
diff --git a/ntransformer_amd/csrc/engine/model_debug.cpp b/ntransformer_amd/csrc/engine/model_debug.cpp
--- a/ntransformer_amd/csrc/engine/model_debug.cpp
+++ b/ntransformer_amd/csrc/engine/model_debug.cpp
@@ -9,6 +9,7 @@
     if (tp_world_ > 1) return NTK_E_SHAPE;
     const size_t bytes = (size_t)T * cfg_.hidden_size * 4;
     void* s = stream_;
+    touch_token_state();
     NT_TRY(ntk_memcpy_h2d_async(hidden_, hidden_in, bytes, s));
     int rc;
     if (mode == 0) {
diff --git a/ntransformer_amd/csrc/engine/model_decode.cpp b/ntransformer_amd/csrc/engine/model_decode.cpp
--- a/ntransformer_amd/csrc/engine/model_decode.cpp
+++ b/ntransformer_amd/csrc/engine/model_decode.cpp
@@ -20,14 +20,18 @@
     if (begin) prof_->push_back({cls, e, nullptr, 1, false}); else prof_->back().b = e;
 }
 
-int Model::enqueue_token(bool greedy) {
+int Model::enqueue_token(bool greedy, bool graph_form, bool primed) {
     const int H = cfg_.hidden_size;
     void* s = stream_;
     tp_call_ = 0;
-    prof_mark(2, true);
-    const int est = ntk_embed_rows(hidden_, token_embd_.ptr, d_token_, 1, H, token_embd_.dtype, s);
-    prof_mark(2, false);
-    if (est != NTK_OK && est != NTK_E_DTYPE) return est;
+    tail_primes_ = false;
+    if (!primed) {
+        prof_mark(2, true);
+        const int est = ntk_embed_rows(hidden_, token_embd_.ptr, d_token_, 1, H, token_embd_.dtype, s);
+        prof_mark(2, false);
+        if (est != NTK_OK && est != NTK_E_DTYPE) return est;
+    }
+    int n_pairs = 0;
     if (use_persistent_now()) {
         NT_TRY(launch_persistent());
     } else {
@@ -35,11 +39,24 @@
         const DevTensor* const w = &output_;
         const bool timed = is_quant(w->dtype);
         if (timed) prof_mark(0, true);
-        NT_TRY(decode_project(&w, &logits_, 1, hidden_, &output_norm_, nullptr, 16, 0, false));
+        int st = NTK_E_DTYPE;
+        if (graph_form && greedy && tp_world_ == 1 && repack_ && (rp_mask() & 16) && w->rp != nullptr && w->dtype == NTK_DT_Q8_0) {
+            const ntk_gemv_seg seg = {w->rp, logits_, (int)w->out_f, w->dtype};
+            st = ntk_gemv_q8l_argmax(&seg, hidden_, (int)w->in_f, (const float*)output_norm_.ptr, cfg_.norm_eps, argmax_scratch_, &n_pairs, s);
+            if (!not_taken(st)) NT_TRY(st);
+        }
+        if (not_taken(st)) {
+            n_pairs = 0;
+            NT_TRY(decode_project(&w, &logits_, 1, hidden_, &output_norm_, nullptr, 16, 0, false));
+        }
         if (timed) prof_mark(0, false);
     }
     prof_mark(2, true);
-    if (greedy) NT_TRY(ntk_argmax_advance(logits_, cfg_.vocab_size, d_token_, h_token_, h_ring_, d_pos_, argmax_scratch_, s));
+    if (greedy && n_pairs > 0) {
+        const int est = ntk_greedy_tail(argmax_scratch_, n_pairs, d_token_, h_token_, h_ring_, d_pos_, hidden_, token_embd_.ptr, H, token_embd_.dtype, s);
+        if (est != NTK_OK && est != NTK_E_DTYPE) return est;
+        tail_primes_ = true;
+    } else if (greedy) NT_TRY(ntk_argmax_advance(logits_, cfg_.vocab_size, d_token_, h_token_, h_ring_, d_pos_, argmax_scratch_, s));
     else NT_TRY(ntk_advance_pos(d_pos_, s));
     if (tp_world_ > 1) NT_TRY(ntk_tp_advance_epoch(tp_comm_, s));
     prof_mark(2, false);
@@ -165,15 +182,22 @@
 
 int Model::decode_step_fused(bool greedy, bool use_graph) {
     pick_attention_regime();
+    const bool primed = hidden_primed_ && greedy && use_graph && !use_persistent_now();
+    touch_token_state();
     if (!use_graph) return enqueue_token(greedy);
-    ihipGraphExec_t*& slot = graphs_[greedy ? 1 : 0][use_persistent_now() ? kPersistentSlot : attn_regime_];
+    const int k = use_persistent_now() ? kPersistentSlot : attn_regime_;
+    ihipGraphExec_t*& slot = graphs_[primed ? 1 : 0][greedy ? 1 : 0][k];
     hipStream_t st = static_cast<hipStream_t>(stream_);
     if (!slot) {
         hipGraphExec_t ex = nullptr;
-        NT_TRY(capture_graph(st, tp_world_ > 1 ? hipStreamCaptureModeRelaxed : hipStreamCaptureModeThreadLocal, [&] { return enqueue_token(greedy); }, &ex));
+        NT_TRY(capture_graph(st, tp_world_ > 1 ? hipStreamCaptureModeRelaxed : hipStreamCaptureModeThreadLocal,
+                             [&] { return enqueue_token(greedy, true, primed); }, &ex));
         slot = reinterpret_cast<ihipGraphExec_t*>(ex);
-    }
-    return hipGraphLaunch(reinterpret_cast<hipGraphExec_t>(slot), st) == hipSuccess ? NTK_OK : NTK_E_LAUNCH;
+        if (greedy) graph_primes_[primed ? 1 : 0][k] = tail_primes_;
+    }
+    if (hipGraphLaunch(reinterpret_cast<hipGraphExec_t>(slot), st) != hipSuccess) return NTK_E_LAUNCH;
+    hidden_primed_ = greedy && graph_primes_[primed ? 1 : 0][k];
+    return NTK_OK;
 }
 
 int Model::profile_token(float ms[4], int calls[4], bool coarse) {
@@ -181,6 +205,7 @@
     rec.reserve(1024);
     prof_ = &rec;
     prof_coarse_ = coarse;
+    touch_token_state();
     pick_attention_regime();
     int rc = enqueue_token(true);
     if (coarse && !rec.empty()) {
diff --git a/ntransformer_amd/csrc/engine/model_prompt.cpp b/ntransformer_amd/csrc/engine/model_prompt.cpp
--- a/ntransformer_amd/csrc/engine/model_prompt.cpp
+++ b/ntransformer_amd/csrc/engine/model_prompt.cpp
@@ -11,6 +11,7 @@
     const int H = cfg_.hidden_size;
     void* s = stream_;
     tp_call_ = 0;
+    touch_token_state();
     if (ntk_memcpy_h2d_async(tokens_dev_, tokens, (size_t)T * 4, s) != NTK_OK) return nullptr;
     const int est = ntk_embed_rows(hidden_, token_embd_.ptr, tokens_dev_, T, H, token_embd_.dtype, s);
     if (est == NTK_E_DTYPE) fprintf(stderr, "Error: Unsupported embedding dtype: %s\n", dtype_name(token_embd_.dtype));
@@ -369,6 +370,7 @@
     NT_TRY(score_buffers());
     void* s = stream_;
     tp_call_ = 0;
+    touch_token_state();
     NT_TRY(ntk_memcpy_h2d_async(tokens_dev_, tokens, (size_t)T * 4, s));
     NT_TRY(ntk_memcpy_h2d_async(score_targets_, targets, (size_t)T * 4, s));
     const int est = ntk_embed_rows(hidden_, token_embd_.ptr, tokens_dev_, T, H, token_embd_.dtype, s);
@@ -436,6 +438,7 @@
     const int H = cfg_.hidden_size, N = kMaxSequences;
     void* s = stream_;
     tp_call_ = 0;
+    touch_token_state();
     int* const host = batch_host_;
     KvTarget kv{0, slots, 0};
     for (int b = 0; b < N; ++b) {
diff --git a/ntransformer_amd/csrc/gemv.hip b/ntransformer_amd/csrc/gemv.hip
--- a/ntransformer_amd/csrc/gemv.hip
+++ b/ntransformer_amd/csrc/gemv.hip
@@ -3,6 +3,7 @@
 #include "ntk_experiments.h"
 #endif
 #include <algorithm>
+#include <cfloat>
 #include <cmath>
 #include <cstdio>
 #include <cstdlib>
@@ -16,11 +17,13 @@
 #endif
 
 enum { NS_ANY = 0, NS_ONE = 1, NS_SPLIT = 2 };
-template <int DT, bool NORM, bool XFAST, bool A16, bool ATT = false, bool XI = false, bool LM = false, int NSF = NS_ANY>
-__device__ __forceinline__ void gemv_quant_body(const GemvParams& p, const int bid, const int nblk, const AttnFuse* attp = nullptr) {
+template <int DT, bool NORM, bool XFAST, bool A16, bool ATT = false, bool XI = false, bool LM = false, int NSF = NS_ANY, bool AMAX = false>
+__device__ __forceinline__ void gemv_quant_body(const GemvParams& p, const int bid, const int nblk, const AttnFuse* attp = nullptr,
+                                                float* amax_sv = nullptr, int* amax_si = nullptr) {
     using F = Fmt<DT>;
     static_assert(!LM || (DT == NTK_DT_Q8_0 && !A16 && !ATT && !XI), "lane-major rows: Q8_0");
     static_assert(NSF == NS_ANY || LM, "compile-time slice forms: the lane-major kernels");
+    static_assert(!AMAX || NSF == NS_ONE, "arg-max candidates: rows of one slice (a wave owns whole rows)");
     constexpr int NL = LM ? 4 : F::NL;
     constexpr int STAGE = LM ? 0 : NL * 1024 + 64;
     extern __shared__ __attribute__((aligned(16))) uint8_t smem[];
@@ -62,7 +65,8 @@
     const int wave = __builtin_amdgcn_readfirstlane(tid >> 6);
     const int ns = NSF == NS_ONE ? 1 : p.ns;
     const bool single = NSF == NS_ANY ? p.ns == 1 : NSF == NS_ONE;
-    const int nwaves = ns * p.rw;
+    const int nwaves = NSF == NS_ONE ? (int)(blockDim.x >> 6) : ns * p.rw;
+    const bool streams = NSF != NS_ONE || wave < p.rw;
     const int s = wave % ns;
     const int g = wave / ns;
     constexpr bool norm = NORM;
@@ -82,7 +86,7 @@
     const int group = bid * p.rw + g;
     const int ngroups = nblk * p.rw;
     const int mats = p.silu_pair ? 2 : 1;
-    const int n_my = (p.total_rows > group) ? ((p.total_rows - 1 - group) / ngroups + 1) * mats : 0;
+    const int n_my = (streams && p.total_rows > group) ? ((p.total_rows - 1 - group) / ngroups + 1) * mats : 0;
 
     static_assert(MAX_SEG == 3, "locate / seg_y: unrolled for three segments");
     const int seg_rows0 = p.seg[0].rows, seg_rows1 = p.seg[1].rows;
@@ -152,7 +156,11 @@
             c[j] = __builtin_nontemporal_load(reinterpret_cast<const u32x4*>(a + 16u * (unsigned)(j * lm_nl + lm_lane)));
         sc = __builtin_nontemporal_load(reinterpret_cast<const uint32_t*>(a + 64u * (unsigned)lm_nl + 4u * (unsigned)lm_lane));
     };
-    auto issue_first = [&]() { issue(); if constexpr (LM) issue_lm(pf, pf_sc); };
+    auto issue_first = [&]() {
+        if constexpr (NSF == NS_ONE) { if (!streams) return; }
+        issue();
+        if constexpr (LM) issue_lm(pf, pf_sc);
+    };
     if (n_my <= 0) { cu_seg = 0; cu_row = 0; }
 
     f32x2 x2[32];
@@ -313,6 +321,7 @@
                 GV_STAMP(9);
                 __syncthreads();
                 GV_STAMP(10);
+                if constexpr (NSF == NS_ONE && !AMAX) { if (!streams) return; }
                 if (s < GS) read_own_row(0);
 #ifdef NTK_GEMV_TRACE
                 asm volatile("s_waitcnt lgkmcnt(0)" ::: "memory");
@@ -349,6 +358,7 @@
                         ximg[img_index(c, g0)] = NORM ? p.x[c] * rms_inv * p.norm_w[c] : p.x[c];
                 }
                 __syncthreads();
+                if constexpr (NSF == NS_ONE && !AMAX) { if (!streams) return; }
                 if (s >= g0 && s < g0 + GS) read_own_row(g0);
             }
         }
@@ -416,6 +426,8 @@
         prefetch_resid(b + 1);
     };
 
+    float amax_v = -FLT_MAX;
+    int amax_i = 0x7FFFFFFF;
     auto row_step = [&](const int q, u32x4 (&cur)[NL], uint32_t& cur_sc, u32x4 (&nxt)[LM ? NL : 1], uint32_t& nxt_sc) __attribute__((always_inline)) {
         const int seg = pf_seg, row = pf_row, shift = A16 ? 0 : pf_shift;
         const float res = pf_res;
@@ -464,6 +476,7 @@
                 float v = tot;
                 if (p.resid != nullptr && seg == 0) v = res + v;
                 p.seg[seg].y[row] = v;
+                if constexpr (AMAX) amax_merge(amax_v, amax_i, v, row);
             }
         } else {
             const int b = q / RB, i = q % RB;
@@ -487,6 +500,18 @@
         }
         for (; done < p.nbatch; ++done) __syncthreads();
     }
+    if constexpr (AMAX) {
+        int* const red_i = reinterpret_cast<int*>(red + 8);
+        if (lane == 63) { red[wave] = amax_v; red_i[wave] = amax_i; }
+        __syncthreads();
+        if (tid == 0) {
+            float v = red[0];
+            int i = red_i[0];
+            for (int w = 1; w < nwaves; ++w) amax_merge(v, i, red[w], red_i[w]);
+            amax_sv[bid] = v;
+            amax_si[bid] = i;
+        }
+    }
 #ifdef NTK_EXPERIMENTS
     if constexpr (ATT) att_finish(*attp, nblk);
 #endif
@@ -502,6 +527,10 @@
 template <bool NORM, bool XFAST, int NSF>
 __global__ __launch_bounds__(512, Fmt<NTK_DT_Q8_0>::MINW) void gemv_q8l_kernel(const GemvParams p) {
     gemv_quant_body<NTK_DT_Q8_0, NORM, XFAST, false, false, false, true, NSF>(p, (int)blockIdx.x, (int)gridDim.x);
+}
+template <bool XFAST>
+__global__ __launch_bounds__(512, Fmt<NTK_DT_Q8_0>::MINW) void gemv_q8l_argmax_kernel(const GemvParams p, float* __restrict__ sv, int* __restrict__ si) {
+    gemv_quant_body<NTK_DT_Q8_0, true, XFAST, false, false, false, true, NS_ONE, true>(p, (int)blockIdx.x, (int)gridDim.x, nullptr, sv, si);
 }
 template <bool UNPACK>
 __global__ __launch_bounds__(256) void q8l_pack_kernel(uint8_t* __restrict__ dst, const uint8_t* __restrict__ src, const int rows, const int in,
@@ -673,6 +702,10 @@
     int grid = (int)std::min<long>((total + p.rw - 1) / p.rw, max_wg);
     grid = std::max(grid, 1);
     L.grid = grid;
+    if (lm && p.ns == 1 && total % grid == 0) {
+        const long share = total / grid, depth = (share + L.nwaves - 1) / L.nwaves;
+        if (share % depth == 0) p.rw = (int)(share / depth);
+    }
     const long ngroups = (long)grid * p.rw;
     const long rows_per_group = (total + ngroups - 1) / ngroups;
     p.nbatch = (int)((rows_per_group * mats + RB - 1) / RB);
@@ -816,6 +849,24 @@
     return last_launch_status();
 }
 
+static int q8l_gemv_argmax(const ntk_gemv_seg* seg, const float* x, int in, const float* norm_w, float eps, float* scratch, int* n_pairs, hipStream_t st) {
+    int ns, sc;
+    if (!q8l_layout(in, ns, sc) || ns != 1) return NTK_E_SHAPE;
+    if (reinterpret_cast<uintptr_t>(seg->W) & 15) return NTK_E_ALIGN;
+    GemvLaunch L;
+    const int rc = prepare_quant<NTK_DT_Q8_0>(seg, 1, x, in, norm_w, eps, nullptr, 0, max_workgroups(), L, true);
+    if (rc != NTK_OK) return rc;
+    if (L.grid > 1024 || L.nwaves > 8 || L.lds > 64 * 1024) return NTK_E_SHAPE;
+    using KernelFn = void (*)(const GemvParams, float*, int*);
+    static const KernelFn table[2] = {gemv_q8l_argmax_kernel<false>, gemv_q8l_argmax_kernel<true>};
+#ifdef NTK_GEMV_TRACE
+    L.p.trace_slot = 0;
+#endif
+    hipLaunchKernelGGL(table[L.xfast ? 1 : 0], dim3(L.grid), dim3(64 * L.nwaves), L.lds, st, L.p, scratch, reinterpret_cast<int*>(scratch + 1024));
+    *n_pairs = L.grid;
+    return last_launch_status();
+}
+
 #ifdef NTK_EXPERIMENTS
 template <int DT>
 static int launch_att(const AttnFuse& att, const ntk_gemv_seg* seg, int in, const float* resid, hipStream_t st) {
@@ -906,6 +957,15 @@
     return ntk::q8l_pack(raw, packed, rows, in_features, true, ntk::resolve_stream(stream));
 }
 
+int ntk_gemv_q8l_argmax(const ntk_gemv_seg* seg, const float* x, int in_features, const float* norm_w, float eps, float* scratch, int* n_pairs,
+                        void* stream) {
+    if (!seg || !seg->W || !seg->y || !x || !norm_w || !scratch || !n_pairs) return NTK_E_NULL;
+    if (seg->dtype != NTK_DT_Q8_0) return NTK_E_DTYPE;
+    if (seg->rows <= 0 || in_features <= 0) return NTK_E_SHAPE;
+    if ((reinterpret_cast<uintptr_t>(x) & 15) || (reinterpret_cast<uintptr_t>(norm_w) & 15)) return NTK_E_ALIGN;
+    return ntk::q8l_gemv_argmax(seg, x, in_features, norm_w, eps, scratch, n_pairs, ntk::resolve_stream(stream));
+}
+
 int ntk_gemv(float* y, const void* W, const float* x, int out_features, int in_features, int weight_dtype, void* stream) {
     if (!y || !W || !x) return NTK_E_NULL;
     if (out_features < 0 || in_features <= 0) return NTK_E_SHAPE;
diff --git a/ntransformer_amd/ops.py b/ntransformer_amd/ops.py
--- a/ntransformer_amd/ops.py
+++ b/ntransformer_amd/ops.py
@@ -418,6 +418,23 @@
     check(_lib.lib().ntk_argmax(_p(logits), n, _p(d_out_token), _p(h_mirror), _p(scratch), stream), "argmax")
 
 
+def argmax_advance(logits, n, d_out_token, d_pos, scratch, h_mirror=None, h_ring4=None, stream=None):
+    check(_lib.lib().ntk_argmax_advance(_p(logits), n, _p(d_out_token), _p(h_mirror), _p(h_ring4), _p(d_pos), _p(scratch), stream), "argmax_advance")
+
+
+def gemv_q8l_argmax(W, y, rows, dtype, x, in_features, norm_w, eps, scratch, stream=None) -> int:
+    seg = (GemvSeg * 1)()
+    seg[0].W, seg[0].y, seg[0].rows, seg[0].dtype = _p(W), _p(y), rows, int(dtype)
+    n = C.c_int(0)
+    check(_lib.lib().ntk_gemv_q8l_argmax(seg, _p(x), in_features, _p(norm_w), eps, _p(scratch), C.byref(n), stream), "gemv_q8l_argmax")
+    return n.value
+
+
+def greedy_tail(scratch, n_pairs, d_out_token, d_pos, hidden_out, table, hidden, dtype, h_mirror=None, h_ring4=None, stream=None):
+    check(_lib.lib().ntk_greedy_tail(_p(scratch), n_pairs, _p(d_out_token), _p(h_mirror), _p(h_ring4), _p(d_pos), _p(hidden_out), _p(table), hidden,
+                                     int(dtype), stream), "greedy_tail")
+
+
 def logprob_rows(logits, n_rows, vocab, ld, targets, logprob, top1=None, stream=None):
     check(_lib.lib().ntk_logprob_rows(_p(logits), n_rows, vocab, ld, _p(targets), _p(logprob), _p(top1), stream), "logprob_rows")
 
```

After: 559.7 tokens/s, median of 6. No clear change (+0.9%).
